# mmaker/c-lwe-snarks

Measured on AMD Instinct MI355X. Metric: snark_proofs_per_sec, higher is better.
Workload: dtype u32 limbs (704-bit integers mod 2^704) + AES-256 bytes; int8 digits on the matrix cores, int32 accumulation (exact)

## Files before the change

c-lwe-snarks_amd/__init__.py:

```python
from __future__ import annotations

import ctypes
import os
from dataclasses import dataclass

import numpy as np

_HERE = os.path.dirname(os.path.abspath(__file__))
LIB_PATH = os.environ.get("MFHIP_LIB") or os.path.join(_HERE, "libmfhip.so")
P = 0xFFFFFFFB


class MfhError(RuntimeError):
    pass


@dataclass(frozen=True)
class Params:

    n: int = 1470
    logq: int = 736
    d: int = 1 << 15
    m: int = 21845

    @property
    def L(self):
        return (self.logq + 63) // 64

    @property
    def K(self):
        return self.logq // 64

    @property
    def lanes(self):
        return (64 * self.K + 55) // 56

    @property
    def ctb(self):
        return self.logq // 8

    @property
    def ctr_ct(self):
        return self.ctb * self.n

    @property
    def ctr_s(self):
        return 0

    @property
    def ctr_as(self):
        return self.ctr_ct * self.d

    @property
    def ctr_bt(self):
        return 2 * self.ctr_ct * self.d

    @property
    def ctr_bv(self):
        return 2 * self.ctr_ct * self.d + self.ctr_ct

    @property
    def ct_limbs(self):
        return (self.n + 1) * self.L


DEBUG = Params(d=256, m=64)
DEFAULT = Params()


class _CParams(ctypes.Structure):
    _fields_ = [("n", ctypes.c_uint32), ("logq", ctypes.c_uint32), ("d", ctypes.c_uint32), ("m", ctypes.c_uint32)]


_lib = None

EXPORTS = [
    "mfh_ctx_create", "mfh_ctx_destroy", "mfh_set_stream", "mfh_sync", "mfh_scrub_staging", "mfh_last_error", "mfh_set_seed",
    "mfh_keystream", "mfh_sample_rows", "mfh_ct_add", "mfh_ct_mul_ui", "mfh_ct_addmul_ui", "mfh_eval_rows",
    "mfh_encrypt_rows", "mfh_decrypt", "mfh_ct_smudge", "mfh_ssp_upload", "mfh_witness_poly", "mfh_version",
    "mfh_workspace_bytes", "mfh_last_kernel_ms", "mfh_set_timing", "mfh_set_overlap", "mfh_eval_rows_multi", "mfh_prove_batch", "mfh_crs_mm_image_bytes", "mfh_crs_expand_mm", "mfh_crs_set_resident_mm", "mfh_witness_poly_multi", "mfh_witness_poly_mm", "mfh_poly_h_multi", "mfh_poly_mul", "mfh_poly_add", "mfh_poly_prepare_t",
    "mfh_ssp_prepare", "mfh_poly_h", "mfh_setup_messages", "mfh_setup", "mfh_setup_image", "mfh_crs_image_set_b", "mfh_prove",
    "mfh_prove_partial", "mfh_prove_finish", "mfh_ct_to_lanes", "mfh_ct_from_lanes", "mfh_lanes_per_value", "mfh_digest128", "mfh_timing_drain", "mfh_timing_busy_ms", "mfh_timing_work_rows", "mfh_set_batch_image", "mfh_set_batch_slabs", "mfh_set_expand_path", "mfh_set_encrypt_path", "mfh_set_batch_launch", "mfh_set_batch_bw", "mfh_set_mm_chunk_rows", "mfh_set_mm_pack", "mfh_set_poly_exact", "mfh_poly_exact_fallbacks", "mfh_set_mm_stream", "mfh_add_dotp", "mfh_set_encrypt_chunks", "mfh_set_witness_per", "mfh_set_eval_path", "mfh_set_decrypt_path", "mfh_decrypt_rows",
    "mfh_crs_mm_share_bytes", "mfh_crs_expand_mm_share", "mfh_crs_set_resident_mm_share", "mfh_batch_chain", "mfh_batch_witness_cols", "mfh_batch_chain_from_w", "mfh_witness_poly_mm_cols", "mfh_prove_batch_partial", "mfh_prove_batch_finish",
    "mfh_resident_row_bytes", "mfh_crs_expand", "mfh_eval_rows_resident", "mfh_crs_set_resident",
    "mfh_witness_lanes", "mfh_witness_from_lanes", "mfh_prove_partial_w", "mfh_verify",
    "mfh_ssp_set_prg", "mfh_ssp_prg_make_t", "mfh_ssp_prg_fill",
    "mfh_resident_share_rows", "mfh_crs_expand_share", "mfh_crs_set_resident_share", "mfh_crs_set_resident_prefix",
    "mfh_prove_batch_supergroup", "mfh_prove_batch_stream_wait", "mfh_set_mm_width",
    "mfh_setup_public", "mfh_prove_public", "mfh_prove_batch_public", "mfh_vk_derive", "mfh_verify_public",
    "mfh_ssp_from_rows", "mfh_ssp_set_rows", "mfh_ssp_rows_fill", "mfh_circuit_create", "mfh_circuit_destroy", "mfh_circuit_assign",
    "mfh_circuit_create_global",
]


def load_library():
    global _lib
    if _lib is not None:
        return _lib
    if not os.path.exists(LIB_PATH):
        raise MfhError(f"{LIB_PATH} is missing: run `python -c 'import __graft_entry__ as g; g.build()'` "
                       "(hipcc --offload-arch=gfx950).  There is no CPU fallback.")
    lib = ctypes.CDLL(LIB_PATH)
    vp, u64, sz, i32, u32 = ctypes.c_void_p, ctypes.c_uint64, ctypes.c_size_t, ctypes.c_int, ctypes.c_uint32
    sig = {
        "mfh_ctx_create": (i32, [ctypes.POINTER(vp), i32, ctypes.POINTER(_CParams)]),
        "mfh_ctx_destroy": (None, [vp]),
        "mfh_set_stream": (i32, [vp, vp]),
        "mfh_sync": (i32, [vp]),
        "mfh_scrub_staging": (i32, [vp]),
        "mfh_last_error": (ctypes.c_char_p, [vp]),
        "mfh_set_seed": (i32, [vp, ctypes.c_char_p]),
        "mfh_keystream": (i32, [vp, u64, vp, sz]),
        "mfh_sample_rows": (i32, [vp, u64, sz, vp]),
        "mfh_ct_add": (i32, [vp, vp, vp, vp, sz]),
        "mfh_ct_mul_ui": (i32, [vp, vp, vp, u32, sz]),
        "mfh_ct_addmul_ui": (i32, [vp, vp, vp, u32, sz]),
        "mfh_eval_rows": (i32, [vp, u64, sz, vp, vp, vp, vp, vp, i32]),
        "mfh_encrypt_rows": (i32, [vp, u64, sz, vp, vp, vp, vp]),
        "mfh_decrypt": (i32, [vp, vp, vp, sz, vp]),
        "mfh_ct_smudge": (i32, [vp, vp, sz, ctypes.c_char_p, sz, ctypes.c_char_p]),
        "mfh_ssp_upload": (i32, [vp, vp, vp, sz, sz]),
        "mfh_witness_poly": (i32, [vp, vp, ctypes.c_char_p, u32, vp]),
        "mfh_version": (ctypes.c_char_p, []),
        "mfh_workspace_bytes": (sz, [vp]),
        "mfh_last_kernel_ms": (ctypes.c_float, [vp, ctypes.c_char_p]),
        "mfh_set_timing": (i32, [vp, i32]),
        "mfh_set_overlap": (i32, [vp, i32]),
        "mfh_eval_rows_multi": (i32, [vp, u64, sz, vp, vp, u32, u32, vp, i32]),
        "mfh_poly_h_multi": (i32, [vp, vp, vp, u32]),
        "mfh_witness_poly_mm": (i32, [vp, vp, u32, ctypes.c_char_p, sz, vp, vp]),
        "mfh_witness_poly_multi": (i32, [vp, vp, u32, ctypes.c_char_p, sz, vp, vp]),
        "mfh_crs_mm_image_bytes": (sz, [vp]),
        "mfh_crs_expand_mm": (i32, [vp, vp, vp]),
        "mfh_crs_set_resident_mm": (i32, [vp, vp]),
        "mfh_prove_batch": (i32, [vp, vp, vp, u32, ctypes.c_char_p, sz, vp, ctypes.c_char_p, sz, ctypes.c_char_p, vp]),
        "mfh_prove_batch_supergroup": (u32, [vp]),
        "mfh_set_mm_width": (i32, [vp, u32, i32]),
        "mfh_prove_batch_stream_wait": (i32, [vp, u32, vp]),
        "mfh_poly_mul": (i32, [vp, vp, sz, vp, sz, vp]),
        "mfh_poly_add": (i32, [vp, vp, vp, sz, vp]),
        "mfh_poly_prepare_t": (i32, [vp, vp]),
        "mfh_ssp_prepare": (i32, [vp, vp]),
        "mfh_poly_h": (i32, [vp, vp, vp]),
        "mfh_setup_messages": (i32, [vp, vp, u32, u32, u32, vp]),
        "mfh_setup": (i32, [vp, vp, u32, u32, u32, vp, vp, vp]),
        "mfh_setup_image": (i32, [vp, vp, u32, u32, u32, vp, vp, vp, vp]),
        "mfh_prove": (i32, [vp, vp, vp, ctypes.c_char_p, u32, ctypes.c_char_p, sz, ctypes.c_char_p, vp]),
        "mfh_prove_partial": (i32, [vp, vp, vp, ctypes.c_char_p, u32, u32, u32, vp]),
        "mfh_prove_finish": (i32, [vp, vp, ctypes.c_char_p, sz, ctypes.c_char_p]),
        "mfh_lanes_per_value": (u32, [vp]),
        "mfh_digest128": (i32, [vp, vp, sz, vp]),
        "mfh_ct_to_lanes": (i32, [vp, vp, sz, vp]),
        "mfh_ct_from_lanes": (i32, [vp, vp, sz, vp]),
        "mfh_add_dotp": (i32, [vp, vp, vp, vp, sz]),
        "mfh_crs_set_resident_prefix": (i32, [vp, vp, sz]),
        "mfh_resident_share_rows": (sz, [vp, u32, u32]),
        "mfh_crs_expand_share": (i32, [vp, vp, u32, u32, vp]),
        "mfh_crs_set_resident_share": (i32, [vp, vp, u32, u32]),
        "mfh_ssp_set_prg": (i32, [vp, u64, vp]),
        "mfh_ssp_prg_make_t": (i32, [vp, u64, ctypes.c_char_p, vp]),
        "mfh_ssp_prg_fill": (i32, [vp, u64, sz, sz, vp]),
        "mfh_verify": (i32, [vp, vp, u32, u32, u32, vp, vp, sz, vp]),
        "mfh_witness_lanes": (i32, [vp, vp, ctypes.c_char_p, u32, u32, vp]),
        "mfh_witness_from_lanes": (i32, [vp, vp, vp, u32, vp]),
        "mfh_prove_partial_w": (i32, [vp, vp, vp, ctypes.c_char_p, u32, u32, u32, vp, vp]),
        "mfh_resident_row_bytes": (sz, [vp]),
        "mfh_crs_expand": (i32, [vp, u64, sz, vp, vp]),
        "mfh_crs_image_set_b": (i32, [vp, sz, sz, vp, vp]),
        "mfh_eval_rows_resident": (i32, [vp, vp, sz, sz, vp, vp, vp, vp, i32]),
        "mfh_crs_set_resident": (i32, [vp, vp]),
        "mfh_timing_drain": (i32, [vp, ctypes.c_char_p, ctypes.POINTER(u64), ctypes.POINTER(ctypes.c_double), ctypes.POINTER(u64),
                                   ctypes.POINTER(ctypes.c_float)]),
        "mfh_timing_busy_ms": (ctypes.c_double, [vp]),
        "mfh_timing_work_rows": (u64, [vp]),
        "mfh_set_batch_image": (i32, [vp, i32]),
        "mfh_set_mm_chunk_rows": (i32, [vp, u32]),
        "mfh_set_mm_pack": (i32, [vp, i32]),
        "mfh_set_poly_exact": (i32, [vp, i32]),
        "mfh_poly_exact_fallbacks": (ctypes.c_long, [vp]),
        "mfh_set_mm_stream": (i32, [vp, i32, i32, i32, u32]),
        "mfh_set_batch_launch": (i32, [vp, u32, i32]),
        "mfh_set_batch_bw": (i32, [vp, i32]),
        "mfh_set_encrypt_path": (i32, [vp, i32]),
        "mfh_set_expand_path": (i32, [vp, i32]),
        "mfh_set_batch_slabs": (i32, [vp, u32]),
        "mfh_set_encrypt_chunks": (i32, [vp, u32]),
        "mfh_set_eval_path": (i32, [vp, i32]),
        "mfh_set_decrypt_path": (i32, [vp, i32]),
        "mfh_decrypt_rows": (i32, [vp, u64, sz, vp, vp, vp]),
        "mfh_set_witness_per": (i32, [vp, u32]),
        "mfh_crs_mm_share_bytes": (sz, [vp, u32, u32]),
        "mfh_crs_expand_mm_share": (i32, [vp, vp, u32, u32, vp]),
        "mfh_crs_set_resident_mm_share": (i32, [vp, vp, u32, u32]),
        "mfh_batch_chain": (i32, [vp, vp, u32, ctypes.c_char_p, sz, vp, vp, vp, vp]),
        "mfh_batch_witness_cols": (i32, [vp, vp, u32, ctypes.c_char_p, sz, vp, u32, u32, vp, sz]),
        "mfh_batch_chain_from_w": (i32, [vp, vp, u32, vp, vp, vp]),
        "mfh_witness_poly_mm_cols": (i32, [vp, vp, u32, ctypes.c_char_p, sz, vp, u32, u32, vp, sz]),
        "mfh_prove_batch_partial": (i32, [vp, vp, u32, u32, u32, ctypes.c_char_p, sz, vp, vp, vp, sz, vp]),
        "mfh_prove_batch_finish": (i32, [vp, vp, u32, vp, ctypes.c_char_p, sz, ctypes.c_char_p, vp]),
        "mfh_setup_public": (i32, [vp, vp, u32, u32, u32, u32, vp, vp, vp, vp]),
        "mfh_prove_public": (i32, [vp, vp, vp, u32, ctypes.c_char_p, u32, ctypes.c_char_p, sz, ctypes.c_char_p, vp]),
        "mfh_prove_batch_public": (i32, [vp, vp, vp, u32, u32, ctypes.c_char_p, sz, vp, ctypes.c_char_p, sz, ctypes.c_char_p, vp]),
        "mfh_vk_derive": (i32, [vp, vp, u32, u32, vp]),
        "mfh_verify_public": (i32, [vp, vp, u32, u32, u32, vp, vp, ctypes.c_char_p, sz, sz, vp]),
        "mfh_ssp_from_rows": (i32, [vp, u32, vp, vp, vp, vp]),
        "mfh_ssp_set_rows": (i32, [vp, u32, vp, vp, vp, u32]),
        "mfh_ssp_rows_fill": (i32, [vp, sz, sz, vp]),
        "mfh_circuit_create": (i32, [vp, u32, u32, vp, u32, vp, ctypes.POINTER(vp)]),
        "mfh_circuit_create_global": (i32, [vp, u32, u32, vp, u32, vp, ctypes.POINTER(vp)]),
        "mfh_circuit_destroy": (None, [vp]),
        "mfh_circuit_assign": (i32, [vp, vp, u32, vp, sz, vp, sz, vp]),
    }
    for name, (res, args) in sig.items():
        fn = getattr(lib, name)
        fn.restype = res
        fn.argtypes = args
    _lib = lib
    return lib


def rows_to_csr(rows):
    if isinstance(rows, tuple) and len(rows) == 3 and all(isinstance(a, np.ndarray) for a in rows):
        row_ptr, wire, coef = rows
    else:
        lens = [len(r) for r in rows]
        row_ptr = np.zeros(len(lens) + 1, dtype=np.int64)
        np.cumsum(lens, out=row_ptr[1:])
        flat = [(int(w), int(a) % P) for r in rows for (w, a) in r]
        wire = np.array([w for w, _ in flat], dtype=np.int64)
        coef = np.array([a for _, a in flat], dtype=np.int64)
    if len(row_ptr) == 0 or min(np.min(row_ptr), np.min(wire, initial=0), np.min(coef, initial=0)) < 0:
        raise MfhError("rows: row_ptr needs nrows + 1 entries, and no entry may be negative")
    if max(np.max(row_ptr), np.max(wire, initial=0), np.max(coef, initial=0)) > 0xFFFFFFFF:
        raise MfhError("rows: entries must fit 32 bits")
    return tuple(np.ascontiguousarray(a, dtype=np.uint32) for a in (row_ptr, wire, coef))


def _ptr(t):
    return ctypes.c_void_p(t.data_ptr()) if t is not None else ctypes.c_void_p(0)


CIRCUIT_MAX_WIRES = 32767


class CircuitProgram:

    def __init__(self, ctx, nin, ngates, handle, state="lds"):
        self._ctx, self.nin, self.ngates, self._h, self.state = ctx, nin, ngates, handle, state

    def close(self):
        if self._h:
            self._ctx.lib.mfh_circuit_destroy(self._h)
            self._h = ctypes.c_void_p()

    def __del__(self):
        try:
            self.close()
        except Exception:
            pass


class Context:

    def __init__(self, params: Params = DEFAULT, device: int = 0):
        import torch

        if not torch.cuda.is_available():
            raise MfhError("no HIP device visible: the MI355X path has no CPU fallback")
        self.torch = torch
        self.lib = load_library()
        self.params = params
        self.device = torch.device("cuda", device)
        self._h = ctypes.c_void_p()
        cp = _CParams(params.n, params.logq, params.d, params.m)
        rc = self.lib.mfh_ctx_create(ctypes.byref(self._h), device, ctypes.byref(cp))
        if rc != 0:
            raise MfhError(f"mfh_ctx_create failed ({rc})")
        self._chk(self.lib.mfh_set_stream(self._h, ctypes.c_void_p(torch.cuda.current_stream(self.device).cuda_stream)))

    def close(self):
        if self._h:
            self.lib.mfh_ctx_destroy(self._h)
            self._h = ctypes.c_void_p()

    def __del__(self):
        try:
            self.close()
        except Exception:
            pass

    def _chk(self, rc):
        if rc != 0:
            raise MfhError(f"libmfhip error {rc}: {self.lib.mfh_last_error(self._h).decode()}")

    def empty(self, nbytes):
        return self.torch.empty(int(nbytes), dtype=self.torch.uint8, device=self.device)

    def zeros(self, nbytes):
        return self.torch.zeros(int(nbytes), dtype=self.torch.uint8, device=self.device)

    def to_device(self, arr):
        a = np.ascontiguousarray(arr)
        if not a.flags.writeable:
            import warnings

            with warnings.catch_warnings():
                warnings.simplefilter("ignore", UserWarning)
                return self.torch.from_numpy(a.view(np.uint8).reshape(-1)).to(self.device)
        return self.torch.from_numpy(a.view(np.uint8).reshape(-1)).to(self.device)

    def to_host(self, t, dtype=np.uint8):
        return t.cpu().numpy().view(dtype)

    def sync(self):
        self._chk(self.lib.mfh_sync(self._h))

    def set_timing(self, on=True):
        self._chk(self.lib.mfh_set_timing(self._h, 1 if on else 0))

    def set_overlap(self, mode=1):
        self._chk(self.lib.mfh_set_overlap(self._h, int(mode)))

    def set_batch_image(self, on=True):
        self._chk(self.lib.mfh_set_batch_image(self._h, 1 if on else 0))

    def set_batch_slabs(self, nslabs=0):
        self._chk(self.lib.mfh_set_batch_slabs(self._h, int(nslabs)))

    def set_expand_path(self, path=0):
        self._chk(self.lib.mfh_set_expand_path(self._h, int(path)))

    def set_encrypt_path(self, path=0):
        self._chk(self.lib.mfh_set_encrypt_path(self._h, int(path)))

    def set_eval_path(self, path=0):
        self._chk(self.lib.mfh_set_eval_path(self._h, int(path)))

    def set_encrypt_chunks(self, chunks=0):
        self._chk(self.lib.mfh_set_encrypt_chunks(self._h, int(chunks)))

    def set_witness_per(self, statements=0):
        self._chk(self.lib.mfh_set_witness_per(self._h, int(statements)))

    def set_batch_launch(self, groups_per_launch=4, merge_regions=True):
        self._chk(self.lib.mfh_set_batch_launch(self._h, int(groups_per_launch), 1 if merge_regions else 0))

    def set_batch_bw(self, merged=True):
        self._chk(self.lib.mfh_set_batch_bw(self._h, 1 if merged else 0))

    def set_mm_stream(self, map=0, persistent=False, sync_mode=0, spin_max=64):
        self._chk(self.lib.mfh_set_mm_stream(self._h, int(map), int(persistent), int(sync_mode), int(spin_max)))

    def set_mm_width(self, per_xcd=32, early_chain=False):
        self._chk(self.lib.mfh_set_mm_width(self._h, int(per_xcd), 1 if early_chain else 0))

    def set_mm_pack(self, on=True):
        self._chk(self.lib.mfh_set_mm_pack(self._h, 1 if on else 0))

    def set_poly_exact(self, mode=1):
        self._chk(self.lib.mfh_set_poly_exact(self._h, int(mode)))

    def poly_exact_fallbacks(self):
        return int(self.lib.mfh_poly_exact_fallbacks(self._h))

    def set_mm_chunk_rows(self, rows=0):
        self._chk(self.lib.mfh_set_mm_chunk_rows(self._h, int(rows)))

    def timing_drain(self, which):
        n, rows, ms, last = ctypes.c_uint64(), ctypes.c_uint64(), ctypes.c_double(), ctypes.c_float()
        self._chk(self.lib.mfh_timing_drain(self._h, which.encode(), ctypes.byref(n), ctypes.byref(ms), ctypes.byref(rows), ctypes.byref(last)))
        return n.value, ms.value, rows.value

    def timing_busy_ms(self):
        return float(self.lib.mfh_timing_busy_ms(self._h))

    def timing_work_rows(self):
        return int(self.lib.mfh_timing_work_rows(self._h))

    def last_kernel_ms(self, which):
        return float(self.lib.mfh_last_kernel_ms(self._h, which.encode()))

    def set_seed(self, seed: bytes):
        assert len(seed) == 40
        self._chk(self.lib.mfh_set_seed(self._h, bytes(seed)))

    def keystream(self, off, nbytes, out=None):
        out = self.empty(nbytes) if out is None else out
        self._chk(self.lib.mfh_keystream(self._h, off, _ptr(out), nbytes))
        return out

    def sample_rows(self, off, nrows):
        p = self.params
        out = self.empty(nrows * p.n * p.L * 8)
        self._chk(self.lib.mfh_sample_rows(self._h, off, nrows, _ptr(out)))
        return out

    def ct_add(self, a, b, count=1, out=None):
        out = self.empty(a.numel()) if out is None else out
        self._chk(self.lib.mfh_ct_add(self._h, _ptr(out), _ptr(a), _ptr(b), count))
        return out

    def ct_mul_ui(self, a, x, count=1, out=None):
        out = self.empty(a.numel()) if out is None else out
        self._chk(self.lib.mfh_ct_mul_ui(self._h, _ptr(out), _ptr(a), x, count))
        return out

    def ct_addmul_ui(self, rop, a, x, count=1):
        self._chk(self.lib.mfh_ct_addmul_ui(self._h, _ptr(rop), _ptr(a), x, count))
        return rop

    def eval_rows(self, off, nrows, c8, coeff0, coeff1=None, rop0=None, rop1=None, accumulate=False):
        p = self.params
        if rop0 is None:
            rop0 = self.empty(p.ct_limbs * 8)
        if coeff1 is not None and rop1 is None:
            rop1 = self.empty(p.ct_limbs * 8)
        self._chk(self.lib.mfh_eval_rows(self._h, off, nrows, _ptr(c8), _ptr(coeff0), _ptr(coeff1), _ptr(rop0), _ptr(rop1),
                                         1 if accumulate else 0))
        return rop0, rop1

    def eval_rows_multi(self, off, nrows, c8, coeffs, nvec, out=None, accumulate=False, coeff_bytes=4):
        out = self.empty(nvec * self.params.ct_limbs * 8) if out is None else out
        self._chk(self.lib.mfh_eval_rows_multi(self._h, off, nrows, _ptr(c8), _ptr(coeffs), nvec, coeff_bytes, _ptr(out), 1 if accumulate else 0))
        return out

    def encrypt_rows(self, off, nrows, sk, msg, err, out=None):
        p = self.params
        out = self.empty(nrows * p.ctb) if out is None else out
        self._chk(self.lib.mfh_encrypt_rows(self._h, off, nrows, _ptr(sk), _ptr(msg), _ptr(err), _ptr(out)))
        return out

    def decrypt(self, sk, cts, count, out=None):
        out = self.empty(4 * count) if out is None else out
        self._chk(self.lib.mfh_decrypt(self._h, _ptr(sk), _ptr(cts), count, _ptr(out)))
        return out

    def set_decrypt_path(self, path=0):
        self._chk(self.lib.mfh_set_decrypt_path(self._h, int(path)))

    def decrypt_rows(self, off, nrows, sk, c8, out=None):
        out = self.empty(4 * nrows) if out is None else out
        self._chk(self.lib.mfh_decrypt_rows(self._h, off, nrows, _ptr(sk), _ptr(c8), _ptr(out)))
        return out

    def ct_smudge(self, cts, count, mag: bytes, maglen, sign: bytes):
        self._chk(self.lib.mfh_ct_smudge(self._h, _ptr(cts), count, bytes(mag), maglen, bytes(sign)))
        return cts

    def ssp_upload(self, ssp_host_u64: np.ndarray, d_ssp=None, first_slot=0, nslots=None):
        p = self.params
        nslots = p.m + 3 if nslots is None else nslots
        if d_ssp is None:
            d_ssp = self.empty((p.m + 3) * p.d * 4)
        a = np.ascontiguousarray(ssp_host_u64)
        self._chk(self.lib.mfh_ssp_upload(self._h, ctypes.c_void_p(a.ctypes.data), _ptr(d_ssp), first_slot, nslots))
        return d_ssp

    def ssp_from_rows(self, rows, d_ssp=None):
        p = self.params
        row_ptr, wire, coef = rows_to_csr(rows)
        if d_ssp is None:
            d_ssp = self.empty((p.m + 3) * p.d * 4)
        self._chk(self.lib.mfh_ssp_from_rows(self._h, len(row_ptr) - 1, ctypes.c_void_p(row_ptr.ctypes.data), ctypes.c_void_p(wire.ctypes.data),
                                             ctypes.c_void_p(coef.ctypes.data), _ptr(d_ssp)))
        return d_ssp

    def ssp_set_rows(self, rows, lu_max=0):
        if rows is None:
            self._chk(self.lib.mfh_ssp_set_rows(self._h, 0, None, None, None, 0))
            return
        row_ptr, wire, coef = rows_to_csr(rows)
        self._chk(self.lib.mfh_ssp_set_rows(self._h, len(row_ptr) - 1, ctypes.c_void_p(row_ptr.ctypes.data), ctypes.c_void_p(wire.ctypes.data),
                                            ctypes.c_void_p(coef.ctypes.data), int(lu_max)))

    def ssp_rows_fill(self, first_slot, nslots):
        out = self.empty(max(nslots, 1) * self.params.d * 4)
        self._chk(self.lib.mfh_ssp_rows_fill(self._h, first_slot, nslots, _ptr(out)))
        return out

    def circuit_load(self, compiled, state="lds"):
        if state not in ("lds", "global", "auto"):
            raise MfhError(f"circuit_load: state must be 'lds', 'global' or 'auto', got {state!r}")
        gates = np.ascontiguousarray(compiled.gates, dtype=np.uint32).reshape(-1, 3)
        asserts = np.ascontiguousarray(compiled.asserts, dtype=np.uint32).reshape(-1, 2)
        nin = compiled.nwires - len(gates)
        if state == "auto":
            state = "lds" if compiled.nwires <= CIRCUIT_MAX_WIRES else "global"
        create = self.lib.mfh_circuit_create if state == "lds" else self.lib.mfh_circuit_create_global
        h = ctypes.c_void_p()
        self._chk(create(self._h, nin, len(gates), ctypes.c_void_p(gates.ctypes.data), len(asserts), ctypes.c_void_p(asserts.ctypes.data), ctypes.byref(h)))
        return CircuitProgram(self, nin, len(gates), h, state)

    def circuit_assign(self, prog, bits):
        bits = np.asarray(bits, dtype=np.uint8)
        if bits.ndim != 2 or bits.shape[1] != prog.nin:
            raise MfhError(f"circuit_assign: bits must be [nb, {prog.nin}] (public then private bits), got {bits.shape}")
        nb = bits.shape[0]
        packed = np.ascontiguousarray(np.packbits(bits & 1, axis=1, bitorder="little"))
        stride = (self.params.m + 7) // 8
        witness = np.zeros((nb, stride), dtype=np.uint8)
        holds = np.zeros(nb, dtype=np.uint8)
        self._chk(self.lib.mfh_circuit_assign(self._h, prog._h, nb, ctypes.c_void_p(packed.ctypes.data), packed.shape[1], ctypes.c_void_p(witness.ctypes.data),
# ... 313 lines not shown
```

c-lwe-snarks_amd/csrc/ctx.hpp:

```cpp
#pragma once
#include <hip/hip_runtime.h>

#include <stdint.h>
#include <string.h>

#include <string>
#include <vector>

#include "aes_dev.hpp"
#include "mfhip.h"
#include "ssp_prg.hpp"

#define HIP_TRY(ctx, expr)                                                        \
  do {                                                                            \
    hipError_t e_ = (expr);                                                       \
    if (e_ != hipSuccess) {                                                       \
      (ctx)->err = std::string(#expr) + ": " + hipGetErrorString(e_);             \
      return MFH_EDEVICE;                                                         \
    }                                                                             \
  } while (0)

struct PolyState;
struct SspInterp;
struct SspRows;
struct RowsTree;

struct PinBuf {
  void *p = nullptr;
  size_t cap = 0;
  hipEvent_t ev = nullptr;
  bool pending = false;
  size_t used = 0;
};

struct mfh_ctx {
  mfh_params P{};
  int device = 0;
  hipStream_t own_stream = nullptr;
  hipStream_t stream = nullptr;
  mf::AesKey key{};
  bool have_seed = false;
  uint32_t *d_t0 = nullptr;
  void *ws = nullptr;
  size_t ws_bytes = 0;
  void *ws2 = nullptr;
  size_t ws2_bytes = 0;
  int mm_ws_sel = 0;
  void *ws3 = nullptr;
  size_t ws3_bytes = 0;
  std::vector<hipEvent_t> ev_cdone, ev_rdone, ev_wdone;
  std::vector<hipEvent_t> ev_round;
  std::vector<hipEvent_t> ev_sgdone;
  uint32_t last_batch_sg = 0, last_batch_n = 0;
  void *wws = nullptr;
  size_t wws_bytes = 0;
  uint64_t *lazy = nullptr;
  uint32_t *lazy_cnt = nullptr;
  size_t lazy_bytes = 0;
  bool eval_dense = false;
  bool overlap = true;
  int overlap_mode = 1;
  hipStream_t side = nullptr, side2 = nullptr;
  hipEvent_t ev_fork = nullptr, ev_join = nullptr;
  hipEvent_t ev_chain = nullptr, ev_chain_done = nullptr;
  std::string err;
  bool timing = false;
  struct Timed {
    hipEvent_t e0, e1;
    int kind;
    uint64_t rows;
    uint64_t work;
    int sub;
  };
  std::vector<Timed> timed;
  double last_busy_ms = 0;
  uint64_t last_work_rows = 0;
  std::vector<hipEvent_t> ev_pool;
  PolyState *poly = nullptr;
  void *aux = nullptr;
  size_t aux_bytes = 0;
  uint32_t *d_msg = nullptr;
  size_t msg_rows = 0;
  uint32_t *d_prover = nullptr;
  size_t prover_words = 0;
  std::vector<uint32_t> h_cw;
  const uint8_t *mm_image = nullptr;
  uint32_t mm_rank = 0, mm_world = 1;
  uint64_t mm_off[3] = {0, 0, 0}, mm_rows[3] = {0, 0, 0};
  size_t mm_base[3] = {0, 0, 0};
  void *ssp_frag = nullptr;
  size_t ssp_frag_bytes = 0;
  const uint32_t *ssp_frag_src = nullptr;
  SspInterp *interp = nullptr;
  void *circ_io = nullptr;
  size_t circ_io_bytes = 0;
  void *circ_state = nullptr;
  size_t circ_state_bytes = 0;
  void *d_batch = nullptr;
  size_t batch_bytes = 0;
  void *batch_img = nullptr;
  size_t batch_img_bytes = 0;
  int batch_image = 1;
  int mm_map = 1;
  bool mm_persist = true;
  bool mm_wave1 = false;
  uint32_t mm_sync_mode = 0, mm_spin = 64;
  uint32_t mm_width = 32;
  size_t early_ws_half = 0;
  bool batch_early_chain = false;
  uint32_t *mm_sync = nullptr;
  int poly_exact = 1;
  bool mm_pack = true;
  uint32_t mm_chunk_rows = 131071;
  int expand_path = 0;
  int enc_path = 0;
  uint32_t ncu = 256;
  int dec_path = 0;
  int eval_path = 0;
  uint32_t enc_chunks = 0;
  uint32_t witness_per = 0;
  uint32_t batch_slabs = 0;
  int batch_bw_merged = 1;
  int batch_merge = 1;
  uint32_t batch_ngl = 8;
  PinBuf pin_rows, pin_cw, pin_smudge;
  PinBuf pin_pub;
  uint8_t *d_pub = nullptr;
  size_t pub_bytes = 0;
  PinBuf pin_wring[8];
  uint32_t pin_wnext = 0;
  hipEvent_t ev_sample = nullptr;
  void *sample_tmp = nullptr;
  size_t sample_bytes = 0;
  void *uploader = nullptr;
  bool prg_on = false;
  uint64_t prg_seed = 0;
  const uint32_t *prg_t = nullptr;
  SspRows *rows = nullptr;
  RowsTree *rows_tree = nullptr;
  const uint32_t *rows_prefix = nullptr;
  uint32_t rows_lu_max = 0;
  const uint8_t *resident_rows = nullptr;
  uint64_t resident_nrows = ~0ull;
  bool resident_sharded = false;
  uint32_t res_rank = 0, res_world = 1;
};

struct Timer {
  mfh_ctx *c;
  mfh_ctx::Timed t{};
  bool on;
  Timer(mfh_ctx *c_, int kind, uint64_t rows, uint64_t work = 0, int sub = 0) : c(c_), on(c_->timing) {
    if (!on) return;
    auto get = [&]() {
      hipEvent_t e;
      if (!c->ev_pool.empty()) { e = c->ev_pool.back(); c->ev_pool.pop_back(); }
      else hipEventCreate(&e);
      return e;
    };
    t.e0 = get(); t.e1 = get(); t.kind = kind; t.rows = rows; t.work = work ? work : rows; t.sub = sub;
    hipEventRecord(t.e0, c->stream);
  }
  ~Timer() {
    if (!on) return;
    hipEventRecord(t.e1, c->stream);
    c->timed.push_back(t);
  }
};

inline void *pin_acquire(mfh_ctx *c, PinBuf &b, size_t bytes) {
  if (b.pending) { hipEventSynchronize(b.ev); b.pending = false; }
  if (bytes > b.cap) {
    if (b.p) hipHostFree(b.p);
    b.cap = (bytes + 4095) & ~(size_t)4095;
    if (hipHostMalloc(&b.p, b.cap, hipHostMallocDefault) != hipSuccess) { b.p = nullptr; b.cap = 0; c->err = "hipHostMalloc failed"; return nullptr; }
  }
  if (!b.ev) hipEventCreateWithFlags(&b.ev, hipEventDisableTiming);
  b.used = bytes;
  return b.p;
}
inline void pin_release(mfh_ctx *c, PinBuf &b) {
  hipEventRecord(b.ev, c->stream);
  b.pending = true;
}
inline void pin_scrub(PinBuf &b) {
  if (b.pending) { hipEventSynchronize(b.ev); b.pending = false; }
  if (b.p && b.used) {
    volatile unsigned char *q = (volatile unsigned char *)b.p;
    memset((void *)q, 0, b.used);
    __asm__ __volatile__("" : : "r"(b.p) : "memory");
  }
  b.used = 0;
}
inline void pin_free(PinBuf &b) {
  if (b.pending) hipEventSynchronize(b.ev);
  if (b.p) hipHostFree(b.p);
  if (b.ev) hipEventDestroy(b.ev);
  b = PinBuf();
}

inline int ssp_src(mfh_ctx *c, const uint32_t *d_ssp, mf::SspSrc &src, bool rows_ok = false) {
  if (d_ssp) { src = mf::SspSrc{d_ssp, d_ssp, 0}; return MFH_OK; }
  if (c->rows_prefix) {
    if (!rows_ok) { c->err = "this entry point does not take the row SSP (mfh_ssp_set_rows): pass a dense d_ssp"; return MFH_EUNSUPPORTED; }
    src = mf::SspSrc{c->rows_prefix, c->rows_prefix, 0, c->rows_lu_max + 2};
    return MFH_OK;
  }
  if (!c->prg_on || !c->prg_t) { c->err = "d_ssp is NULL and no generator-defined SSP is registered (mfh_ssp_set_prg)"; return MFH_EINVAL; }
  src = mf::SspSrc{nullptr, c->prg_t, c->prg_seed};
  return MFH_OK;
}

void mfh_poly_destroy(mfh_ctx *c);
void ssp_interp_free(mfh_ctx *c);
void ssp_rows_free(mfh_ctx *c, bool tree);
int ssp_rows_check(mfh_ctx *c, const char *who, uint32_t nrows, const uint32_t *h_row_ptr, const uint32_t *h_wire, const uint32_t *h_coef);
int ssp_rows_tree(mfh_ctx *c, const char *who, const uint32_t *&d_t, const uint32_t *&h_w);
int ssp_rows_witness(mfh_ctx *c, uint32_t nstmt, const uint8_t *h_bits, size_t bits_stride, const uint32_t *h_delta, uint32_t *d_w, size_t w_stride);
int ssp_rows_msg_evals(mfh_ctx *c, uint32_t s, uint32_t beta, uint32_t *d_msg_evals);
inline bool ssp_is_rows(const mfh_ctx *c, const uint32_t *d_ssp) { return !d_ssp && c->rows_prefix; }
inline int ssp_rows_lu_check(mfh_ctx *c, const uint32_t *d_ssp, uint32_t lu) {
  if (ssp_is_rows(c, d_ssp) && lu > c->rows_lu_max) { c->err = "lu exceeds the lu_max the row SSP was registered with (mfh_ssp_set_rows)"; return MFH_EINVAL; }
  return MFH_OK;
}
extern "C" int mfh_witness_poly_mm(mfh_ctx *c, const uint32_t *d_ssp, uint32_t nstmt, const uint8_t *h_bits, size_t bits_stride, const uint32_t *h_delta,
                                   uint32_t *d_w);
extern "C" int mfh_witness_poly_mm_cols(mfh_ctx *c, const uint32_t *d_ssp, uint32_t nstmt, const uint8_t *h_bits, size_t bits_stride, const uint32_t *h_delta,
                                        uint32_t col0, uint32_t ncols, uint32_t *d_w, size_t w_stride);
extern "C" int mfh_poly_h_multi(mfh_ctx *c, const uint32_t *d_v, uint32_t *d_h, uint32_t nb);
int aux_reserve(mfh_ctx *c, size_t bytes);
int expand_mm_region(mfh_ctx *c, uint64_t off, uint32_t nrows, const uint8_t *c8, uint8_t *image);
int encrypt_rows_mm(mfh_ctx *c, uint64_t off, size_t nrows, const uint64_t *sk, const uint32_t *msg, const uint64_t *err, uint8_t *c8);
int decrypt_mm(mfh_ctx *c, const uint64_t *sk, const uint64_t *cts, size_t count, uint32_t *out);
int decrypt_rows_mm(mfh_ctx *c, uint64_t off, size_t nrows, const uint64_t *sk, const uint8_t *c8, uint32_t *out);

struct MmIo {
  const uint32_t *coef[2];
  uint32_t csplit;
  uint64_t *out[2];
  uint32_t osplit;
  uint64_t ostride;
  const uint8_t *bits;
  uint32_t bits_stride;
  int64_t *sc_zeroed;
  uint64_t cstride;
  uint32_t bits_row0;
  const uint64_t *add_ct;
  const uint32_t *add_scale;
  uint32_t sa_from1;
};
int eval_rows_multi_io(mfh_ctx *c, uint64_t off, size_t nrows, const uint8_t *d_c8, const MmIo &io, uint32_t nvec, uint32_t coeff_bytes, int accumulate);
int eval_rows_multi_io_set(mfh_ctx *c, uint64_t off, size_t nrows, const uint8_t *d_c8, const MmIo *ios, const uint32_t *nvecs, uint32_t ng,
                           uint32_t coeff_bytes);
struct MmRegion { uint64_t off; const uint8_t *c8; };
int eval_rows_multi_io_regions(mfh_ctx *c, const MmRegion *regs, uint32_t nreg, size_t nrows, const MmIo *ios, const uint32_t *nvecs, uint32_t ng,
                               uint32_t coeff_bytes, int accumulate);
bool mm_image_covers(const mfh_ctx *c, uint64_t off, size_t nrows);
struct MmsPlan {
  uint32_t ng, ngt, ND, nrows, nchunks, rpc, rpad, ntiles, mtiles;
  size_t cd_bytes, part_bytes;
  const uint8_t *img[2];
  int8_t *cd;
  int *part;
};
bool mms_plan(mfh_ctx *c, const MmRegion *regs, uint32_t nreg, size_t nrows, const MmIo *ios, const uint32_t *nvecs, uint32_t ng, uint32_t coeff_bytes,
              MmsPlan &P);
size_t mms_ws_bytes(const MmsPlan &P);
void mms_bind(MmsPlan &P, void *ws);
int mms_digits(mfh_ctx *c, const MmsPlan &P, const MmIo *ios, const uint32_t *nvecs);
int mms_stream(mfh_ctx *c, const MmsPlan &P);
int mms_finish(mfh_ctx *c, const MmsPlan &P, const MmIo *ios, const uint32_t *nvecs, int accumulate);

inline int buf_reserve(mfh_ctx *c, void *&buf, size_t &have, size_t bytes) {
  if (bytes <= have) return MFH_OK;
  if (buf) {
    hipStreamSynchronize(c->stream);
    hipFree(buf);
    buf = nullptr;
    have = 0;
  }
  bytes = (bytes + (1u << 20) - 1) & ~(size_t)((1u << 20) - 1);
  if (hipMalloc(&buf, bytes) != hipSuccess) {
    c->err = "hipMalloc(workspace) failed";
    return MFH_ENOMEM;
  }
  have = bytes;
  return MFH_OK;
}
inline int lazy_reserve(mfh_ctx *c, size_t bytes) {
  if (bytes <= c->lazy_bytes) return MFH_OK;
  if (c->lazy) {
    hipStreamSynchronize(c->stream);
    hipFree(c->lazy);
    c->lazy = nullptr;
    c->lazy_bytes = 0;
  }
  bytes = (bytes + 255) & ~(size_t)255;
  if (hipMalloc((void **)&c->lazy, bytes + 256) != hipSuccess) {
    c->err = "hipMalloc(lazy image) failed";
    return MFH_ENOMEM;
  }
  if (hipMemsetAsync(c->lazy, 0, bytes + 256, c->stream) != hipSuccess) return MFH_EDEVICE;
  c->lazy_cnt = reinterpret_cast<uint32_t *>(reinterpret_cast<uint8_t *>(c->lazy) + bytes);
  c->lazy_bytes = bytes;
  return MFH_OK;
}
inline int ws_reserve(mfh_ctx *c, size_t bytes) { return buf_reserve(c, c->ws, c->ws_bytes, bytes); }
inline int wws_reserve(mfh_ctx *c, size_t bytes) { return buf_reserve(c, c->wws, c->wws_bytes, bytes); }
inline int ws2_reserve(mfh_ctx *c, size_t bytes) { return buf_reserve(c, c->ws2, c->ws2_bytes, bytes); }
```

c-lwe-snarks_amd/csrc/evalmm.hip:

```cpp
#include <algorithm>
#include <cstring>

#include "ctx.hpp"

namespace {

using mf::AesKey;

constexpr int CT = 4;
constexpr int SB = 88;
constexpr int VB = 92;
constexpr int MB = CT * SB;
constexpr int MT = MB / 32;
constexpr int RT = 128;
constexpr int TSTRIDE = 384;
constexpr int BLK_PER_ROW = 24;
static_assert(MB % 32 == 0 && CT * VB + 15 <= TSTRIDE, "tile geometry");

typedef int v4i __attribute__((ext_vector_type(4)));
typedef int v16i __attribute__((ext_vector_type(16)));

__device__ __forceinline__ uint32_t coef_at(const MmIo &io, uint32_t v, uint32_t nrows, uint32_t i) {
  if (io.bits) {
    const uint32_t a = io.bits_row0 + i;
// ... 1029 lines not shown
      y ^= y >> 16;
      y *= 0x7FEB352Du;
      y ^= y >> 15;
      y *= 0x846CA68Bu;
      y ^= y >> 16;
      x[e] = y;
    }
    v4i bq[4];
#pragma unroll
    for (int w = 0; w < 4; w++)
#pragma unroll
      for (int j = 0; j < 4; j++) {
        const uint32_t lo = __builtin_amdgcn_perm(x[4 * j + 1], x[4 * j], 0x0c0c0400u + 0x00000101u * w);
        const uint32_t hi = __builtin_amdgcn_perm(x[4 * j + 3], x[4 * j + 2], 0x04000c0cu + 0x01010000u * w);
        bq[w][j] = (int)((lo | hi) ^ 0x80808080u);
      }
#pragma unroll
    for (int t = 0; t < MT; t++)
#pragma unroll
      for (int w = 0; w < 4; w++) acc[t][w] = __builtin_amdgcn_mfma_i32_32x32x32_i8(aq[t], bq[w], acc[t][w], 0, 0, 0);
  };
  uint32_t K = K0;
  for (; K + 2 <= K1; K += 2) {
    step(K, 0);
    step(K + 1, 1);
  }
  if (K < K1) step(K, 0);
#pragma unroll
  for (int t = 0; t < MT; t++)
#pragma unroll
    for (int w = 0; w < 4; w++)
#pragma unroll
      for (int e = 0; e < 16; e++) {
        const uint32_t stmt = 32 * t + (e & 3) + 8 * (e >> 2) + 4 * h;
        part[(((uint64_t)blockIdx.y * 4 + w) * (32 * MT) + stmt) * d + k] = acc[t][w][e];
      }
}
__global__ __launch_bounds__(512) void k_witness_mm8q_prg(const uint32_t *__restrict__ rowkeys, const v4i *__restrict__ bitfrag, uint32_t nrowsel ,
                                                          uint32_t ksteps_per_chunk, uint32_t d, int *__restrict__ part, WCols wc) {
  constexpr int MT = 8, RING = 4;
  __shared__ v4i bits[RING][MT][64];
  __shared__ uint32_t xch[3][2][4][64][4];
  const uint32_t tid = threadIdx.x, lane = tid & 63, wave = tid >> 6;
  const uint32_t r32 = lane & 31, h = lane >> 5;
  const uint32_t tile = wave >> 2, pl = wave & 3;
  const uint32_t sh = pl >> 1, pp = pl & 1;
  const uint32_t pos = (pl + (lane >> 4)) & 3;
  const uint32_t ktl = blockIdx.x * 2 + tile, kt = wc.kt0 + ktl;
  const uint32_t kc = kt * 32 + r32 + 0x632BE5ABu;
  const uint32_t K0 = blockIdx.y * ksteps_per_chunk, K1 = min((nrowsel + 31) / 32, K0 + ksteps_per_chunk);
  v16i acc[4][2];
#pragma unroll
  for (int t = 0; t < 4; t++)
#pragma unroll
    for (int q = 0; q < 2; q++)
#pragma unroll
      for (int e = 0; e < 16; e++) acc[t][q][e] = 0;
  if (K0 >= K1) return;
  auto bits_load = [&](uint32_t K) -> v4i { return bitfrag[(uint64_t)min(K, K1 - 1) * MT * 64 + tid]; };
  auto bits_store = [&](uint32_t K, v4i st) { (&bits[K % RING][0][0])[tid] = st; };
  auto rk_load = [&](uint32_t K) -> uint4 { return *reinterpret_cast<const uint4 *>(rowkeys + 32 * (uint64_t)min(K, K1 - 1) + 16 * h + 4 * pos); };
  auto hash1 = [&](uint32_t rowkey) -> uint32_t {
#ifdef WPRG_NOHASH
    return kc ^ rowkey;
#endif
    uint32_t y = kc * rowkey;
    y ^= y >> 16;
    y *= 0x7FEB352Du;
    y ^= y >> 15;
    y *= 0x846CA68Bu;
    y ^= y >> 16;
    return y;
  };
  auto publish = [&](uint32_t K, const uint32_t (&x)[4]) {
#pragma unroll
    for (int w = 0; w < 4; w++) {
      const uint32_t lo = __builtin_amdgcn_perm(x[1], x[0], 0x0c0c0400u + 0x00000101u * w);
      const uint32_t hi = __builtin_amdgcn_perm(x[3], x[2], 0x04000c0cu + 0x01010000u * w);
      xch[K % 3][tile][w][lane][pos] = (lo | hi) ^ 0x80808080u;
    }
  };
  auto fragment = [&](uint32_t K, uint32_t q) -> v4i { return *reinterpret_cast<const v4i *>(&xch[K % 3][tile][2 * pp + q][lane][0]); };
  uint4 rkr[4];
  v4i sta, stb;
  sta = bits_load(K0);
  bits_store(K0, sta);
  sta = bits_load(K0 + 1);
  stb = bits_load(K0 + 2);
  {
    const uint4 r0 = rk_load(K0), r1 = rk_load(K0 + 1);
    const uint32_t x0[4] = {hash1(r0.x), hash1(r0.y), hash1(r0.z), hash1(r0.w)};
    const uint32_t x1[4] = {hash1(r1.x), hash1(r1.y), hash1(r1.z), hash1(r1.w)};
    publish(K0, x0);
    publish(K0 + 1, x1);
  }
#pragma unroll
  for (int i = 2; i <= 5; i++) rkr[i & 3] = rk_load(K0 + i);
  __syncthreads();
  v4i bq0 = fragment(K0, 0), bq1 = fragment(K0, 1);
  uint32_t K = K0;
  auto step = [&](int slot, v4i &st) {
    const v4i bn0 = fragment(K + 1, 0), bn1 = fragment(K + 1, 1);
    const uint4 rk = rkr[(slot + 2) & 3];
    const uint32_t hr[4] = {rk.x, rk.y, rk.z, rk.w};
    uint32_t hx[4];
    bits_store(K + 1, st);
    const v4i *aq = &bits[K % RING][4 * sh][lane];
#pragma unroll
    for (int t = 0; t < 4; t++) {
      const v4i a = aq[t * 64];
#ifdef WPRG_NOMFMA
      acc[t][0][0] += a[0] ^ bq0[t];
      acc[t][1][0] += a[1] ^ bq1[t];
#else
      acc[t][0] = __builtin_amdgcn_mfma_i32_32x32x32_i8(a, bq0, acc[t][0], 0, 0, 0);
      acc[t][1] = __builtin_amdgcn_mfma_i32_32x32x32_i8(a, bq1, acc[t][1], 0, 0, 0);
#endif
      hx[t] = hash1(hr[t]);
    }
    publish(K + 2, hx);
    rkr[(slot + 2) & 3] = rk_load(K + 6);
    bq0 = bn0;
    bq1 = bn1;
    st = bits_load(K + 3);
#ifndef WPRG_NOSYNC
    __syncthreads();
#endif
    K++;
  };
  while (K + 4 <= K1) {
    step(0, sta);
    step(1, stb);
    step(2, sta);
    step(3, stb);
  }
  if (K < K1) step(0, sta);
  if (K < K1) step(1, stb);
  if (K < K1) step(2, sta);
  uint32_t dd = d;
  asm volatile("" : "+s"(dd));
#pragma unroll
  for (int q = 0; q < 2; q++) {
    int *dst = part + (((uint64_t)blockIdx.y * 4 + 2 * pp + q) * (32 * MT) + 128 * sh) * dd + ktl * 32 + r32 + (uint64_t)(4 * h) * dd;
#pragma unroll
    for (int t = 0; t < 4; t++) {
#pragma unroll
      for (int e = 0; e < 16; e++) dst[(uint64_t)((e & 3) + 8 * (e >> 2)) * dd] = acc[t][q][e];
      dst += (uint64_t)32 * dd;
    }
  }
}
__global__ __launch_bounds__(512) void k_witness_mm8q(const v4i *__restrict__ sspfrag, const v4i *__restrict__ bitfrag, uint32_t nrowsel ,
                                                      uint32_t ksteps_per_chunk, uint32_t d, int *__restrict__ part, const uint32_t *__restrict__ tpoly ,
                                                      const uint32_t *__restrict__ cnt_delta, uint32_t nstmt, uint32_t *__restrict__ w_out, WCols wc) {
  constexpr int MT = 8, RING = 4, PF = 4;
  __shared__ v4i bits[RING][MT][64];
  __shared__ uint32_t xch[2][3][16][64];
  const uint32_t tid = threadIdx.x, lane = tid & 63, wave = tid >> 6;
  const uint32_t r32 = lane & 31, h = lane >> 5;
  const uint32_t tile = wave >> 2, pl = wave & 3;
  const uint32_t ktl = blockIdx.x * 2 + tile, kt = wc.kt0 + ktl;
  const uint32_t K0 = blockIdx.y * ksteps_per_chunk, K1 = min((nrowsel + 31) / 32, K0 + ksteps_per_chunk);
  v16i acc[MT];
#pragma unroll
  for (int t = 0; t < MT; t++)
#pragma unroll
    for (int e = 0; e < 16; e++) acc[t][e] = 0;
  if (K0 >= K1) return;
  auto bits_load = [&](uint32_t K) -> v4i { return bitfrag[(uint64_t)min(K, K1 - 1) * MT * 64 + tid]; };
  auto bits_store = [&](uint32_t K, v4i st) { (&bits[K % RING][0][0])[tid] = st; };
  auto ssp_load = [&](uint32_t K) -> v4i { return sspfrag[(((uint64_t)kt * wc.KS + min(K, K1 - 1)) * 4 + pl) * 64 + lane]; };
  v4i stg[PF], bq[PF];
  {
    const v4i s0 = bits_load(K0), s1 = bits_load(K0 + 1);
    __builtin_amdgcn_sched_barrier(0);
#pragma unroll
    for (int i = 0; i < PF; i++) {
      bq[i] = ssp_load(K0 + i);
      stg[i] = bits_load(K0 + 2 + i);
      __builtin_amdgcn_sched_barrier(0);
    }
    bits_store(K0, s0);
    bits_store(K0 + 1, s1);
  }
  __syncthreads();
  v4i acur[MT];
#pragma unroll
  for (int t = 0; t < MT; t++) acur[t] = bits[K0 % RING][t][lane];
  uint32_t K = K0;
  auto step = [&](int slot) {
    bits_store(K + 2, stg[slot]);
    v4i anext[MT];
    const v4i *aq = &bits[(K + 1) % RING][0][lane];
#pragma unroll
    for (int t = 0; t < MT; t++) anext[t] = aq[t * 64];
    __builtin_amdgcn_sched_barrier(0);
#pragma unroll
    for (int t = 0; t < MT; t++) acc[t] = __builtin_amdgcn_mfma_i32_32x32x32_i8(acur[t], bq[slot], acc[t], 0, 0, 0);
    __builtin_amdgcn_sched_barrier(0);
    bq[slot] = ssp_load(K + PF);
    stg[slot] = bits_load(K + 2 + PF);
#pragma unroll
    for (int t = 0; t < MT; t++) acur[t] = anext[t];
    __syncthreads();
    K++;
  };
  while (K + PF <= K1) {
#pragma unroll
    for (int i = 0; i < PF; i++) step(i);
  }
#pragma unroll
  for (int i = 0; i + 1 < PF; i++)
    if (K < K1) step(i);
  uint32_t dd = d;
  asm volatile("" : "+s"(dd));
  if (part) {
    int *dst = part + ((uint64_t)blockIdx.y * 4 + pl) * (32 * MT) * dd + ktl * 32 + r32 + (uint64_t)(4 * h) * dd;
#pragma unroll
    for (int t = 0; t < MT; t++) {
#pragma unroll
      for (int e = 0; e < 16; e++) dst[(uint64_t)((e & 3) + 8 * (e >> 2)) * dd] = acc[t][e];
      dst += (uint64_t)32 * dd;
    }
    return;
  }
  asm volatile("" : "+s"(cnt_delta), "+s"(tpoly));
  const uint32_t k = ktl * 32 + r32;
  const uint64_t tk = tpoly[k], ws = wc.wstride, P = MFH_P;
#pragma unroll
  for (int t = 0; t < MT; t++) {
    const uint32_t owner = t >> 1;
    uint32_t mine[16];
#pragma unroll
    for (int e = 0; e < 16; e++) {
      const uint32_t b = 32 * t + (e & 3) + 8 * (e >> 2) + 4 * h;
      mine[e] = (uint32_t)acc[t][e] + (b < nstmt ? 128u * cnt_delta[2 * b] : 0u);
    }
    if (pl != owner) {
      const uint32_t sidx = pl - (pl > owner);
#pragma unroll
      for (int e = 0; e < 16; e++) xch[tile][sidx][e][lane] = mine[e];
    }
    __syncthreads();
    if (pl == owner) {
#pragma unroll
      for (int e = 0; e < 16; e++) {
        const uint32_t b = 32 * t + (e & 3) + 8 * (e >> 2) + 4 * h;
        if (b < nstmt) {
          uint64_t val = (uint64_t)mine[e] << (8 * owner);
#pragma unroll
          for (int o = 0; o < 4; o++)
            if (o != (int)owner) val += (uint64_t)xch[tile][o - (o > (int)owner)][e][lane] << (8 * o);
          w_out[(uint64_t)b * ws + k] = (uint32_t)((val % P + tk * cnt_delta[2 * b + 1] % P) % P);
        }
      }
    }
    __syncthreads();
  }
}
__global__ void k_witness_bits(const uint8_t *__restrict__ bits, size_t bits_stride, uint32_t nstmt, uint32_t nrowsel, uint32_t ksteps, uint32_t MT,
                               int8_t *__restrict__ bitfrag) {
  const uint32_t i = blockIdx.x * blockDim.x + threadIdx.x;
  if (i >= ksteps * MT * 64) return;
  const uint32_t lane = i & 63, t = (i >> 6) % MT, K = (i >> 6) / MT, stmt = 32 * t + (lane & 31), h = lane >> 5;
  const uint32_t r0 = K * 32 + 16 * h;
  uint32_t w = 0;
  if (stmt < nstmt && r0 < nrowsel) {
    const uint8_t *b = bits + (size_t)stmt * bits_stride + (r0 >> 3);
    w = b[0];
    if (r0 + 8 < nrowsel) w |= (uint32_t)b[1] << 8;
    if (nrowsel - r0 < 16) w &= (1u << (nrowsel - r0)) - 1;
  }
  uint32_t o[4];
#pragma unroll
  for (int q = 0; q < 4; q++) {
    const uint32_t n4 = (w >> (4 * q)) & 15;
    o[q] = (n4 & 1) | ((n4 & 2) << 7) | ((n4 & 4) << 14) | ((n4 & 8) << 21);
  }
  reinterpret_cast<uint4 *>(bitfrag)[i] = uint4{o[0], o[1], o[2], o[3]};
}
__global__ void k_witness_mm_finish(const int *__restrict__ part, uint32_t nchunks, const uint32_t *__restrict__ t, const uint32_t *__restrict__ cnt_delta,
                                    uint32_t nstmt, uint32_t mrows , uint32_t d, uint32_t *__restrict__ w_out, uint64_t wstride) {
  const uint32_t k = blockIdx.x * blockDim.x + threadIdx.x, b = blockIdx.y;
  if (k >= d || b >= nstmt) return;
  const uint64_t corr = 128ull * cnt_delta[2 * b];
  const uint32_t delta = cnt_delta[2 * b + 1];
  uint64_t val = 0;
#pragma unroll
  for (int w = 0; w < 4; w++) {
    int64_t g = 0;
    for (uint32_t ch = 0; ch < nchunks; ch++) g += part[(((uint64_t)ch * 4 + w) * mrows + b) * d + k];
    val += (uint64_t)(g + (int64_t)corr) << (8 * w);
  }
  const uint64_t P = MFH_P;
  w_out[(uint64_t)b * wstride + k] = (uint32_t)((val % P + (uint64_t)t[k] * delta % P) % P);
}

}

extern "C" {

struct WideGeom { uint32_t ct, sby, vby, mt, mbp, LL; };
static WideGeom wide_geom(const mfh_ctx *c) {
  if (c->P.logq == 736) return {W16<736>::CT, W16<736>::SBY, W16<736>::VBY, W16<736>::MT, W16<736>::MBP, W16<736>::LL};
  return {W16<1472>::CT, W16<1472>::SBY, W16<1472>::VBY, W16<1472>::MT, W16<1472>::MBP, W16<1472>::LL};
}

#define FINISH_LAUNCH(kern, ND_, PK_, grid, ...)                                                                         \
  do {                                                                                                                   \
    if ((PK_) && wg.sby / 4 <= 22) hipLaunchKernelGGL((kern<ND_, 22, true>), grid, dim3(256), 0, c->stream, __VA_ARGS__);  \
    else if (PK_) hipLaunchKernelGGL((kern<ND_, 46, true>), grid, dim3(256), 0, c->stream, __VA_ARGS__);                 \
    else if (wg.sby / 4 <= 22) hipLaunchKernelGGL((kern<ND_, 22, false>), grid, dim3(256), 0, c->stream, __VA_ARGS__);   \
    else hipLaunchKernelGGL((kern<ND_, 46, false>), grid, dim3(256), 0, c->stream, __VA_ARGS__);                         \
  } while (0)
// ... 209 lines not shown
  if (mms_group_args(P, ios, nvecs, A)) {
    uint32_t nvmax = 0;
    for (uint32_t g = 0; g < P.ngt; g++) nvmax = std::max(nvmax, nvecs[g]);
    FINISH_LAUNCH(k_evalmm_finish_groups, 4, pk, dim3(n + 1, (nvmax + 63) / 64, P.ngt), P.part, (uint64_t)(P.part_bytes / 4), P.nchunks, P.ntiles, (uint32_t)N2, n, P.nrows,
                  wg.ct, wg.mbp, wg.sby, wg.LL, A, accumulate);
    HIP_TRY(c, hipGetLastError());
    return MFH_OK;
  }
  for (uint32_t g = 0; g < P.ngt; g++) {
    const dim3 fgrid(n + 1, (nvecs[g] + 63) / 64);
    int *pg = P.part + g * (P.part_bytes / 4);
    if (P.ND == 4)
      FINISH_LAUNCH(k_evalmm_finish, 4, pk, fgrid, pg, ios[g].sc_zeroed, P.nchunks, P.ntiles, (uint32_t)N2, nvecs[g], n, P.nrows, wg.ct, wg.mbp, wg.sby, wg.LL, ios[g],
                    accumulate);
    else
      FINISH_LAUNCH(k_evalmm_finish, 1, pk, fgrid, pg, ios[g].sc_zeroed, P.nchunks, P.ntiles, (uint32_t)N2, nvecs[g], n, P.nrows, wg.ct, wg.mbp, wg.sby, wg.LL, ios[g],
                    accumulate);
  }
  HIP_TRY(c, hipGetLastError());
  return MFH_OK;
}
int eval_rows_multi_io_regions(mfh_ctx *c, const MmRegion *regs, uint32_t nreg, size_t nrows, const MmIo *ios, const uint32_t *nvecs, uint32_t ng,
                               uint32_t coeff_bytes, int accumulate) {
  if (!c || !regs || !ios || !nvecs || !ng || !nreg || nreg * ng > 16) return MFH_EINVAL;
  MmsPlan P;
  if (!mms_plan(c, regs, nreg, nrows, ios, nvecs, ng, coeff_bytes, P)) {
    for (uint32_t g = 0; g < nreg * ng; g++) {
      int rc = eval_rows_multi_io(c, regs[g / ng].off, nrows, regs[g / ng].c8, ios[g], nvecs[g], coeff_bytes, accumulate);
      if (rc) return rc;
    }
    return MFH_OK;
  }
  HIP_TRY(c, hipSetDevice(c->device));
  int rc = c->mm_ws_sel ? ws2_reserve(c, mms_ws_bytes(P)) : ws_reserve(c, mms_ws_bytes(P));
  if (rc) return rc;
  mms_bind(P, c->mm_ws_sel ? c->ws2 : c->ws);
  rc = mms_digits(c, P, ios, nvecs);
  if (!rc) rc = mms_stream(c, P);
  if (!rc) rc = mms_finish(c, P, ios, nvecs, accumulate);
  return rc;
}
int eval_rows_multi_io_set(mfh_ctx *c, uint64_t off, size_t nrows, const uint8_t *d_c8, const MmIo *ios, const uint32_t *nvecs, uint32_t ng,
                           uint32_t coeff_bytes) {
  const MmRegion reg = {off, d_c8};
  return eval_rows_multi_io_regions(c, &reg, 1, nrows, ios, nvecs, ng, coeff_bytes, 0);
}
bool mm_image_covers(const mfh_ctx *c, uint64_t off, size_t nrows) {
  for (int r = 0; r < 3 && c->mm_image; r++)
    if (c->mm_off[r] == off && c->mm_rows[r] == nrows && nrows) return true;
  return false;
}

extern "C" {

static size_t mm_region_bytes(const mfh_ctx *c, uint64_t rows) {
  const WideGeom wg = wide_geom(c);
  const uint64_t mtiles = (uint64_t)((c->P.n + 1 + wg.ct - 1) / wg.ct) * wg.mt, ksteps = (rows + RT2 - 1) / RT2 * (RT2 / 64);
  return (size_t)(mtiles * ksteps * 1024);
}
struct MmShare { uint64_t row0[3], rows[3]; };
static MmShare mm_share(const mfh_ctx *c, uint32_t rank, uint32_t world) {
  const uint64_t d = c->P.d, m = c->P.m;
  const uint64_t loS = d * rank / world, cS = d * (rank + 1) / world - loS, lo = m * rank / world, cnt = m * (rank + 1) / world - lo;
  return MmShare{{loS, d + loS, 2 * d + lo}, {cS, cS, cnt}};
}
size_t mfh_crs_mm_share_bytes(const mfh_ctx *c, uint32_t rank, uint32_t world) {
  if (!c || !world || rank >= world) return 0;
  const MmShare sh = mm_share(c, rank, world);
  return mm_region_bytes(c, sh.rows[0]) + mm_region_bytes(c, sh.rows[1]) + mm_region_bytes(c, sh.rows[2]);
}
size_t mfh_crs_mm_image_bytes(const mfh_ctx *c) { return mfh_crs_mm_share_bytes(c, 0, 1); }
int mfh_crs_expand_mm_share(mfh_ctx *c, const uint8_t *d_crs_c8, uint32_t rank, uint32_t world, uint8_t *d_image) {
  if (!c || !d_crs_c8 || !d_image || !world || rank >= world) return MFH_EINVAL;
  if (!c->have_seed) { c->err = "mfh_set_seed has not been called"; return MFH_EINVAL; }
  const WideGeom wg = wide_geom(c);
  const uint32_t n = c->P.n;
  if (((uint64_t)n * wg.vby) & 7) { c->err = "mfh_crs_expand_mm: the row length must be a multiple of 8"; return MFH_EUNSUPPORTED; }
  HIP_TRY(c, hipSetDevice(c->device));
  const uint64_t ctr_ct = (uint64_t)wg.vby * n;
  const MmShare sh = mm_share(c, rank, world);
  AesKey keyx = c->key;
  for (int i = 56; i < 60; i++) keyx.rk[i] ^= 0x80808080u;
  const uint32_t ntiles = (n + 1 + wg.ct - 1) / wg.ct;
  size_t base = 0;
  for (int r = 0; r < 3; r++) {
    if (!sh.rows[r]) continue;
    const uint32_t units = (uint32_t)((sh.rows[r] + RT2 - 1) / RT2);
    const uint32_t nchunks = std::max(1u, std::min(units, 4u));
    const uint32_t rpc = (units + nchunks - 1) / nchunks * RT2;
    Timer t(c, 9, sh.rows[r]);
    const dim3 grid(ntiles, (uint32_t)((sh.rows[r] + rpc - 1) / rpc));
    const uint8_t *c8 = d_crs_c8 + (size_t)sh.row0[r] * wg.vby;
    if (c->expand_path == 0 && ((ctr_ct * sh.row0[r]) & 7) == 0) {
      int rc = expand_mm_region(c, ctr_ct * sh.row0[r], (uint32_t)sh.rows[r], c8, d_image + base);
      if (rc) return rc;
      base += mm_region_bytes(c, sh.rows[r]);
      continue;
    }
    if (c->P.logq == 736)
      hipLaunchKernelGGL((k_evalmm16<1, 736>), grid, dim3(1024), 0, c->stream, keyx, c->d_t0, ctr_ct * sh.row0[r], n, (uint32_t)sh.rows[r], rpc, c8,
                         (const int8_t *)nullptr, (int *)nullptr, d_image + base);
    else
      hipLaunchKernelGGL((k_evalmm16<1, 1472>), grid, dim3(1024), 0, c->stream, keyx, c->d_t0, ctr_ct * sh.row0[r], n, (uint32_t)sh.rows[r], rpc, c8,
                         (const int8_t *)nullptr, (int *)nullptr, d_image + base);
    base += mm_region_bytes(c, sh.rows[r]);
  }
  HIP_TRY(c, hipGetLastError());
  return MFH_OK;
}
int mfh_crs_expand_mm(mfh_ctx *c, const uint8_t *d_crs_c8, uint8_t *d_image) { return mfh_crs_expand_mm_share(c, d_crs_c8, 0, 1, d_image); }
int mfh_set_mm_stream(mfh_ctx *c, int map, int persistent, int sync_mode, uint32_t spin_max) {
  if (!c || map < 0 || map > 1 || sync_mode < 0 || sync_mode > 2 || persistent < 0 || persistent > 2) return MFH_EINVAL;
  c->mm_map = map;
  c->mm_persist = persistent != 0;
  c->mm_wave1 = persistent == 2;
  c->mm_sync_mode = (uint32_t)sync_mode;
  c->mm_spin = spin_max;
  return MFH_OK;
}
int mfh_set_mm_width(mfh_ctx *c, uint32_t per_xcd, int early_chain) {
  if (!c || per_xcd < 1 || per_xcd > 32) return MFH_EINVAL;
  c->mm_width = per_xcd;
  c->batch_early_chain = early_chain != 0;
  return MFH_OK;
}
int mfh_set_mm_pack(mfh_ctx *c, int on) {
  if (!c) return MFH_EINVAL;
  c->mm_pack = on != 0;
  return MFH_OK;
}
int mfh_set_mm_chunk_rows(mfh_ctx *c, uint32_t rows) {
  if (!c || rows > 131071) return MFH_EINVAL;
  c->mm_chunk_rows = rows ? rows : 131071;
  return MFH_OK;
}
int mfh_crs_set_resident_mm_share(mfh_ctx *c, const uint8_t *d_image, uint32_t rank, uint32_t world) {
  if (!c || !world || rank >= world) return MFH_EINVAL;
  c->mm_image = d_image;
  c->mm_rank = rank;
  c->mm_world = world;
  const uint64_t ctr_ct = (uint64_t)wide_geom(c).vby * c->P.n;
  const MmShare sh = mm_share(c, rank, world);
  size_t base = 0;
  for (int r = 0; r < 3; r++) {
    c->mm_off[r] = ctr_ct * sh.row0[r];
    c->mm_rows[r] = sh.rows[r];
    c->mm_base[r] = base;
    base += mm_region_bytes(c, sh.rows[r]);
  }
  return MFH_OK;
}
int mfh_crs_set_resident_mm(mfh_ctx *c, const uint8_t *d_image) { return mfh_crs_set_resident_mm_share(c, d_image, 0, 1); }

int mfh_witness_poly_mm_cols(mfh_ctx *c, const uint32_t *d_ssp, uint32_t nstmt, const uint8_t *h_bits, size_t bits_stride, const uint32_t *h_delta,
                             uint32_t col0, uint32_t ncols, uint32_t *d_w, size_t w_stride) {
  if (!c || !h_bits || !h_delta || !d_w || nstmt == 0 || nstmt > 256) return MFH_EINVAL;
  mf::SspSrc src;
  {
    int rc0 = ssp_src(c, d_ssp, src);
    if (rc0) return rc0;
  }
  const uint32_t MT = nstmt > 128 ? 8 : nstmt > 64 ? 4 : nstmt > 32 ? 2 : 1;
  const uint32_t d = c->P.d, m = c->P.m;
  if (d % 128 || m < 2) { c->err = "mfh_witness_poly_mm: d must be a multiple of 128"; return MFH_EUNSUPPORTED; }
  if ((uint64_t)col0 + ncols > d || w_stride < ncols) return MFH_EINVAL;
  if (ncols == 0) return MFH_OK;
  if (col0 % 128 || ncols % 128) { c->err = "mfh_witness_poly_mm_cols: the coefficient range must start and end at multiples of 128"; return MFH_EUNSUPPORTED; }
  const uint32_t nc = ncols;
  const WCols wc = {col0 / 32, (m - 1 + 31) / 32, (uint64_t)w_stride};
  const uint32_t *tpoly = src.t + col0;
  for (uint32_t b = 0; b < nstmt; b++)
    if (h_delta[b] >= MFH_P) { c->err = "delta must be < p"; return MFH_EINVAL; }
  HIP_TRY(c, hipSetDevice(c->device));
  const uint32_t nrowsel = m - 1, ksteps = (nrowsel + 31) / 32;
  const bool fused = MT == 8 && src.dense && m < 65536 && (nc >= 16384 || ksteps <= 64);
  const uint32_t nchunks = fused ? 1u : std::min(ksteps, 4u), kpc = (ksteps + nchunks - 1) / nchunks;
  const size_t sfrag_b = (size_t)ksteps * 32 * d * 4;
  if (src.dense && (c->ssp_frag_src != d_ssp || c->ssp_frag_bytes < sfrag_b)) {
    if (c->ssp_frag_bytes < sfrag_b) {
      if (c->ssp_frag) { hipStreamSynchronize(c->stream); hipFree(c->ssp_frag); c->ssp_frag = nullptr; c->ssp_frag_bytes = 0; }
      HIP_TRY(c, hipMalloc(&c->ssp_frag, sfrag_b));
      c->ssp_frag_bytes = sfrag_b;
    }
    const uint64_t nthreads = (uint64_t)ksteps * (d / 32) * 256;
    hipLaunchKernelGGL(k_ssp_frag, dim3((uint32_t)((nthreads + 255) / 256)), dim3(256), 0, c->stream, d_ssp, nrowsel, d, (uint32_t *)c->ssp_frag);
    HIP_TRY(c, hipGetLastError());
    c->ssp_frag_src = d_ssp;
  }
  const size_t packed = (size_t)nstmt * bits_stride, head_b = ((packed + 8 + 256 * 8 + 255) & ~(size_t)255);
  const size_t frag_b = (size_t)ksteps * MT * 1024, part_b = (size_t)nchunks * 4 * 32 * MT * nc * 4;
  const size_t rk_b = src.dense ? 0 : (((size_t)ksteps * 32 * 4 + 255) & ~(size_t)255);
  int rc = wws_reserve(c, head_b + frag_b + part_b + rk_b);
  if (rc) return rc;
  PinBuf &wpin = c->pin_wring[c->pin_wnext++ % 8];
  uint8_t *stage = (uint8_t *)pin_acquire(c, wpin, head_b);
  if (!stage) return MFH_ENOMEM;
  memcpy(stage, h_bits, packed);
  uint32_t *cd = (uint32_t *)(stage + packed + ((8 - packed % 8) % 8));
  for (uint32_t b = 0; b < nstmt; b++) {
    uint32_t cnt = 0;
    const uint8_t *hb = h_bits + (size_t)b * bits_stride;
    for (uint32_t r = 0; r + 8 <= nrowsel; r += 8) cnt += (uint32_t)__builtin_popcount(hb[r >> 3]);
    for (uint32_t r = nrowsel & ~7u; r < nrowsel; r++) cnt += (hb[r >> 3] >> (r & 7)) & 1;
    cd[2 * b] = cnt;
    cd[2 * b + 1] = h_delta[b];
  }
  uint8_t *dev = (uint8_t *)c->wws;
  HIP_TRY(c, hipMemcpyAsync(dev, stage, head_b, hipMemcpyHostToDevice, c->stream));
  pin_release(c, wpin);
  const uint32_t *d_cd = (const uint32_t *)(dev + packed + ((8 - packed % 8) % 8));
  int8_t *d_frag = (int8_t *)(dev + head_b);
  int *d_part = (int *)(dev + head_b + frag_b);
  hipLaunchKernelGGL(k_witness_bits, dim3((uint32_t)((frag_b / 16 + 255) / 256)), dim3(256), 0, c->stream, dev, bits_stride, nstmt, nrowsel, ksteps, MT, d_frag);
  if (!src.dense) {
    uint32_t *d_rk = (uint32_t *)(dev + head_b + frag_b + part_b);
    const dim3 grid(nc / 128, (ksteps + kpc - 1) / kpc);
    hipLaunchKernelGGL(k_prg_rowkeys, dim3((ksteps * 32 + 255) / 256), dim3(256), 0, c->stream, src.seed, ksteps * 32, d_rk);
    if (MT == 8)
      hipLaunchKernelGGL(k_witness_mm8q_prg, dim3(nc / 64, (ksteps + kpc - 1) / kpc), dim3(512), 0, c->stream, d_rk, (const v4i *)d_frag, nrowsel, kpc, nc, d_part, wc);
    else if (MT == 1) hipLaunchKernelGGL(k_witness_mm_prg<1>, grid, dim3(256), 0, c->stream, d_rk, (const v4i *)d_frag, nrowsel, kpc, nc, d_part, wc);
    else if (MT == 2) hipLaunchKernelGGL(k_witness_mm_prg<2>, grid, dim3(256), 0, c->stream, d_rk, (const v4i *)d_frag, nrowsel, kpc, nc, d_part, wc);
    else hipLaunchKernelGGL(k_witness_mm_prg<4>, grid, dim3(256), 0, c->stream, d_rk, (const v4i *)d_frag, nrowsel, kpc, nc, d_part, wc);
  } else if (MT == 8) {
    hipLaunchKernelGGL(k_witness_mm8q, dim3(nc / 64, (ksteps + kpc - 1) / kpc), dim3(512), 0, c->stream, (const v4i *)c->ssp_frag, (const v4i *)d_frag, nrowsel, kpc, nc,
                       fused ? (int *)nullptr : d_part, tpoly, d_cd, nstmt, d_w, wc);
    if (fused) {
      HIP_TRY(c, hipGetLastError());
      return MFH_OK;
    }
  } else if (MT == 1)
    hipLaunchKernelGGL(k_witness_mm<1>, dim3(nc / 128, (ksteps + kpc - 1) / kpc), dim3(256), 0, c->stream, (const v4i *)c->ssp_frag, (const v4i *)d_frag,
                       nrowsel, kpc, nc, d_part, wc);
  else if (MT == 2)
    hipLaunchKernelGGL(k_witness_mm<2>, dim3(nc / 128, (ksteps + kpc - 1) / kpc), dim3(256), 0, c->stream, (const v4i *)c->ssp_frag, (const v4i *)d_frag,
                       nrowsel, kpc, nc, d_part, wc);
  else
    hipLaunchKernelGGL(k_witness_mm<4>, dim3(nc / 128, (ksteps + kpc - 1) / kpc), dim3(256), 0, c->stream, (const v4i *)c->ssp_frag, (const v4i *)d_frag,
                       nrowsel, kpc, nc, d_part, wc);
  hipLaunchKernelGGL(k_witness_mm_finish, dim3((nc + 255) / 256, nstmt), dim3(256), 0, c->stream, d_part, (ksteps + kpc - 1) / kpc, tpoly, d_cd, nstmt, 32 * MT,
                     nc, d_w, (uint64_t)w_stride);
  HIP_TRY(c, hipGetLastError());
  return MFH_OK;
}

int mfh_witness_poly_mm(mfh_ctx *c, const uint32_t *d_ssp, uint32_t nstmt, const uint8_t *h_bits, size_t bits_stride, const uint32_t *h_delta,
                        uint32_t *d_w) {
  if (!c) return MFH_EINVAL;
  if (ssp_is_rows(c, d_ssp)) {
    if (!h_bits || !h_delta || !d_w || nstmt == 0 || nstmt > 256) return MFH_EINVAL;
    return ssp_rows_witness(c, nstmt, h_bits, bits_stride, h_delta, d_w, c->P.d);
  }
  return mfh_witness_poly_mm_cols(c, d_ssp, nstmt, h_bits, bits_stride, h_delta, 0, c->P.d, d_w, c->P.d);
}

}
```

c-lwe-snarks_amd/csrc/mfhip.hip:

```cpp
#include <hip/hip_runtime.h>

#include <stdint.h>
#include <stdio.h>
#include <string.h>

#include <algorithm>
#include <string>
#include <thread>
#include <vector>

#include "aes_dev.hpp"
#include "mfhip.h"

using mf::AesKey;

template <int LOGQ>
struct PS {
  static constexpr int CTB = LOGQ / 8;
  static constexpr int EW = CTB / 4;
  static constexpr int L = (LOGQ + 63) / 64;
  static constexpr int K = LOGQ / 64;
  static constexpr int KW = 2 * K;
  static constexpr int TILE = LOGQ == 736 ? 512 : 256;
  static constexpr int ROWS = 2;
// ... 936 lines not shown
  if (P->logq != 736 && P->logq != 1472) return MFH_EUNSUPPORTED;
  if (P->n == 0 || P->n > (1u << 20)) return MFH_EINVAL;
  int ndev = 0;
  if (hipGetDeviceCount(&ndev) != hipSuccess || ndev <= 0 || device < 0 || device >= ndev) return MFH_EDEVICE;
  if (hipSetDevice(device) != hipSuccess) return MFH_EDEVICE;
  mfh_ctx *c = new mfh_ctx();
  c->P = *P;
  c->device = device;
  {
    int ncu = 0;
    if (hipDeviceGetAttribute(&ncu, hipDeviceAttributeMultiprocessorCount, device) == hipSuccess && ncu > 0) c->ncu = (uint32_t)ncu;
  }
  if (hipStreamCreateWithFlags(&c->own_stream, hipStreamNonBlocking) != hipSuccess) {
    delete c;
    return MFH_EDEVICE;
  }
  c->stream = c->own_stream;
  uint32_t t0[512];
  mf::make_t0_le(t0);
  for (int a = 0; a < 256; a++) t0[256 + a] = (t0[a] << 24) | (t0[a] >> 8);
  if (hipMalloc(&c->d_t0, sizeof t0) != hipSuccess || hipMemcpy(c->d_t0, t0, sizeof t0, hipMemcpyHostToDevice) != hipSuccess) {
    mfh_ctx_destroy(c);
    return MFH_EDEVICE;
  }
  *out = c;
  return MFH_OK;
}

void mfh_ctx_destroy(mfh_ctx *c) {
  if (!c) return;
  hipSetDevice(c->device);
  if (c->stream) hipStreamSynchronize(c->stream);
  mfh_poly_destroy(c);
  ssp_interp_free(c);
  ssp_rows_free(c, true);
  upload_free(c);
  if (c->sample_tmp) hipFree(c->sample_tmp);
  if (c->ev_sample) hipEventDestroy(c->ev_sample);
  pin_free(c->pin_rows);
  for (auto &b : c->pin_wring) pin_free(b);
  pin_free(c->pin_cw);
  pin_free(c->pin_smudge);
  pin_free(c->pin_pub);
  if (c->side) hipStreamSynchronize(c->side);
  if (c->ws) hipFree(c->ws);
  if (c->wws) hipFree(c->wws);
  if (c->ws2) hipFree(c->ws2);
  if (c->ws3) hipFree(c->ws3);
  if (c->mm_sync) hipFree(c->mm_sync);
  for (hipEvent_t e : c->ev_round) hipEventDestroy(e);
  for (hipEvent_t e : c->ev_sgdone) hipEventDestroy(e);
  for (hipEvent_t e : c->ev_cdone) hipEventDestroy(e);
  for (hipEvent_t e : c->ev_rdone) hipEventDestroy(e);
  for (hipEvent_t e : c->ev_wdone) hipEventDestroy(e);
  if (c->lazy) hipFree(c->lazy);
  if (c->aux) hipFree(c->aux);
  if (c->ev_fork) hipEventDestroy(c->ev_fork);
  if (c->ev_join) hipEventDestroy(c->ev_join);
  if (c->ev_chain) hipEventDestroy(c->ev_chain);
  if (c->ev_chain_done) hipEventDestroy(c->ev_chain_done);
  if (c->side) hipStreamDestroy(c->side);
  if (c->side2) hipStreamDestroy(c->side2);
  if (c->d_msg) hipFree(c->d_msg);
  if (c->d_prover) hipFree(c->d_prover);
  if (c->d_pub) hipFree(c->d_pub);
  if (c->d_batch) hipFree(c->d_batch);
  if (c->batch_img) hipFree(c->batch_img);
  if (c->circ_io) hipFree(c->circ_io);
  if (c->circ_state) hipFree(c->circ_state);
  if (c->ssp_frag) hipFree(c->ssp_frag);
  if (c->d_t0) hipFree(c->d_t0);
  for (auto &t : c->timed) { hipEventDestroy(t.e0); hipEventDestroy(t.e1); }
  for (auto e : c->ev_pool) hipEventDestroy(e);
  if (c->own_stream) hipStreamDestroy(c->own_stream);
  delete c;
}

int mfh_set_stream(mfh_ctx *c, void *s) {
  if (!c) return MFH_EINVAL;
  c->stream = (hipStream_t)s;
  return MFH_OK;
}

int mfh_sync(mfh_ctx *c) {
  if (!c) return MFH_EINVAL;
  HIP_TRY(c, hipStreamSynchronize(c->stream));
  return MFH_OK;
}

int mfh_scrub_staging(mfh_ctx *c) {
  if (!c) return MFH_EINVAL;
  pin_scrub(c->pin_rows);
  pin_scrub(c->pin_cw);
  pin_scrub(c->pin_smudge);
  for (auto &b : c->pin_wring) pin_scrub(b);
  return MFH_OK;
}

const char *mfh_last_error(const mfh_ctx *c) { return c ? c->err.c_str() : "null context"; }
size_t mfh_workspace_bytes(const mfh_ctx *c) { return c ? c->ws_bytes : 0; }
int mfh_set_overlap(mfh_ctx *c, int en) {
  if (!c) return MFH_EINVAL;
  c->overlap = en != 0;
  c->overlap_mode = en > 1 ? en : 1;
  return MFH_OK;
}

int mfh_set_expand_path(mfh_ctx *c, int path) {
  if (!c || path < 0 || path > 1) return MFH_EINVAL;
  c->expand_path = path;
  return MFH_OK;
}

int mfh_set_encrypt_path(mfh_ctx *c, int path) {
  if (!c || path < 0 || path > 2) return MFH_EINVAL;
  c->enc_path = path;
  return MFH_OK;
}

int mfh_set_eval_path(mfh_ctx *c, int path) {
  if (!c || path < 0 || path > 1) return MFH_EINVAL;
  c->eval_path = path;
  return MFH_OK;
}
int mfh_set_encrypt_chunks(mfh_ctx *c, uint32_t chunks) {
  if (!c || chunks > 64) return MFH_EINVAL;
  c->enc_chunks = chunks;
  return MFH_OK;
}
int mfh_set_witness_per(mfh_ctx *c, uint32_t statements) {
  if (!c || (statements && (statements < 32 || statements > 256))) return MFH_EINVAL;
  c->witness_per = statements;
  return MFH_OK;
}
int mfh_set_batch_slabs(mfh_ctx *c, uint32_t nslabs) {
  if (!c || nslabs > 256) return MFH_EINVAL;
  c->batch_slabs = nslabs;
  return MFH_OK;
}

int mfh_set_batch_launch(mfh_ctx *c, uint32_t groups_per_launch, int merge_regions) {
  if (!c || groups_per_launch < 1 || groups_per_launch > 8) return MFH_EINVAL;
  c->batch_ngl = groups_per_launch;
  c->batch_merge = merge_regions != 0;
  return MFH_OK;
}

int mfh_set_batch_bw(mfh_ctx *c, int merged) {
  if (!c) return MFH_EINVAL;
  c->batch_bw_merged = merged != 0;
  return MFH_OK;
}

int mfh_set_batch_image(mfh_ctx *c, int en) {
  if (!c) return MFH_EINVAL;
  c->batch_image = en != 0;
  if (!en && c->batch_img) {
    HIP_TRY(c, hipDeviceSynchronize());
    hipFree(c->batch_img);
    c->batch_img = nullptr;
    c->batch_img_bytes = 0;
  }
  return MFH_OK;
}

int mfh_set_timing(mfh_ctx *c, int en) {
  if (!c) return MFH_EINVAL;
  c->timing = en != 0;
  return MFH_OK;
}
static int timing_kind(const char *which) {
  if (!strcmp(which, "keystream")) return 0;
  if (!strcmp(which, "eval1")) return 1;
  if (!strcmp(which, "eval2")) return 2;
  if (!strcmp(which, "encrypt")) return 3;
  if (!strcmp(which, "eval")) return 12;
  if (!strcmp(which, "expand")) return 4;
  if (!strcmp(which, "mac1")) return 5;
  if (!strcmp(which, "mac2")) return 6;
  if (!strcmp(which, "evalmm")) return 7;
  if (!strcmp(which, "evalmm_resident")) return 8;
  if (!strcmp(which, "expandmm")) return 9;
  if (!strcmp(which, "decrypt")) return 11;
  if (!strcmp(which, "decrypt_rows")) return 13;
  if (!strcmp(which, "mmstream_bw")) return 14;
  if (!strcmp(which, "mmstream_rounds")) return 10;
  if (!strcmp(which, "mmstream_rounds_persistent")) return 110;
  if (!strcmp(which, "mmstream_bw_persistent")) return 114;
  if (!strcmp(which, "ssp_interp")) return 15;
  if (!strcmp(which, "circuit_assign")) return 16;
  if (!strcmp(which, "circuit_assign_global")) return 17;
  return -1;
}

int mfh_timing_drain(mfh_ctx *c, const char *which, uint64_t *count, double *total_ms, uint64_t *total_rows, float *last_ms) {
  if (!c || !which) return MFH_EINVAL;
  const int kind = timing_kind(which);
  if (kind < 0) return MFH_EINVAL;
  HIP_TRY(c, hipStreamSynchronize(c->stream));
  if (c->side) HIP_TRY(c, hipStreamSynchronize(c->side));
  uint64_t n = 0, rows = 0, work = 0;
  double tot = 0;
  float last = -1.f;
  std::vector<mfh_ctx::Timed> keep;
  std::vector<std::pair<float, float>> spans;
  hipEvent_t base = nullptr;
  for (auto &t : c->timed) {
    const bool match = t.kind == kind || (kind == 12 && (t.kind == 1 || t.kind == 2)) || (kind == 8 && (t.kind == 10 || t.kind == 14)) || (kind >= 100 && t.kind == kind - 100 && t.sub == 1);
    if (!match) { keep.push_back(t); continue; }
    float ms = 0;
    if (hipEventElapsedTime(&ms, t.e0, t.e1) == hipSuccess) {
      n++; tot += ms; rows += t.rows; work += t.work; last = ms;
      if (!base) base = t.e0;
      float s0 = 0;
      if (hipEventElapsedTime(&s0, base, t.e0) == hipSuccess) spans.emplace_back(s0, s0 + ms);
    }
  }
  std::sort(spans.begin(), spans.end());
  double busy = 0;
  float hi = -1e30f;
  for (auto &sp : spans) {
    if (sp.second <= hi) continue;
    busy += sp.second - std::max(sp.first, hi);
    hi = sp.second;
  }
  c->last_busy_ms = busy;
  c->last_work_rows = work;
  for (auto &t : c->timed) {
    const bool match = t.kind == kind || (kind == 12 && (t.kind == 1 || t.kind == 2)) || (kind == 8 && (t.kind == 10 || t.kind == 14)) || (kind >= 100 && t.kind == kind - 100 && t.sub == 1);
    if (!match) continue;
    c->ev_pool.push_back(t.e0);
    c->ev_pool.push_back(t.e1);
  }
  c->timed.swap(keep);
  if (count) *count = n;
  if (total_ms) *total_ms = tot;
  if (total_rows) *total_rows = rows;
  if (last_ms) *last_ms = last;
  return MFH_OK;
}

double mfh_timing_busy_ms(const mfh_ctx *c) { return c ? c->last_busy_ms : -1.0; }
uint64_t mfh_timing_work_rows(const mfh_ctx *c) { return c ? c->last_work_rows : 0; }

float mfh_last_kernel_ms(mfh_ctx *c, const char *which) {
  float last = -1.f;
  if (mfh_timing_drain(c, which, nullptr, nullptr, nullptr, &last) != MFH_OK) return -1.f;
  return last;
}

int mfh_set_seed(mfh_ctx *c, const uint8_t seed[40]) {
  if (!c || !seed) return MFH_EINVAL;
  mf::expand_key(c->key, seed);
  c->have_seed = true;
  return MFH_OK;
}

#define NEED_SEED(c)                                  \
  do {                                                \
    if (!(c)->have_seed) {                            \
      (c)->err = "mfh_set_seed has not been called";  \
      return MFH_EINVAL;                              \
    }                                                 \
  } while (0)

#define DISPATCH_LOGQ(c, CALL736, CALL1472) \
  do {                                      \
    if ((c)->P.logq == 736) {               \
      CALL736;                              \
    } else {                                \
      CALL1472;                             \
    }                                       \
  } while (0)

int mfh_digest128(mfh_ctx *c, const void *d_buf, size_t nbytes, uint64_t h_digest[2]) {
  if (!c || (!d_buf && nbytes) || !h_digest || (reinterpret_cast<uintptr_t>(d_buf) & 3)) return MFH_EINVAL;
  HIP_TRY(c, hipSetDevice(c->device));
  int rc = aux_reserve(c, 16);
  if (rc) return rc;
  HIP_TRY(c, hipMemsetAsync(c->aux, 0, 16, c->stream));
  const uint64_t nwords = (nbytes + 3) / 4;
  const uint32_t grid = (uint32_t)std::min<uint64_t>(2048, (nwords + 255) / 256);
  if (grid) hipLaunchKernelGGL(k_digest128, dim3(grid), dim3(256), 0, c->stream, (const uint8_t *)d_buf, (uint64_t)nbytes, (unsigned long long *)c->aux);
  HIP_TRY(c, hipGetLastError());
  HIP_TRY(c, hipMemcpyAsync(h_digest, c->aux, 16, hipMemcpyDeviceToHost, c->stream));
  HIP_TRY(c, hipStreamSynchronize(c->stream));
  return MFH_OK;
}

int mfh_keystream(mfh_ctx *c, uint64_t off, void *d_out, size_t nbytes) {
  if (!c || (!d_out && nbytes)) return MFH_EINVAL;
  NEED_SEED(c);
  if (!nbytes) return MFH_OK;
  HIP_TRY(c, hipSetDevice(c->device));
  uint64_t nblk = ((off & 15) + nbytes + 15) >> 4;
  uint32_t grid = (uint32_t)std::min<uint64_t>((nblk + 1023) / 1024, 256 * 2);
  {
    Timer t(c, 0, nblk);
    hipLaunchKernelGGL(k_keystream, dim3(grid), dim3(1024), 0, c->stream, c->key, c->d_t0, off, (uint8_t *)d_out, (uint64_t)nbytes);
  }
  HIP_TRY(c, hipGetLastError());
  return MFH_OK;
}

int mfh_sample_rows(mfh_ctx *c, uint64_t off, size_t nrows, uint64_t *d_out) {
  if (!c || (!d_out && nrows)) return MFH_EINVAL;
// ... 669 lines not shown
```

c-lwe-snarks_amd/csrc/poly.hip:

```cpp
#include <algorithm>

#include "ctx.hpp"
#include "ntt.hpp"

namespace {

#define MF_NEEDED(need, vs) do { if ((need) && (vs) >= *(need)) return; } while (0)

using namespace mf_ntt;

__device__ __forceinline__ uint32_t lz_mont(uint32_t a, uint32_t b, uint32_t p, uint32_t ninv) {
  uint64_t t = (uint64_t)a * b;
  uint32_t m = (uint32_t)t * ninv;
  return (uint32_t)((t + (uint64_t)m * p) >> 32);
}
__device__ __forceinline__ uint32_t lz_add(uint32_t a, uint32_t b, uint32_t p2) {
  uint32_t s = a + b;
  return min(s, s - p2);
}
__device__ __forceinline__ uint32_t lz_canon(uint32_t a, uint32_t p) { return min(a, a - p); }
__device__ __forceinline__ void lz_dif(uint32_t &x, uint32_t &y, uint32_t w, uint32_t p, uint32_t ninv) {
  const uint32_t u = x, z = y;
  x = lz_add(u, z, 2 * p);
  y = lz_mont(u - z + 2 * p, w, p, ninv);
// ... 761 lines not shown
  std::vector<uint32_t> one(Nc);
  HIP_TRY(c, hipMemcpyAsync(one.data(), sp, (size_t)Nc * 4, hipMemcpyDeviceToHost, c->stream));
  HIP_TRY(c, hipStreamSynchronize(c->stream));
  if (one[0] != 1 || std::any_of(one.begin() + 1, one.end(), [](uint32_t x) { return x != 0; })) return MFH_OK;
  HIP_TRY(c, hipMalloc(&S->d_That, (size_t)3 * Nc * 4));
  hipLaunchKernelGGL(k_ntt_load, dim3((Nc + 255) / 256, 3), dim3(256), 0, c->stream, inv[cur], Nc, Nc, S->P, S->d_That, (size_t)0, (const uint32_t *)nullptr,
                     (const uint32_t *)nullptr);
  forward(c, S->d_That, logNc);
  std::vector<uint32_t> pw((size_t)4 * Nc);
  for (int j = 0; j < 4; j++) {
    uint64_t z = 0x9e3779b97f4a7c15ull * (uint64_t)(j + 1);
    z = (z ^ (z >> 30)) * 0xbf58476d1ce4e5b9ull;
    z = (z ^ (z >> 27)) * 0x94d049bb133111ebull;
    const uint64_t r = 2 + (z ^ (z >> 31)) % (P32 - 2);
    uint64_t x = 1, tv = 0;
    for (uint32_t i = 0; i < Nc; i++) {
      pw[(size_t)j * Nc + i] = (uint32_t)x;
      if (i < d) tv = (tv + x * t[i]) % P32;
      x = x * r % P32;
    }
    S->chk_t[j] = (uint32_t)tv;
  }
  HIP_TRY(c, hipMalloc(&S->d_chk, pw.size() * 4));
  HIP_TRY(c, hipMemcpyAsync(S->d_chk, pw.data(), pw.size() * 4, hipMemcpyHostToDevice, c->stream));
  HIP_TRY(c, hipGetLastError());
  HIP_TRY(c, hipStreamSynchronize(c->stream));
  S->logNc = logNc;
  S->cyc = true;
  return MFH_OK;
}

}

int ntt_reserve(mfh_ctx *c, uint32_t logmax) { return poly_init(c, std::max(logmax, 1u)); }
const Primes3 &ntt_primes(const mfh_ctx *c) { return c->poly->P; }
Crt ntt_crt_make(const mfh_ctx *c, uint32_t logB) { return make_crt(c->poly, logB); }
void ntt_blocks_forward(mfh_ctx *c, uint32_t *buf, uint32_t N, uint32_t logB, uint32_t nb) {
  PolyState *S = c->poly;
  const uint32_t half_max = 1u << (S->logmax - 1), B = std::min(logB, 11u);
  const uint32_t *nil = nullptr;
  uint32_t top = logB - B, len = 1u << logB;
  while (top) {
    const uint32_t k = top > 5 ? std::min(top - 3, 5u) : top;
    dim3 g(((N >> k) + 255) / 256, 3 * nb);
    switch (k) {
      case 5: hipLaunchKernelGGL(k_ntt_dif_multi<5>, g, dim3(256), 0, c->stream, buf, N, len, S->d_tw, half_max, S->P, nil, 0u, (size_t)0, nil, nil); break;
      case 4: hipLaunchKernelGGL(k_ntt_dif_multi<4>, g, dim3(256), 0, c->stream, buf, N, len, S->d_tw, half_max, S->P, nil, 0u, (size_t)0, nil, nil); break;
      case 3: hipLaunchKernelGGL(k_ntt_dif_multi<3>, g, dim3(256), 0, c->stream, buf, N, len, S->d_tw, half_max, S->P, nil, 0u, (size_t)0, nil, nil); break;
      case 2: hipLaunchKernelGGL(k_ntt_dif_multi<2>, g, dim3(256), 0, c->stream, buf, N, len, S->d_tw, half_max, S->P, nil, 0u, (size_t)0, nil, nil); break;
      default: hipLaunchKernelGGL(k_ntt_dif_multi<1>, g, dim3(256), 0, c->stream, buf, N, len, S->d_tw, half_max, S->P, nil, 0u, (size_t)0, nil, nil); break;
    }
    len >>= k;
    top -= k;
  }
  hipLaunchKernelGGL(k_ntt_lds<false>, dim3(N >> B, 3 * nb), dim3(256), 0, c->stream, buf, N, B, S->d_tw, half_max, S->P);
}
void ntt_blocks_inverse(mfh_ctx *c, uint32_t *buf, uint32_t N, uint32_t logB, uint32_t nb) {
  PolyState *S = c->poly;
  const uint32_t half_max = 1u << (S->logmax - 1), B = std::min(logB, 11u);
  hipLaunchKernelGGL(k_ntt_lds<true>, dim3(N >> B, 3 * nb), dim3(256), 0, c->stream, buf, N, B, S->d_twi, half_max, S->P);
  uint32_t top = logB - B, len = 2u << B;
  while (top) {
    const uint32_t k = top > 5 ? std::min(top - 3, 5u) : top;
    dim3 g(((N >> k) + 255) / 256, 3 * nb);
    const uint32_t *nil = nullptr;
    switch (k) {
      case 5: hipLaunchKernelGGL(k_ntt_dit_multi<5>, g, dim3(256), 0, c->stream, buf, N, len, S->d_twi, half_max, S->P, nil); break;
      case 4: hipLaunchKernelGGL(k_ntt_dit_multi<4>, g, dim3(256), 0, c->stream, buf, N, len, S->d_twi, half_max, S->P, nil); break;
      case 3: hipLaunchKernelGGL(k_ntt_dit_multi<3>, g, dim3(256), 0, c->stream, buf, N, len, S->d_twi, half_max, S->P, nil); break;
      case 2: hipLaunchKernelGGL(k_ntt_dit_multi<2>, g, dim3(256), 0, c->stream, buf, N, len, S->d_twi, half_max, S->P, nil); break;
      default: hipLaunchKernelGGL(k_ntt_dit_multi<1>, g, dim3(256), 0, c->stream, buf, N, len, S->d_twi, half_max, S->P, nil); break;
    }
    len <<= k;
    top -= k;
  }
}

void mfh_poly_destroy(mfh_ctx *c) {
  delete c->poly;
  c->poly = nullptr;
}

extern "C" {

int mfh_poly_mul(mfh_ctx *c, const uint32_t *d_a, size_t la, const uint32_t *d_b, size_t lb, uint32_t *d_c) {
  if (!c || !d_a || !d_b || !d_c || !la || !lb) return MFH_EINVAL;
  HIP_TRY(c, hipSetDevice(c->device));
  int rc = poly_init(c, std::max(ceil_log2(la + lb - 1), 1u));
  if (rc) return rc;
  return poly_mul(c, d_a, (uint32_t)la, d_b, (uint32_t)lb, nullptr, 0, d_c, (uint32_t)(la + lb - 1));
}

int mfh_poly_prepare_t(mfh_ctx *c, const uint32_t *d_t) {
  if (!c) return MFH_EINVAL;
  c->ssp_frag_src = nullptr;
  if (c->poly) {
    c->poly->have_t = false;
    c->poly->cyc = false;
  }
  if (!d_t) return MFH_EINVAL;
  HIP_TRY(c, hipSetDevice(c->device));
  const uint32_t d = c->P.d;
  std::vector<uint32_t> t(d);
  HIP_TRY(c, hipMemcpyAsync(t.data(), d_t, (size_t)d * 4, hipMemcpyDeviceToHost, c->stream));
  HIP_TRY(c, hipStreamSynchronize(c->stream));
  int64_t dt = -1;
  for (int64_t i = (int64_t)d - 1; i >= 0; i--)
    if (t[i]) { dt = i; break; }
  if (dt < 0) {
    c->err = "t(x) is the zero polynomial: (v^2-1)/t is undefined (nmod_poly_div would raise)";
    return MFH_EINVAL;
  }
  const uint32_t n = 2 * d - 1 - (uint32_t)dt;
  uint32_t logmax = std::max(ceil_log2((size_t)2 * d), ceil_log2((size_t)2 * n + dt + 2));
  int rc = poly_init(c, logmax);
  if (rc) return rc;
  PolyState *S = c->poly;
  for (uint32_t **p : {&S->d_G, &S->d_Ghat, &S->d_f})
    if (*p) { hipFree(*p); *p = nullptr; }
  S->have_t = false;
  S->d = d; S->dt = (uint32_t)dt; S->n = n;
  S->logN2 = std::max(ceil_log2((size_t)2 * n - 1), 1u);
  const uint32_t N2 = 1u << S->logN2;
  HIP_TRY(c, hipMalloc(&S->d_G, (size_t)std::max(n, 2u) * 4 * 2));
  HIP_TRY(c, hipMalloc(&S->d_Ghat, (size_t)3 * N2 * 4));
  HIP_TRY(c, hipMalloc(&S->d_f, (size_t)(dt + 1) * 4));
  hipLaunchKernelGGL(k_reverse, g1((uint32_t)dt + 1), dim3(256), 0, c->stream, d_t, dt, (uint32_t)dt + 1, S->d_f);
  uint32_t g0 = invp(t[dt]);
  HIP_TRY(c, hipMemsetAsync(S->d_G, 0, (size_t)std::max(n, 2u) * 4 * 2, c->stream));
  HIP_TRY(c, hipMemcpyAsync(S->d_G, &g0, 4, hipMemcpyHostToDevice, c->stream));
  HIP_TRY(c, hipStreamSynchronize(c->stream));
  for (uint32_t k = 1; k < n;) {
    const uint32_t k2 = std::min(2 * k, n);
    const uint32_t lf = std::min(k2, (uint32_t)dt + 1);
    rc = poly_mul(c, S->d_f, lf, S->d_G, k, nullptr, 0, S->d_tmp, std::min(k2, lf + k - 1));
    if (rc) return rc;
    if (lf + k - 1 < k2) HIP_TRY(c, hipMemsetAsync(S->d_tmp + (lf + k - 1), 0, (size_t)(k2 - (lf + k - 1)) * 4, c->stream));
    hipLaunchKernelGGL(k_two_minus, g1(k2), dim3(256), 0, c->stream, S->d_tmp, k2);
    rc = poly_mul(c, S->d_G, k, S->d_tmp, k2, nullptr, 0, S->d_tmp2, k2);
    if (rc) return rc;
    HIP_TRY(c, hipMemcpyAsync(S->d_G, S->d_tmp2, (size_t)k2 * 4, hipMemcpyDeviceToDevice, c->stream));
    k = k2;
  }
  hipLaunchKernelGGL(k_ntt_load, dim3((N2 + 255) / 256, 3), dim3(256), 0, c->stream, S->d_G, n, N2, S->P, S->d_Ghat, (size_t)0, (const uint32_t *)nullptr,
                     (const uint32_t *)nullptr);
  forward(c, S->d_Ghat, S->logN2);
  HIP_TRY(c, hipGetLastError());
  HIP_TRY(c, hipStreamSynchronize(c->stream));
  if ((rc = prepare_exact(c, d_t, t))) return rc;
  S->have_t = true;
  return MFH_OK;
}

int mfh_poly_h_multi(mfh_ctx *c, const uint32_t *d_v, uint32_t *d_h, uint32_t nb) {
  if (!c || !d_v || !d_h || !nb || nb > kMaxBatch) return MFH_EINVAL;
  PolyState *S = c->poly;
  if (!S || !S->have_t) {
    c->err = "mfh_poly_prepare_t has not been called for this SSP";
    return MFH_EINVAL;
  }
  HIP_TRY(c, hipSetDevice(c->device));
  int rc = poly_batch_reserve(c, nb);
  if (rc) return rc;
  const uint32_t d = S->d, n = S->n;
  const size_t Nmax = (size_t)1 << S->logmax;
  const uint32_t *need = nullptr;
  bool exact = S->cyc && c->poly_exact && nb >= 4;
  if (exact && c->poly_exact == 1) {
    if (*(volatile uint32_t *)S->h_seen) {
      *(volatile uint32_t *)S->h_seen = 0;
      S->rest = 64;
    }
    if (S->rest) {
      S->rest--;
      exact = false;
    }
  }
  if (exact) {
    const uint32_t Nc = 1u << S->logNc;
    HIP_TRY(c, hipMemsetAsync(S->d_need, 0, 4, c->stream));
    if (S->logNc >= 12 && S->logNc <= 16) {
      const uint32_t half_max = 1u << (S->logmax - 1), K = S->logNc - 11;
      const Crt C = make_crt(S, S->logNc);
      const dim3 gs(((Nc >> K) + 255) / 256, nb), gl(Nc >> 11, 3 * nb);
      forward_top(c, S->d_bufA, S->logNc, nb, d_v, d, d);
      hipLaunchKernelGGL(k_ntt_lds_mul8, gl, dim3(256), 0, c->stream, S->d_bufA, (const uint32_t *)nullptr, Nc, S->d_tw, S->d_twi, half_max, S->P, (const uint32_t *)nullptr);
#define MF_SEAM(K_, LAST_, out_, keep_, stride_) \
  hipLaunchKernelGGL((k_exact_seam<K_, LAST_>), gs, dim3(256), 0, c->stream, S->d_bufA, Nc, S->d_tw, S->d_twi, half_max, S->P, C, out_, keep_, stride_)
#define MF_SEAM_K(LAST_, out_, keep_, stride_)                  \
  switch (K) {                                                  \
    case 1: MF_SEAM(1, LAST_, out_, keep_, stride_); break;     \
    case 2: MF_SEAM(2, LAST_, out_, keep_, stride_); break;     \
    case 3: MF_SEAM(3, LAST_, out_, keep_, stride_); break;     \
    case 4: MF_SEAM(4, LAST_, out_, keep_, stride_); break;     \
    default: MF_SEAM(5, LAST_, out_, keep_, stride_); break;    \
  }
      MF_SEAM_K(false, (uint32_t *)nullptr, 0u, (size_t)0)
      hipLaunchKernelGGL(k_ntt_lds_mul8, gl, dim3(256), 0, c->stream, S->d_bufA, (const uint32_t *)S->d_That, Nc, S->d_tw, S->d_twi, half_max, S->P, (const uint32_t *)nullptr);
      MF_SEAM_K(true, d_h, d, (size_t)d)
#undef MF_SEAM_K
#undef MF_SEAM
    } else {
      rc = poly_mul(c, d_v, d, d_v, d, nullptr, 0, S->d_tmp, Nc, nb, d, Nmax, nullptr, S->logNc);
      if (rc) return rc;
      hipLaunchKernelGGL(k_sub_const0, dim3(nb), dim3(64), 0, c->stream, S->d_tmp, 1u, Nmax, (const uint32_t *)nullptr);
      rc = poly_mul(c, S->d_tmp, Nc, nullptr, Nc, S->d_That, S->logNc, d_h, d, nb, Nmax, d, nullptr, S->logNc);
      if (rc) return rc;
    }
    hipLaunchKernelGGL(k_exact_check, dim3(nb), dim3(1024), 0, c->stream, d_v, d_h, d, S->d_chk, Nc, uint4{S->chk_t[0], S->chk_t[1], S->chk_t[2], S->chk_t[3]},
                       S->d_need, S->h_seen);
    need = S->d_need;
  }
  const uint32_t *map = need ? need + 2 : nullptr;
  if (S->dt >= 1) {
    rc = poly_mul(c, d_v, d, d_v, d, nullptr, 0, S->d_tmp2, n, nb, d, Nmax, need, 0, map, (int64_t)(2 * d - 2), 2 * d - 1);
    if (rc) return rc;
    rc = poly_mul(c, S->d_tmp2, n, nullptr, n, S->d_Ghat, S->logN2, d_h, d, nb, Nmax, d, need, 0, nullptr, (int64_t)n - 1, n, map);
    if (rc) return rc;
    HIP_TRY(c, hipGetLastError());
    return MFH_OK;
  }
  rc = poly_mul(c, d_v, d, d_v, d, nullptr, 0, S->d_tmp, 2 * d - 1, nb, d, Nmax, need, 0, map);
  if (rc) return rc;
  hipLaunchKernelGGL(k_sub_const0, dim3(nb), dim3(64), 0, c->stream, S->d_tmp, 1u, Nmax, need);
  hipLaunchKernelGGL(k_reverse, dim3((n + 255) / 256, nb), dim3(256), 0, c->stream, S->d_tmp, (int64_t)(2 * d - 2), n, S->d_tmp2, Nmax, Nmax, need);
  rc = poly_mul(c, S->d_tmp2, n, nullptr, n, S->d_Ghat, S->logN2, S->d_tmp, n, nb, Nmax, Nmax, need);
  if (rc) return rc;
  hipLaunchKernelGGL(k_unreverse_pad, dim3((d + 255) / 256, nb), dim3(256), 0, c->stream, S->d_tmp, n, d, d_h, Nmax, (size_t)d, need, map);
  HIP_TRY(c, hipGetLastError());
  return MFH_OK;
}
int mfh_set_poly_exact(mfh_ctx *c, int mode) {
  if (!c || mode < 0 || mode > 2) return MFH_EINVAL;
  c->poly_exact = mode;
  if (c->poly && c->poly->h_seen) {
    *c->poly->h_seen = 0;
    c->poly->rest = 0;
  }
  return MFH_OK;
}
long mfh_poly_exact_fallbacks(mfh_ctx *c) {
  if (!c || !c->poly || !c->poly->cyc) return -1;
  HIP_TRY(c, hipSetDevice(c->device));
  uint32_t w[2] = {0, 0};
  if (hipMemcpyAsync(w, c->poly->d_need, 8, hipMemcpyDeviceToHost, c->stream) != hipSuccess || hipStreamSynchronize(c->stream) != hipSuccess ||
      hipMemsetAsync(c->poly->d_need + 1, 0, 4, c->stream) != hipSuccess)
    return -1;
  return (long)w[1];
}
int mfh_poly_h(mfh_ctx *c, const uint32_t *d_v, uint32_t *d_h) { return mfh_poly_h_multi(c, d_v, d_h, 1); }

int mfh_poly_add(mfh_ctx *c, const uint32_t *d_a, const uint32_t *d_b, size_t count, uint32_t *d_out) {
  if (!c || !d_a || !d_b || !d_out) return MFH_EINVAL;
  HIP_TRY(c, hipSetDevice(c->device));
  hipLaunchKernelGGL(k_add_vec, g1((uint32_t)count), dim3(256), 0, c->stream, d_a, d_b, (uint32_t)count, d_out);
  HIP_TRY(c, hipGetLastError());
  return MFH_OK;
}

}
```

c-lwe-snarks_amd/csrc/snark.hip:

```cpp
#include <algorithm>
#include <cstdlib>
#include <cstring>
#include <vector>

#include "ctx.hpp"
#include "p32.hpp"

namespace {

__device__ __forceinline__ uint32_t ssp_coef(const mf::SspSrc &src, uint32_t slot, uint32_t rowkey, uint32_t d, uint32_t k) {
  if (src.dense) return src.dense[(uint64_t)slot * d + k];
  return slot == 0 ? src.t[k] : mf::ssp_prg_coeff(rowkey, k);
}

__global__ void k_powers(uint32_t s, uint32_t d, uint32_t *__restrict__ pw) {
  uint32_t k = blockIdx.x * blockDim.x + threadIdx.x;
  if (k >= d) return;
  uint32_t r = 1, b = s, e = k;
  while (e) {
    if (e & 1) r = mulp(r, b);
    b = mulp(b, b);
    e >>= 1;
  }
  pw[k] = r;
// ... 516 lines not shown
constexpr uint32_t BSG_REGEN = 248;

struct OnStream {
  mfh_ctx *c;
  hipStream_t keep;
  OnStream(mfh_ctx *c_, hipStream_t s) : c(c_), keep(c_->stream) { c->stream = s; }
  ~OnStream() { c->stream = keep; }
};
struct OnSide {
  mfh_ctx *c;
  hipStream_t keep;
  OnSide(mfh_ctx *c_, hipStream_t s) : c(c_), keep(c_->stream) { c->stream = s; c->mm_ws_sel = 1; }
  ~OnSide() { c->stream = keep; c->mm_ws_sel = 0; }
};

struct BatchScratch {
  uint32_t *WHV;
  uint8_t *CW;
  size_t cw_stride, cw_delta_off;
  uint32_t *SMU;
  uint8_t *SMS;
  uint32_t *ONE;
  uint64_t *CT_T;
  int64_t *SCZ;
  size_t nslots;
};
int batch_scratch(mfh_ctx *c, uint32_t nproofs, uint32_t whv , BatchScratch &B, uint32_t ncw = 1,
                  uint32_t nsmudge = 0 ) {
  const uint32_t d = c->P.d, m = c->P.m, n = c->P.n;
  const size_t ctl = (size_t)(n + 1) * ((c->P.logq + 63) / 64);
  const size_t nsg = ((size_t)nproofs + BSG_REGEN - 1) / BSG_REGEN;
  B.nslots = nsg * (2 + 2 * ((BSG + BG - 1) / BG));
  const size_t whv_b = (size_t)whv * 3 * BSG * d * 4;
  const size_t packed = ((size_t)BSG * ((m + 6) / 8) + 3) & ~(size_t)3;
  const size_t cw_b = packed + (size_t)BSG * 4;
  const size_t cw_pad = (cw_b + 255) & ~(size_t)255;
  const size_t KW = 2 * (c->P.logq / 64);
  const size_t sm_b = ((size_t)nsmudge * 5 * (KW * 4 + 1) + 255) & ~(size_t)255;
  const size_t need = whv_b + cw_pad * ncw + sm_b + 256 + ctl * 8 + B.nslots * 2048;
  if (c->batch_bytes < need) {
    if (c->d_batch) { hipDeviceSynchronize(); hipFree(c->d_batch); c->d_batch = nullptr; c->batch_bytes = 0; }
    HIP_TRY(c, hipMalloc(&c->d_batch, need));
    c->batch_bytes = need;
  }
  uint8_t *base = (uint8_t *)c->d_batch;
  B.WHV = (uint32_t *)base;
  B.CW = base + whv_b;
  B.cw_stride = cw_pad;
  B.cw_delta_off = packed;
  B.SMU = (uint32_t *)(base + whv_b + cw_pad * ncw);
  B.SMS = (uint8_t *)B.SMU + (size_t)nsmudge * 5 * KW * 4;
  B.ONE = (uint32_t *)(base + whv_b + cw_pad * ncw + sm_b);
  B.CT_T = (uint64_t *)(base + whv_b + cw_pad * ncw + sm_b + 256);
  B.SCZ = (int64_t *)(base + whv_b + cw_pad * ncw + sm_b + 256 + ctl * 8);
  return MFH_OK;
}
int batch_stage_host(mfh_ctx *c, const BatchScratch &B, uint32_t nproofs, const uint8_t *h_bits, size_t bits_stride, const uint32_t *h_delta,
                     const uint8_t *h_mag, size_t maglen, const uint8_t *h_sign, uint32_t SG) {
  const uint32_t m = c->P.m, nsg = (nproofs + SG - 1) / SG;
  const uint32_t bstride = (m + 6) / 8, KW = 2 * (c->P.logq / 64);
  if (maglen + 4 > (size_t)KW * 4) { c->err = "smudge magnitude too wide"; return MFH_EINVAL; }
  const size_t total = (size_t)((uint8_t *)B.SMS - B.CW) + (size_t)nproofs * 5;
  uint8_t *st = (uint8_t *)pin_acquire(c, c->pin_cw, total);
  if (!st) return MFH_ENOMEM;
  for (uint32_t g = 0; g < nsg; g++) {
    const uint32_t s0 = g * SG, sg = std::min(SG, nproofs - s0);
    uint8_t *a = st + (size_t)g * B.cw_stride;
    for (uint32_t b = 0; b < sg; b++) memcpy(a + (size_t)b * bstride, h_bits + (size_t)(s0 + b) * bits_stride, bstride);
    memcpy(a + B.cw_delta_off, h_delta + s0, (size_t)sg * 4);
  }
  uint32_t *up = (uint32_t *)(st + ((uint8_t *)B.SMU - B.CW));
  for (size_t i = 0; i < (size_t)nproofs * 5; i++) {
    uint64_t carry = 0;
    for (uint32_t l = 0; l < KW; l++) {
      uint32_t w = 0;
      const size_t o = (size_t)l * 4;
      if (o < maglen) memcpy(&w, h_mag + i * maglen + o, std::min<size_t>(4, maglen - o));
      const uint64_t t = (uint64_t)w * P32 + carry;
      up[i * KW + l] = (uint32_t)t;
      carry = t >> 32;
    }
  }
  memcpy(st + ((uint8_t *)B.SMS - B.CW), h_sign, (size_t)nproofs * 5);
  HIP_TRY(c, hipMemcpyAsync(B.CW, st, total, hipMemcpyHostToDevice, c->stream));
  pin_release(c, c->pin_cw);
  return MFH_OK;
}
__global__ void k_smudge_batch(uint64_t *cts, uint32_t n, uint32_t L, uint32_t KW, const uint32_t *__restrict__ up, const uint8_t *__restrict__ sign,
                               uint32_t count, uint32_t per, uint32_t slot0, uint32_t uslot0) {
  const uint32_t i = blockIdx.x * blockDim.x + threadIdx.x;
  if (i >= count) return;
  const uint32_t pb = i / per, j = i % per;
  uint32_t *b = reinterpret_cast<uint32_t *>(cts + ((uint64_t)(pb * 5 + slot0 + j) * (n + 1) + n) * L);
  const uint32_t *u = up + (uint64_t)(pb * 5 + uslot0 + j) * KW;
  if (sign[pb * 5 + uslot0 + j] & 1) {
    uint32_t borrow = 0;
    for (uint32_t l = 0; l < KW; l++) {
      const uint64_t t = (uint64_t)b[l] - u[l] - borrow;
      b[l] = (uint32_t)t;
      borrow = (uint32_t)(t >> 63);
    }
  } else {
    uint32_t carry = 0;
    for (uint32_t l = 0; l < KW; l++) {
      const uint64_t t = (uint64_t)b[l] + u[l] + carry;
      b[l] = (uint32_t)t;
      carry = (uint32_t)(t >> 32);
    }
  }
  for (uint32_t l = KW; l < 2 * L; l++) b[l] = 0;
}
int batch_smudge_staged(mfh_ctx *c, const BatchScratch &B, uint64_t *sproofs, uint32_t s0, uint32_t sg) {
  const uint32_t L = (c->P.logq + 63) / 64, KW = 2 * (c->P.logq / 64);
  const uint32_t *up = B.SMU + (size_t)s0 * 5 * KW;
  const uint8_t *sn = B.SMS + (size_t)s0 * 5;
  hipLaunchKernelGGL(k_smudge_batch, dim3((sg * 4 + 63) / 64), dim3(64), 0, c->stream, sproofs, c->P.n, L, KW, up, sn, sg * 4, 4u, 0u, 0u);
  hipLaunchKernelGGL(k_smudge_batch, dim3((sg + 63) / 64), dim3(64), 0, c->stream, sproofs, c->P.n, L, KW, up, sn, sg, 1u, 3u, 4u);
  HIP_TRY(c, hipGetLastError());
  return MFH_OK;
}
int batch_streams(mfh_ctx *c) {
  if (!c->side) {
    HIP_TRY(c, hipStreamCreateWithFlags(&c->side, hipStreamNonBlocking));
    HIP_TRY(c, hipEventCreateWithFlags(&c->ev_fork, hipEventDisableTiming));
    HIP_TRY(c, hipEventCreateWithFlags(&c->ev_join, hipEventDisableTiming));
  }
  if (!c->ev_chain) {
    HIP_TRY(c, hipStreamCreateWithFlags(&c->side2, hipStreamNonBlocking));
    HIP_TRY(c, hipEventCreateWithFlags(&c->ev_chain, hipEventDisableTiming));
    HIP_TRY(c, hipEventCreateWithFlags(&c->ev_chain_done, hipEventDisableTiming));
  }
  return MFH_OK;
}

constexpr uint32_t kPubDirect = 64;
constexpr int kPubNB = 16;
struct PubBatch {
  uint32_t lu;
  const uint8_t *d_ubits;
  uint32_t ub;
  const uint8_t *h_pub;
  size_t pub_stride;
  const uint32_t *h_zero;
  PubBatch at(uint32_t s0) const {
    PubBatch p = *this;
    p.d_ubits += (size_t)s0 * ub;
    if (h_pub) p.h_pub += (size_t)s0 * pub_stride;
    if (h_zero) p.h_zero += s0;
    return p;
  }
};

int batch_chain_launch(mfh_ctx *c, const mf::SspSrc &src, const uint32_t *d_ssp, uint32_t sg, const uint8_t *h_bits, size_t bits_stride,
                       const uint32_t *h_delta, uint32_t *W, uint32_t *H, uint32_t *V, hipEvent_t ev_witness = nullptr, const PubBatch *pub = nullptr) {
  const uint32_t d = c->P.d;
  int rc = MFH_OK;
  auto witness_pass = [&](const uint8_t *bits, size_t stride, const uint32_t *delta, uint32_t *out) -> int {
    if (d % 128 == 0) {
      const uint32_t per = c->witness_per ? c->witness_per : 256u;
      for (uint32_t b0 = 0; b0 < sg; b0 += per) {
        int r = mfh_witness_poly_mm(c, d_ssp, std::min(per, sg - b0), bits + (size_t)b0 * stride, stride, delta + b0, out + (size_t)b0 * d);
        if (r) return r;
      }
    } else {
      for (uint32_t b0 = 0; b0 < sg; b0 += 12) {
        int r = mfh_witness_poly_multi(c, d_ssp, std::min(12u, sg - b0), bits + (size_t)b0 * stride, stride, delta + b0, out + (size_t)b0 * d);
        if (r) return r;
      }
    }
    return MFH_OK;
  };
  rc = witness_pass(h_bits, bits_stride, h_delta, W);
  if (rc) return rc;
  const bool pub_pass = pub && pub->lu > kPubDirect;
  if (pub_pass) {
    rc = witness_pass(pub->h_pub, pub->pub_stride, pub->h_zero, H);
    if (rc) return rc;
  }
  if (ev_witness) HIP_TRY(c, hipEventRecord(ev_witness, c->stream));
  if (pub)
    hipLaunchKernelGGL(k_add_public<kPubNB>, dim3((d + 255) / 256, (sg + kPubNB - 1) / kPubNB), dim3(256), 0, c->stream, W, src, d, pub_pass ? 0u : pub->lu,
                       pub->d_ubits, pub->ub, sg, pub_pass ? H : nullptr, V);
  else
    hipLaunchKernelGGL(k_add_slot_multi, dim3((d + 255) / 256, sg), dim3(256), 0, c->stream, W, src, 1u, d, V);
  HIP_TRY(c, hipGetLastError());
  return mfh_poly_h_multi(c, V, H, sg);
}

struct BatchCoef {
  const uint32_t *w, *h, *v;
  uint64_t stride;
};

int batch_bw(mfh_ctx *c, const uint8_t *d_crs_c8, uint32_t rank, uint32_t world, uint32_t sg, const uint8_t *d_cw, bool has_delta, uint64_t *sproofs,
             const BatchScratch &B, size_t &slot, int accumulate) {
  const uint32_t d = c->P.d, m = c->P.m, n = c->P.n;
  const uint32_t ctb = c->P.logq / 8;
  const size_t ctl = (size_t)(n + 1) * ((c->P.logq + 63) / 64);
  const uint64_t ctr_ct = (uint64_t)ctb * n;
  const uint64_t pstride = 5 * ctl;
  const uint32_t lo = (uint32_t)((uint64_t)m * rank / world), cnt = (uint32_t)((uint64_t)m * (rank + 1) / world) - lo;
  const uint32_t bstride = (m + 6) / 8;
  MmIo io_bw = {{nullptr, nullptr}, sg, {sproofs + 4 * ctl, nullptr}, sg, pstride, d_cw, bstride, B.SCZ + 256 * slot++};
  io_bw.bits_row0 = lo;
  if (has_delta) {
    io_bw.add_ct = B.CT_T;
    io_bw.add_scale = (const uint32_t *)(d_cw + B.cw_delta_off);
  }
  return eval_rows_multi_io(c, ctr_ct * ((uint64_t)2 * d + lo), cnt, d_crs_c8 + ((size_t)2 * d + lo) * ctb, io_bw, sg, 1, accumulate);
}
int batch_rows_supergroup(mfh_ctx *c, const uint8_t *d_crs_c8, uint32_t rank, uint32_t world, uint32_t sg, const uint8_t *h_bits,
                          size_t bits_stride, const BatchCoef &co, uint64_t *sproofs, const BatchScratch &B, size_t &slot,
                          const uint32_t *h_delta, hipEvent_t wait_ev, int accumulate = 0, const uint8_t *d_cw = nullptr, bool bw_done = false,
                          uint32_t ws_slot = 0 , bool *tail_on_side = nullptr ) {
  const uint32_t d = c->P.d, m = c->P.m, n = c->P.n;
  const uint32_t ctb = c->P.logq / 8;
  const size_t ctl = (size_t)(n + 1) * ((c->P.logq + 63) / 64);
  const uint64_t ctr_ct = (uint64_t)ctb * n;
  const uint64_t pstride = 5 * ctl;
  hipStream_t const main_stream = c->stream, side_stream = c->side;
  const uint32_t loS = (uint32_t)((uint64_t)d * rank / world), cS = (uint32_t)((uint64_t)d * (rank + 1) / world) - loS;
  int rc = MFH_OK;
  if (!bw_done) {
    if (!d_cw) {
      const uint32_t bstride = (m + 6) / 8;
      const size_t staged = B.cw_delta_off + (h_delta ? (size_t)sg * 4 : 0);
      uint8_t *h_cw = (uint8_t *)pin_acquire(c, c->pin_cw, staged);
      if (!h_cw) return MFH_ENOMEM;
      for (uint32_t b = 0; b < sg; b++) memcpy(h_cw + (size_t)b * bstride, h_bits + (size_t)b * bits_stride, bstride);
      if (h_delta) memcpy(h_cw + B.cw_delta_off, h_delta, (size_t)sg * 4);
      HIP_TRY(c, hipMemcpyAsync(B.CW, h_cw, staged, hipMemcpyHostToDevice, c->stream));
      pin_release(c, c->pin_cw);
      d_cw = B.CW;
    }
    rc = batch_bw(c, d_crs_c8, rank, world, sg, d_cw, h_delta != nullptr, sproofs, B, slot, accumulate);
    if (rc) return rc;
  }
  if (wait_ev) HIP_TRY(c, hipStreamWaitEvent(main_stream, wait_ev, 0));
  HIP_TRY(c, hipEventRecord(c->ev_fork, main_stream));
  HIP_TRY(c, hipStreamWaitEvent(side_stream, c->ev_fork, 0));
  constexpr uint32_t NGLMAX = 8;
  const uint32_t NGL = c->mm_image ? c->batch_ngl : 1u;
  const MmRegion regs[2] = {{ctr_ct * loS, d_crs_c8 + (size_t)loS * ctb}, {ctr_ct * ((uint64_t)d + loS), d_crs_c8 + ((size_t)d + loS) * ctb}};
  const bool merged = mm_image_covers(c, regs[0].off, cS) && mm_image_covers(c, regs[1].off, cS) && c->batch_merge;
  if (merged) {
    constexpr uint32_t RMAX = (2 * BSG + 62) / 63;
    MmIo io[RMAX][2 * NGLMAX];
    uint32_t nv[RMAX][2 * NGLMAX];
    MmsPlan plan[RMAX];
    uint32_t R = 0;
    size_t ws_need = 0;
    const uint32_t nvtot = 2 * sg;
    auto run_io = [&](int region, uint32_t p, uint32_t cnt, uint32_t lender1) -> MmIo {
      const uint32_t x0 = std::min(p, sg), x1 = std::min(p + cnt, sg), y0 = std::max(p, sg) - sg;
      const uint32_t *X = region == 0 ? co.w : co.h, *Y = region == 0 ? co.h : co.v;
      uint64_t *OX = sproofs + (region == 0 ? 3 : 1) * ctl, *OY = sproofs + (region == 0 ? 0 : 2) * ctl;
      MmIo m = MmIo{{X + (uint64_t)x0 * co.stride, Y + (uint64_t)y0 * co.stride}, x1 - x0, {OX + (uint64_t)x0 * pstride, OY + (uint64_t)y0 * pstride}, x1 - x0, pstride,
                    nullptr, 0, B.SCZ + 256 * slot++, co.stride, 0};
      m.sa_from1 = lender1;
      return m;
    };
    for (uint32_t p0 = 0; p0 < nvtot; R++) {
      uint32_t cnt[NGLMAX], pos[NGLMAX], ng = 0, p = p0;
      for (; ng < NGL && p < nvtot; ng++) {
        pos[ng] = p;
        cnt[ng] = std::min(ng == 0 ? 63u : 64u, nvtot - p);
        p += cnt[ng];
      }
      for (uint32_t k = 0; k < ng; k++) {
        io[R][k] = run_io(0, pos[k], cnt[k], k ? 1 : 0);
        io[R][ng + k] = run_io(1, pos[k], cnt[k], k ? ng + 1 : 0);
        nv[R][k] = nv[R][ng + k] = cnt[k];
      }
      p0 = p;
      if (!mms_plan(c, regs, 2, cS, io[R], nv[R], ng, 4, plan[R])) { c->err = "mfh_prove_batch: the registered image does not serve the S / AS regions"; return MFH_EINVAL; }
      ws_need += (mms_ws_bytes(plan[R]) + 255) & ~(size_t)255;
    }
    const bool early = c->batch_early_chain && tail_on_side;
    if (early && (ws_slot == 0 || c->early_ws_half < ws_need)) {
      if (ws_slot != 0) { c->err = "early chain: a later super-group needs more scratch than the call's first"; return MFH_EINVAL; }
      c->early_ws_half = ws_need;
    }
    rc = buf_reserve(c, c->ws3, c->ws3_bytes, early ? 2 * c->early_ws_half : ws_need);
    if (rc) return rc;
    size_t wo = early ? (size_t)(ws_slot & 1) * c->early_ws_half : 0;
    for (uint32_t r = 0; r < R; r++) {
      mms_bind(plan[r], (uint8_t *)c->ws3 + wo);
      wo += (mms_ws_bytes(plan[r]) + 255) & ~(size_t)255;
      rc = mms_digits(c, plan[r], io[r], nv[r]);
      if (rc) return rc;
    }
    for (uint32_t r = 0; r < R; r++) {
      rc = mms_stream(c, plan[r]);
      if (rc) return rc;
      if (early) {
        while (c->ev_round.size() <= r) {
          hipEvent_t e;
          HIP_TRY(c, hipEventCreateWithFlags(&e, hipEventDisableTiming));
          c->ev_round.push_back(e);
        }
        HIP_TRY(c, hipEventRecord(c->ev_round[r], main_stream));
        HIP_TRY(c, hipStreamWaitEvent(side_stream, c->ev_round[r], 0));
        OnStream side(c, side_stream);
        rc = mms_finish(c, plan[r], io[r], nv[r], accumulate);
        if (rc) return rc;
        continue;
      }
      rc = mms_finish(c, plan[r], io[r], nv[r], accumulate);
      if (rc) return rc;
    }
    if (early) {
      *tail_on_side = true;
      return MFH_OK;
    }
  } else {
    for (uint32_t g0 = 0; g0 < sg; g0 += NGL * BG) {
      MmIo io[2 * NGLMAX];
      uint32_t nv[2 * NGLMAX], ng = 0;
      for (uint32_t k = 0; k < NGL && g0 + k * BG < sg; k++) ng++;
      for (uint32_t k = 0; k < ng; k++) {
        const uint32_t gg = g0 + k * BG, g = std::min(BG, sg - gg);
        uint64_t *proofs = sproofs + (size_t)gg * 5 * ctl;
        const uint64_t o = (uint64_t)gg * co.stride;
        io[k] = MmIo{{co.w + o, co.h + o}, g, {proofs + 3 * ctl, proofs}, g, pstride, nullptr, 0, B.SCZ + 256 * slot++, co.stride, 0};
        io[ng + k] = MmIo{{co.h + o, co.v + o}, g, {proofs + ctl, proofs + 2 * ctl}, g, pstride, nullptr, 0, B.SCZ + 256 * slot++, co.stride, 0};
        nv[k] = nv[ng + k] = 2 * g;
      }
      rc = eval_rows_multi_io_regions(c, regs, 1, cS, io, nv, ng, 4, accumulate);
      if (rc) return rc;
      {
        OnSide side(c, side_stream);
        rc = eval_rows_multi_io_regions(c, regs + 1, 1, cS, io + ng, nv + ng, ng, 4, accumulate);
        if (rc) return rc;
      }
    }
  }
  HIP_TRY(c, hipEventRecord(c->ev_join, side_stream));
  HIP_TRY(c, hipStreamWaitEvent(main_stream, c->ev_join, 0));
  return MFH_OK;
}

int batch_smudge(mfh_ctx *c, uint64_t *sproofs, uint32_t sg, const uint8_t *h_smudge_mag, size_t maglen, const uint8_t *h_smudge_sign) {
  std::vector<uint8_t> mags((size_t)sg * 5 * maglen), signs((size_t)sg * 5);
  for (int pass = 0; pass < 2; pass++) {
    std::fill(mags.begin(), mags.end(), 0);
    std::fill(signs.begin(), signs.end(), 0);
    for (uint32_t b = 0; b < sg; b++) {
      const uint8_t *pm = h_smudge_mag + (size_t)b * 5 * maglen, *ps = h_smudge_sign + (size_t)b * 5;
      if (pass == 0) {
        memcpy(&mags[(size_t)b * 5 * maglen], pm, 4 * maglen);
        memcpy(&signs[(size_t)b * 5], ps, 4);
      } else {
        memcpy(&mags[((size_t)b * 5 + 3) * maglen], pm + 4 * maglen, maglen);
        signs[(size_t)b * 5 + 3] = ps[4];
      }
    }
    int rc = mfh_ct_smudge(c, sproofs, (size_t)sg * 5, mags.data(), maglen, signs.data());
    if (rc) return rc;
  }
  return MFH_OK;
}

int batch_ct_t(mfh_ctx *c, const uint8_t *d_crs_c8, const BatchScratch &B) {
  const uint32_t d = c->P.d, ctb = c->P.logq / 8;
  HIP_TRY(c, hipMemsetD32Async((hipDeviceptr_t)B.ONE, 1, 1, c->stream));
  return mfh_eval_rows(c, (uint64_t)ctb * c->P.n * 2 * d, 1, d_crs_c8 + (size_t)2 * d * ctb, B.ONE, nullptr, B.CT_T, nullptr, 0);
}

struct ImageGuard {
  mfh_ctx *c;
  bool on;
  ~ImageGuard() { if (on) mfh_crs_set_resident_mm(c, nullptr); }
};
int batch_transient_image(mfh_ctx *c, const uint8_t *d_crs_c8, uint32_t nproofs, uint32_t rank, uint32_t world, ImageGuard &guard) {
  const uint32_t ctb = c->P.logq / 8;
  if (c->mm_image || !c->batch_image || nproofs <= BG || (((uint64_t)c->P.n * ctb) & 7)) return MFH_OK;
  const size_t ib = mfh_crs_mm_share_bytes(c, rank, world);
  if (c->batch_img_bytes < ib) {
    if (c->batch_img) { hipDeviceSynchronize(); hipFree(c->batch_img); c->batch_img = nullptr; c->batch_img_bytes = 0; }
    size_t mem_free = 0, mem_total = 0;
    if (hipMemGetInfo(&mem_free, &mem_total) != hipSuccess) mem_free = 0;
    if (ib <= mem_free / 4 * 3 && hipMalloc(&c->batch_img, ib) == hipSuccess) c->batch_img_bytes = ib;
    else { c->batch_img = nullptr; (void)hipGetLastError(); }
  }
  if (!c->batch_img) return MFH_OK;
  int rc = mfh_crs_expand_mm_share(c, d_crs_c8, rank, world, (uint8_t *)c->batch_img);
  if (rc) return rc;
  mfh_crs_set_resident_mm_share(c, (const uint8_t *)c->batch_img, rank, world);
  guard.on = true;
  return MFH_OK;
}

int prove_batch_impl(mfh_ctx *c, const uint8_t *d_crs_c8, const uint32_t *d_ssp, uint32_t nproofs, const uint8_t *h_witness_bits,
                     size_t bits_stride, const uint32_t *h_delta, const uint8_t *h_smudge_mag, size_t maglen, const uint8_t *h_smudge_sign,
                     uint64_t *d_proofs, const PubBatch *pub) {
  if (!c) return MFH_EINVAL;
  if (!nproofs) return MFH_OK;
  if (!d_crs_c8 || !h_witness_bits || !h_delta || !h_smudge_mag || !h_smudge_sign || !d_proofs) return MFH_EINVAL;
  if (c->resident_rows) { c->err = "mfh_prove_batch regenerates the keystream: clear the resident CRS image first"; return MFH_EUNSUPPORTED; }
  if (c->mm_image && c->mm_world != 1) { c->err = "mfh_prove_batch: the registered matrix-core image holds one rank's row shares (use mfh_prove_batch_partial)"; return MFH_EINVAL; }
  mf::SspSrc src;
  {
    int rc0 = ssp_src(c, d_ssp, src, true);
    if (rc0) return rc0;
    if (pub && (rc0 = ssp_rows_lu_check(c, d_ssp, pub->lu))) return rc0;
  }
  const uint32_t d = c->P.d, m = c->P.m, n = c->P.n;
  if (bits_stride < (m + 6) / 8) { c->err = "bits_stride shorter than the m - 1 witness bits"; return MFH_EINVAL; }
  for (uint32_t b = 0; b < nproofs; b++)
    if (h_delta[b] >= P32) { c->err = "delta must be < p"; return MFH_EINVAL; }
  if (maglen + 4 > (size_t)(c->P.logq / 64) * 8) { c->err = "smudge magnitude too wide"; return MFH_EINVAL; }
  const size_t ctl = (size_t)(n + 1) * ((c->P.logq + 63) / 64);
  HIP_TRY(c, hipSetDevice(c->device));
  const bool will_stream = c->mm_image || (c->batch_image && nproofs > BG && (((uint64_t)n * (c->P.logq / 8)) & 7) == 0);
  const uint32_t SG = will_stream ? BSG : BSG_REGEN;
  const uint32_t nsg = (nproofs + SG - 1) / SG;
  uint32_t nsl = 1;
  const uint32_t ctb0 = c->P.logq / 8;
  const bool slabs_ok = !c->mm_image && c->batch_image && nproofs > BG && (((uint64_t)n * ctb0) & 7) == 0;
  if (slabs_ok && c->batch_slabs) nsl = std::min(c->batch_slabs, std::max(1u, std::min(d, m)));
  else if (slabs_ok) {
    size_t mem_free = 0, mem_total = 0;
    if (hipMemGetInfo(&mem_free, &mem_total) == hipSuccess) {
      const size_t ib = mfh_crs_mm_image_bytes(c), avail = mem_free + c->batch_img_bytes + c->batch_bytes;
      if (ib > avail / 4 * 3) {
        const size_t budget = std::max<size_t>(avail / 3, (size_t)1 << 30);
        nsl = (uint32_t)std::min<size_t>(256, (ib + budget - 1) / budget);
        const size_t area = (size_t)3 * BSG * d * 4, maxsg = std::max<size_t>(1, avail / 4 / area);
        if (nsg > maxsg) {
          const size_t ctl0 = (size_t)(n + 1) * ((c->P.logq + 63) / 64);
          for (uint32_t s0 = 0; s0 < nproofs; s0 += (uint32_t)maxsg * SG) {
            const uint32_t cnt = std::min<uint32_t>((uint32_t)maxsg * SG, nproofs - s0);
            const PubBatch sub = pub ? pub->at(s0) : PubBatch{};
            int r = prove_batch_impl(c, d_crs_c8, d_ssp, cnt, h_witness_bits + (size_t)s0 * bits_stride, bits_stride, h_delta + s0,
                                     h_smudge_mag + (size_t)s0 * 5 * maglen, maglen, h_smudge_sign + (size_t)s0 * 5, d_proofs + (size_t)s0 * 5 * ctl0,
                                     pub ? &sub : nullptr);
            if (r) return r;
          }
          c->last_batch_sg = 0;
          return MFH_OK;
        }
      }
    }
  }
  const uint32_t nbuf = nsl > 1 ? nsg : 2;
  while (c->ev_sgdone.size() < nsg) {
    hipEvent_t e;
    HIP_TRY(c, hipEventCreateWithFlags(&e, hipEventDisableTiming));
    c->ev_sgdone.push_back(e);
  }
  c->last_batch_sg = 0;
  BatchScratch B;
  int rc = batch_scratch(c, nproofs, nbuf, B, nsl > 1 ? 1 : nsg, nsl > 1 ? 0 : nproofs);
  if (rc) return rc;
  size_t slot = 0;
  HIP_TRY(c, hipMemsetAsync(B.SCZ, 0, B.nslots * 2048, c->stream));
  rc = batch_streams(c);
  if (rc) return rc;
  while (c->ev_cdone.size() < nbuf) {
    hipEvent_t e0, e1, e2;
    HIP_TRY(c, hipEventCreateWithFlags(&e0, hipEventDisableTiming));
    HIP_TRY(c, hipEventCreateWithFlags(&e1, hipEventDisableTiming));
    HIP_TRY(c, hipEventCreateWithFlags(&e2, hipEventDisableTiming));
    c->ev_cdone.push_back(e0);
    c->ev_rdone.push_back(e1);
    c->ev_wdone.push_back(e2);
  }
  hipStream_t const main_stream = c->stream, chain_stream = c->side2;
  auto whv_of = [&](uint32_t sgi, uint32_t *&W, uint32_t *&H, uint32_t *&V) {
    W = B.WHV + (size_t)(sgi % nbuf) * 3 * BSG * d;
    H = W + (size_t)BSG * d;
    V = H + (size_t)BSG * d;
  };
  auto launch_chain = [&](uint32_t sgi) -> int {
    const uint32_t s0 = sgi * SG, sg = std::min(SG, nproofs - s0);
    uint32_t *WALL, *HALL, *VALL;
    whv_of(sgi, WALL, HALL, VALL);
    OnStream chain(c, chain_stream);
    const PubBatch psg = pub ? pub->at(s0) : PubBatch{};
    int r = batch_chain_launch(c, src, d_ssp, sg, h_witness_bits + (size_t)s0 * bits_stride, bits_stride, h_delta + s0, WALL, HALL, VALL, c->ev_wdone[sgi % nbuf],
                               pub ? &psg : nullptr);
    if (r) return r;
    HIP_TRY(c, hipEventRecord(c->ev_cdone[sgi % nbuf], chain_stream));
    return MFH_OK;
  };
  HIP_TRY(c, hipEventRecord(c->ev_chain, main_stream));
  HIP_TRY(c, hipStreamWaitEvent(chain_stream, c->ev_chain, 0));
  rc = launch_chain(0);
  if (rc) return rc;
  if (nsl > 1) {
    for (uint32_t k = 1; k < nsg; k++) {
      rc = launch_chain(k);
      if (rc) return rc;
    }
    for (;;) {
      size_t ib = 0;
      for (uint32_t r = 0; r < nsl; r++) ib = std::max(ib, mfh_crs_mm_share_bytes(c, r, nsl));
      if (c->batch_img_bytes >= ib) break;
      if (c->batch_img) { hipDeviceSynchronize(); hipFree(c->batch_img); c->batch_img = nullptr; c->batch_img_bytes = 0; }
      size_t mem_free = 0, mem_total = 0;
      const bool fits = hipMemGetInfo(&mem_free, &mem_total) != hipSuccess || ib + ((size_t)8 << 30) <= mem_free;
      if (fits && hipMalloc(&c->batch_img, ib) == hipSuccess) { c->batch_img_bytes = ib; break; }
      c->batch_img = nullptr;
      (void)hipGetLastError();
      const uint32_t cap = std::min<uint32_t>(256u, std::max(1u, std::min(d, m)));
      if (nsl >= cap || c->batch_slabs) { c->err = "mfh_prove_batch: no room for a row slab of the CRS image"; return MFH_ENOMEM; }
      nsl = std::min(cap, nsl * 2);
    }
    rc = batch_ct_t(c, d_crs_c8, B);
    if (rc) return rc;
    ImageGuard slab{c, true};
    for (uint32_t r = 0; r < nsl; r++) {
      rc = mfh_crs_expand_mm_share(c, d_crs_c8, r, nsl, (uint8_t *)c->batch_img);
      if (rc) return rc;
      mfh_crs_set_resident_mm_share(c, (const uint8_t *)c->batch_img, r, nsl);
      HIP_TRY(c, hipMemsetAsync(B.SCZ, 0, B.nslots * 2048, c->stream));
      slot = 0;
      const uint32_t loS = (uint32_t)((uint64_t)d * r / nsl);
      for (uint32_t s0 = 0, sgi = 0; s0 < nproofs; s0 += SG, sgi++) {
        const uint32_t sg = std::min(SG, nproofs - s0);
        uint32_t *WALL, *HALL, *VALL;
        whv_of(sgi, WALL, HALL, VALL);
        const BatchCoef co = {WALL + loS, HALL + loS, VALL + loS, d};
        rc = batch_rows_supergroup(c, d_crs_c8, r, nsl, sg, h_witness_bits + (size_t)s0 * bits_stride, bits_stride, co, d_proofs + (size_t)s0 * 5 * ctl, B, slot,
                                   r == 0 ? h_delta + s0 : nullptr, r == 0 ? c->ev_cdone[sgi % nbuf] : nullptr, r > 0);
        if (rc) return rc;
      }
    }
    for (uint32_t s0 = 0; s0 < nproofs; s0 += SG) {
      rc = batch_smudge(c, d_proofs + (size_t)s0 * 5 * ctl, std::min(SG, nproofs - s0), h_smudge_mag + (size_t)s0 * 5 * maglen, maglen, h_smudge_sign + (size_t)s0 * 5);
      if (rc) return rc;
      HIP_TRY(c, hipEventRecord(c->ev_sgdone[s0 / SG], c->stream));
    }
    c->last_batch_sg = SG;
    c->last_batch_n = nproofs;
    return MFH_OK;
  }
  ImageGuard transient{c, false};
  rc = batch_transient_image(c, d_crs_c8, nproofs, 0, 1, transient);
  if (rc) return rc;
  rc = batch_stage_host(c, B, nproofs, h_witness_bits, bits_stride, h_delta, h_smudge_mag, maglen, h_smudge_sign, SG);
  if (rc) return rc;
  rc = batch_ct_t(c, d_crs_c8, B);
  if (rc) return rc;
  bool bw_done = false;
  if (c->batch_bw_merged && nsg > 1 && mm_image_covers(c, (uint64_t)ctb0 * n * 2 * d, m)) {
    const uint64_t ctr_ct = (uint64_t)ctb0 * n, pstride = 5 * ctl;
    const uint32_t bstride = (m + 6) / 8;
    const MmRegion reg = {ctr_ct * 2 * d, d_crs_c8 + (size_t)2 * d * ctb0};
    for (uint32_t g0 = 0; g0 < nsg; g0 += 8) {
      MmIo ios[8];
      uint32_t nvs[8];
      const uint32_t ng = std::min(8u, nsg - g0);
      for (uint32_t k = 0; k < ng; k++) {
        const uint32_t sgi = g0 + k, s0 = sgi * SG, sg = std::min(SG, nproofs - s0);
        const uint8_t *d_cw = B.CW + (size_t)sgi * B.cw_stride;
        ios[k] = MmIo{{nullptr, nullptr}, sg, {d_proofs + (size_t)s0 * 5 * ctl + 4 * ctl, nullptr}, sg, pstride, d_cw, bstride, B.SCZ + 256 * slot++};
        ios[k].add_ct = B.CT_T;
        ios[k].add_scale = (const uint32_t *)(d_cw + B.cw_delta_off);
        nvs[k] = sg;
      }
      rc = ng > 1 ? eval_rows_multi_io_regions(c, &reg, 1, m, ios, nvs, ng, 1, 0) : eval_rows_multi_io(c, reg.off, m, reg.c8, ios[0], nvs[0], 1, 0);
      if (rc) return rc;
    }
    bw_done = true;
  }
  const bool early = c->batch_early_chain && bw_done;
  bool any_on_side = false;
  for (uint32_t s0 = 0, sgi = 0; s0 < nproofs; s0 += SG, sgi++) {
    const uint32_t sg = std::min(SG, nproofs - s0);
    uint64_t *sproofs = d_proofs + (size_t)s0 * 5 * ctl;
    uint32_t *WALL, *HALL, *VALL;
    whv_of(sgi, WALL, HALL, VALL);
    const BatchCoef co = {WALL, HALL, VALL, d};
    if (early && sgi + 1 < nsg) {
      if (sgi >= 1) HIP_TRY(c, hipStreamWaitEvent(chain_stream, c->ev_rdone[(sgi - 1) % nbuf], 0));
      rc = launch_chain(sgi + 1);
      if (rc) return rc;
    }
    if (early && sgi >= 2) HIP_TRY(c, hipStreamWaitEvent(main_stream, c->ev_sgdone[sgi - 2], 0));
    HIP_TRY(c, hipStreamWaitEvent(main_stream, c->ev_wdone[sgi % nbuf], 0));
    bool on_side = false;
    rc = batch_rows_supergroup(c, d_crs_c8, 0, 1, sg, h_witness_bits + (size_t)s0 * bits_stride, bits_stride, co, sproofs, B, slot, h_delta + s0,
                               c->ev_cdone[sgi % nbuf], 0, B.CW + (size_t)sgi * B.cw_stride, bw_done, sgi, early ? &on_side : nullptr);
    if (rc) return rc;
    if (early) HIP_TRY(c, hipEventRecord(c->ev_rdone[sgi % nbuf], main_stream));
    else if (sgi + 1 < nsg) {
      HIP_TRY(c, hipEventRecord(c->ev_rdone[sgi % nbuf], main_stream));
      HIP_TRY(c, hipStreamWaitEvent(chain_stream, c->ev_rdone[sgi % nbuf], 0));
      rc = launch_chain(sgi + 1);
      if (rc) return rc;
    }
    {
      OnStream tail(c, on_side ? c->side : main_stream);
      rc = batch_smudge_staged(c, B, sproofs, s0, sg);
      if (rc) return rc;
      HIP_TRY(c, hipEventRecord(c->ev_sgdone[sgi], c->stream));
    }
    any_on_side = any_on_side || on_side;
  }
  if (any_on_side) {
    HIP_TRY(c, hipEventRecord(c->ev_join, c->side));
    HIP_TRY(c, hipStreamWaitEvent(main_stream, c->ev_join, 0));
  }
  c->last_batch_sg = SG;
  c->last_batch_n = nproofs;
  return MFH_OK;
}

}

extern "C" {

int mfh_prove_batch(mfh_ctx *c, const uint8_t *d_crs_c8, const uint32_t *d_ssp, uint32_t nproofs, const uint8_t *h_witness_bits,
                    size_t bits_stride, const uint32_t *h_delta, const uint8_t *h_smudge_mag, size_t maglen, const uint8_t *h_smudge_sign,
                    uint64_t *d_proofs) {
  return prove_batch_impl(c, d_crs_c8, d_ssp, nproofs, h_witness_bits, bits_stride, h_delta, h_smudge_mag, maglen, h_smudge_sign, d_proofs, nullptr);
}

int mfh_prove_batch_public(mfh_ctx *c, const uint8_t *d_crs_c8, const uint32_t *d_ssp, uint32_t lu, uint32_t nproofs, const uint8_t *h_bits,
                           size_t bits_stride, const uint32_t *h_delta, const uint8_t *h_smudge_mag, size_t maglen, const uint8_t *h_smudge_sign,
                           uint64_t *d_proofs) {
  if (!c) return MFH_EINVAL;
  if (lu >= c->P.m) { c->err = "lu must be < m (the m - 1 wires of the SSP)"; return MFH_EINVAL; }
  if (!lu) return mfh_prove_batch(c, d_crs_c8, d_ssp, nproofs, h_bits, bits_stride, h_delta, h_smudge_mag, maglen, h_smudge_sign, d_proofs);
  if (!nproofs) return MFH_OK;
  if (!h_bits) return MFH_EINVAL;
  const uint32_t m = c->P.m, bstride = (m + 6) / 8, ub = (lu + 7) / 8;
  if (bits_stride < bstride) { c->err = "bits_stride shorter than the m - 1 witness bits"; return MFH_EINVAL; }
  std::vector<uint8_t> priv((size_t)nproofs * bstride), pubb;
  std::vector<uint32_t> zero;
  for (uint32_t b = 0; b < nproofs; b++) {
    uint8_t *x = priv.data() + (size_t)b * bstride;
    memcpy(x, h_bits + (size_t)b * bits_stride, bstride);
    memset(x, 0, lu >> 3);
    if (lu & 7) x[lu >> 3] &= (uint8_t)(0xffu << (lu & 7));
  }
  if (lu > kPubDirect) {
    pubb.assign((size_t)nproofs * bstride, 0);
    zero.assign(nproofs, 0);
    for (uint32_t b = 0; b < nproofs; b++) {
      uint8_t *x = pubb.data() + (size_t)b * bstride;
      memcpy(x, h_bits + (size_t)b * bits_stride, ub);
      if (lu & 7) x[ub - 1] &= (uint8_t)((1u << (lu & 7)) - 1);
    }
  }
  HIP_TRY(c, hipSetDevice(c->device));
  const size_t need = (size_t)nproofs * ub;
  if (c->pub_bytes < need) {
    if (c->d_pub) { hipDeviceSynchronize(); hipFree(c->d_pub); c->d_pub = nullptr; c->pub_bytes = 0; }
    HIP_TRY(c, hipMalloc(&c->d_pub, need));
    c->pub_bytes = need;
  }
  uint8_t *st = (uint8_t *)pin_acquire(c, c->pin_pub, need);
  if (!st) return MFH_ENOMEM;
  for (uint32_t b = 0; b < nproofs; b++) memcpy(st + (size_t)b * ub, h_bits + (size_t)b * bits_stride, ub);
  HIP_TRY(c, hipMemcpyAsync(c->d_pub, st, need, hipMemcpyHostToDevice, c->stream));
  pin_release(c, c->pin_pub);
  const PubBatch pb{lu, c->d_pub, ub, lu > kPubDirect ? pubb.data() : nullptr, bstride, lu > kPubDirect ? zero.data() : nullptr};
  return prove_batch_impl(c, d_crs_c8, d_ssp, nproofs, priv.data(), bstride, h_delta, h_smudge_mag, maglen, h_smudge_sign, d_proofs, &pb);
}

uint32_t mfh_prove_batch_supergroup(const mfh_ctx *c) { return c ? c->last_batch_sg : 0; }

int mfh_prove_batch_stream_wait(mfh_ctx *c, uint32_t upto, void *hip_stream) {
  if (!c) return MFH_EINVAL;
  if (!c->last_batch_sg || !upto || upto > c->last_batch_n) { c->err = "mfh_prove_batch_stream_wait: no such statements in the last mfh_prove_batch call"; return MFH_EINVAL; }
  HIP_TRY(c, hipStreamWaitEvent((hipStream_t)hip_stream, c->ev_sgdone[(upto - 1) / c->last_batch_sg], 0));
  return MFH_OK;
}

int mfh_batch_chain(mfh_ctx *c, const uint32_t *d_ssp, uint32_t nstmt, const uint8_t *h_witness_bits, size_t bits_stride, const uint32_t *h_delta,
                    uint32_t *d_w, uint32_t *d_h, uint32_t *d_v) {
  if (!c) return MFH_EINVAL;
  if (!nstmt) return MFH_OK;
  if (!h_witness_bits || !h_delta || !d_w || !d_h || !d_v) return MFH_EINVAL;
  mf::SspSrc src;
  int rc = ssp_src(c, d_ssp, src, true);
  if (rc) return rc;
  const uint32_t d = c->P.d, m = c->P.m;
  if (bits_stride < (m + 6) / 8) { c->err = "bits_stride shorter than the m - 1 witness bits"; return MFH_EINVAL; }
  for (uint32_t b = 0; b < nstmt; b++)
    if (h_delta[b] >= P32) { c->err = "delta must be < p"; return MFH_EINVAL; }
  HIP_TRY(c, hipSetDevice(c->device));
  for (uint32_t s0 = 0; s0 < nstmt; s0 += BSG) {
    const size_t o = (size_t)s0 * d;
    rc = batch_chain_launch(c, src, d_ssp, std::min(BSG, nstmt - s0), h_witness_bits + (size_t)s0 * bits_stride, bits_stride, h_delta + s0, d_w + o, d_h + o,
                            d_v + o);
    if (rc) return rc;
  }
  return MFH_OK;
}

int mfh_batch_witness_cols(mfh_ctx *c, const uint32_t *d_ssp, uint32_t nstmt, const uint8_t *h_witness_bits, size_t bits_stride, const uint32_t *h_delta,
                           uint32_t col0, uint32_t ncols, uint32_t *d_w, size_t w_stride) {
  if (!c) return MFH_EINVAL;
  if (!nstmt || !ncols) return MFH_OK;
  if (!h_witness_bits || !h_delta || !d_w) return MFH_EINVAL;
  if (bits_stride < (c->P.m + 6) / 8) { c->err = "bits_stride shorter than the m - 1 witness bits"; return MFH_EINVAL; }
  for (uint32_t s0 = 0; s0 < nstmt; s0 += BSG) {
    int rc = mfh_witness_poly_mm_cols(c, d_ssp, std::min(BSG, nstmt - s0), h_witness_bits + (size_t)s0 * bits_stride, bits_stride, h_delta + s0, col0, ncols,
                                      d_w + (size_t)s0 * w_stride, w_stride);
    if (rc) return rc;
  }
  return MFH_OK;
}
int mfh_batch_chain_from_w(mfh_ctx *c, const uint32_t *d_ssp, uint32_t nstmt, const uint32_t *d_w, uint32_t *d_h, uint32_t *d_v) {
  if (!c) return MFH_EINVAL;
  if (!nstmt) return MFH_OK;
  if (!d_w || !d_h || !d_v) return MFH_EINVAL;
  mf::SspSrc src;
  int rc = ssp_src(c, d_ssp, src, true);
  if (rc) return rc;
  const uint32_t d = c->P.d;
  HIP_TRY(c, hipSetDevice(c->device));
  for (uint32_t s0 = 0; s0 < nstmt; s0 += BSG) {
    const uint32_t sg = std::min(BSG, nstmt - s0);
    const size_t o = (size_t)s0 * d;
    hipLaunchKernelGGL(k_add_slot_multi, dim3((d + 255) / 256, sg), dim3(256), 0, c->stream, d_w + o, src, 1u, d, d_v + o);
    HIP_TRY(c, hipGetLastError());
    rc = mfh_poly_h_multi(c, d_v + o, d_h + o, sg);
    if (rc) return rc;
  }
  return MFH_OK;
}

int mfh_prove_batch_partial(mfh_ctx *c, const uint8_t *d_crs_c8, uint32_t rank, uint32_t world, uint32_t nstmt, const uint8_t *h_witness_bits,
                            size_t bits_stride, const uint32_t *d_w, const uint32_t *d_h, const uint32_t *d_v, size_t coef_stride, uint64_t *d_partial) {
  if (!c || !world || rank >= world) return MFH_EINVAL;
  if (!nstmt) return MFH_OK;
  if (!d_crs_c8 || !h_witness_bits || !d_w || !d_h || !d_v || !d_partial) return MFH_EINVAL;
  if (c->resident_rows) { c->err = "mfh_prove_batch_partial: clear the single-proof resident CRS image first"; return MFH_EUNSUPPORTED; }
  if (c->mm_image && (c->mm_rank != rank || c->mm_world != world)) {
    c->err = "the registered matrix-core image holds the row shares of a different (rank, world)";
    return MFH_EINVAL;
  }
  const uint32_t d = c->P.d, m = c->P.m, n = c->P.n;
  const uint32_t cS = (uint32_t)((uint64_t)d * (rank + 1) / world) - (uint32_t)((uint64_t)d * rank / world);
  if (bits_stride < (m + 6) / 8) { c->err = "bits_stride shorter than the m - 1 witness bits"; return MFH_EINVAL; }
  if (coef_stride < cS) { c->err = "coef_stride shorter than the rank's share of the S / AS rows"; return MFH_EINVAL; }
// ... 79 lines not shown
```

include/mfhip.h:

```cpp
#pragma once
#include <stddef.h>
#include <stdint.h>

#ifdef __cplusplus
extern "C" {
#endif

#define MFH_P 0xfffffffbu

enum {
  MFH_OK = 0,
  MFH_EINVAL = -1,
  MFH_EDEVICE = -2,
  MFH_ENOMEM = -3,
  MFH_EUNSUPPORTED = -4
};

typedef struct {
  uint32_t n;
  uint32_t logq;
  uint32_t d;
  uint32_t m;
} mfh_params;

typedef struct mfh_ctx mfh_ctx;

int mfh_ctx_create(mfh_ctx **out, int device, const mfh_params *P);
void mfh_ctx_destroy(mfh_ctx *ctx);
int mfh_set_stream(mfh_ctx *ctx, void *hip_stream);
int mfh_sync(mfh_ctx *ctx);
int mfh_scrub_staging(mfh_ctx *ctx);
const char *mfh_last_error(const mfh_ctx *ctx);
int mfh_set_seed(mfh_ctx *ctx, const uint8_t h_seed[40]);

int mfh_keystream(mfh_ctx *ctx, uint64_t off, void *d_out, size_t nbytes);
int mfh_sample_rows(mfh_ctx *ctx, uint64_t off, size_t nrows, uint64_t *d_out);

int mfh_ct_add(mfh_ctx *ctx, uint64_t *d_rop, const uint64_t *d_a, const uint64_t *d_b, size_t count);
int mfh_ct_mul_ui(mfh_ctx *ctx, uint64_t *d_rop, const uint64_t *d_a, uint32_t b, size_t count);
int mfh_ct_addmul_ui(mfh_ctx *ctx, uint64_t *d_rop, const uint64_t *d_a, uint32_t b, size_t count);

int mfh_eval_rows(mfh_ctx *ctx, uint64_t off, size_t nrows, const uint8_t *d_c8, const uint32_t *d_coeff0,
                  const uint32_t *d_coeff1, uint64_t *d_rop0, uint64_t *d_rop1, int accumulate);

size_t mfh_resident_row_bytes(const mfh_ctx *ctx);
int mfh_crs_expand(mfh_ctx *ctx, uint64_t off, size_t nrows, const uint8_t *d_c8, void *d_rows_out);
int mfh_crs_image_set_b(mfh_ctx *ctx, size_t first_row, size_t nrows, const uint8_t *d_c8, void *d_rows);
int mfh_eval_rows_resident(mfh_ctx *ctx, const void *d_rows, size_t first_row, size_t nrows, const uint32_t *d_coeff0,
                           const uint32_t *d_coeff1, uint64_t *d_rop0, uint64_t *d_rop1, int accumulate);
int mfh_crs_set_resident(mfh_ctx *ctx, const void *d_rows);
int mfh_crs_set_resident_prefix(mfh_ctx *ctx, const void *d_rows, size_t nrows_resident);
size_t mfh_resident_share_rows(const mfh_ctx *ctx, uint32_t rank, uint32_t world);
int mfh_crs_expand_share(mfh_ctx *ctx, const uint8_t *d_crs_c8, uint32_t rank, uint32_t world, void *d_image);
int mfh_crs_set_resident_share(mfh_ctx *ctx, const void *d_image, uint32_t rank, uint32_t world);

int mfh_encrypt_rows(mfh_ctx *ctx, uint64_t off, size_t nrows, const uint64_t *d_sk, const uint32_t *d_msg,
                     const uint64_t *d_err, uint8_t *d_c8_out);
int mfh_set_encrypt_path(mfh_ctx *ctx, int path);

int mfh_decrypt(mfh_ctx *ctx, const uint64_t *d_sk, const uint64_t *d_cts, size_t count, uint32_t *d_out);
int mfh_set_decrypt_path(mfh_ctx *ctx, int path);
int mfh_decrypt_rows(mfh_ctx *ctx, uint64_t off, size_t nrows, const uint64_t *d_sk, const uint8_t *d_c8, uint32_t *d_out);

int mfh_add_dotp(mfh_ctx *ctx, uint64_t *d_rop, const uint64_t *d_a, const uint64_t *d_b, size_t len);

int mfh_ct_smudge(mfh_ctx *ctx, uint64_t *d_cts, size_t count, const uint8_t *h_mag, size_t maglen, const uint8_t *h_sign);

int mfh_ssp_upload(mfh_ctx *ctx, const void *h_ssp_u64, uint32_t *d_ssp, size_t first_slot, size_t nslots);
int mfh_witness_poly(mfh_ctx *ctx, const uint32_t *d_ssp, const uint8_t *h_witness_bits, uint32_t delta, uint32_t *d_w);

int mfh_ssp_set_prg(mfh_ctx *ctx, uint64_t seed, const uint32_t *d_t);
int mfh_ssp_prg_make_t(mfh_ctx *ctx, uint64_t seed, const uint8_t *h_witness_bits, uint32_t *d_t);
int mfh_ssp_prg_fill(mfh_ctx *ctx, uint64_t seed, size_t first_slot, size_t nslots, uint32_t *d_out);

int mfh_ssp_from_rows(mfh_ctx *ctx, uint32_t nrows, const uint32_t *h_row_ptr, const uint32_t *h_wire, const uint32_t *h_coef, uint32_t *d_ssp);

int mfh_ssp_set_rows(mfh_ctx *ctx, uint32_t nrows, const uint32_t *h_row_ptr, const uint32_t *h_wire, const uint32_t *h_coef, uint32_t lu_max);
int mfh_ssp_rows_fill(mfh_ctx *ctx, size_t first_slot, size_t nslots, uint32_t *d_out);

#define MFH_GATE_XOR 0u
#define MFH_GATE_AND 1u
#define MFH_GATE_OR 2u
#define MFH_GATE_NOT 3u
#define MFH_CIRCUIT_MAX_WIRES 32767u
typedef struct mfh_circuit mfh_circuit;
int mfh_circuit_create(mfh_ctx *ctx, uint32_t nin, uint32_t ngates, const uint32_t *h_gates, uint32_t nasserts, const uint32_t *h_asserts,
                       mfh_circuit **out);
int mfh_circuit_create_global(mfh_ctx *ctx, uint32_t nin, uint32_t ngates, const uint32_t *h_gates, uint32_t nasserts, const uint32_t *h_asserts,
                              mfh_circuit **out);
void mfh_circuit_destroy(mfh_circuit *c);
int mfh_circuit_assign(mfh_ctx *ctx, const mfh_circuit *c, uint32_t nstmt, const uint8_t *h_inputs, size_t in_stride, uint8_t *h_witness_bits,
                       size_t bits_stride, uint8_t *h_holds);

int mfh_poly_mul(mfh_ctx *ctx, const uint32_t *d_a, size_t la, const uint32_t *d_b, size_t lb, uint32_t *d_c);
int mfh_poly_add(mfh_ctx *ctx, const uint32_t *d_a, const uint32_t *d_b, size_t count, uint32_t *d_out);
int mfh_poly_prepare_t(mfh_ctx *ctx, const uint32_t *d_t);
int mfh_ssp_prepare(mfh_ctx *ctx, const uint32_t *d_ssp);
int mfh_poly_h(mfh_ctx *ctx, const uint32_t *d_v, uint32_t *d_h);
int mfh_poly_h_multi(mfh_ctx *ctx, const uint32_t *d_v, uint32_t *d_h, uint32_t nb);
int mfh_set_poly_exact(mfh_ctx *ctx, int mode);
long mfh_poly_exact_fallbacks(mfh_ctx *ctx);

int mfh_setup_messages(mfh_ctx *ctx, const uint32_t *d_ssp, uint32_t alpha, uint32_t beta, uint32_t s, uint32_t *d_msg);
int mfh_setup(mfh_ctx *ctx, const uint32_t *d_ssp, uint32_t alpha, uint32_t beta, uint32_t s, const uint64_t *d_sk,
              const uint64_t *d_err, uint8_t *d_crs_c8);
int mfh_setup_image(mfh_ctx *ctx, const uint32_t *d_ssp, uint32_t alpha, uint32_t beta, uint32_t s, const uint64_t *d_sk,
                    const uint64_t *d_err, uint8_t *d_crs_c8, void *d_rows_image);
int mfh_prove(mfh_ctx *ctx, const uint8_t *d_crs_c8, const uint32_t *d_ssp, const uint8_t *h_witness_bits, uint32_t delta,
              const uint8_t *h_smudge_mag, size_t maglen, const uint8_t *h_smudge_sign, uint64_t *d_proof);

int mfh_verify(mfh_ctx *ctx, const uint32_t *d_ssp, uint32_t alpha, uint32_t beta, uint32_t s, const uint64_t *d_sk,
               const uint64_t *d_proofs, size_t count, uint8_t *d_ok);

int mfh_setup_public(mfh_ctx *ctx, const uint32_t *d_ssp, uint32_t alpha, uint32_t beta, uint32_t s, uint32_t lu, const uint64_t *d_sk,
                     const uint64_t *d_err, uint8_t *d_crs_c8, void *d_rows_image);
int mfh_prove_public(mfh_ctx *ctx, const uint8_t *d_crs_c8, const uint32_t *d_ssp, uint32_t lu, const uint8_t *h_bits, uint32_t delta,
                     const uint8_t *h_smudge_mag, size_t maglen, const uint8_t *h_smudge_sign, uint64_t *d_proof);
int mfh_prove_batch_public(mfh_ctx *ctx, const uint8_t *d_crs_c8, const uint32_t *d_ssp, uint32_t lu, uint32_t nproofs, const uint8_t *h_bits,
                           size_t bits_stride, const uint32_t *h_delta, const uint8_t *h_smudge_mag, size_t maglen, const uint8_t *h_smudge_sign,
                           uint64_t *d_proofs);
int mfh_vk_derive(mfh_ctx *ctx, const uint32_t *d_ssp, uint32_t s, uint32_t lu, uint32_t *d_vk);
int mfh_verify_public(mfh_ctx *ctx, const uint32_t *d_vk, uint32_t lu, uint32_t alpha, uint32_t beta, const uint64_t *d_sk, const uint64_t *d_proofs,
                      const uint8_t *h_statements, size_t stmt_stride, size_t count, uint8_t *d_ok);

size_t mfh_crs_mm_image_bytes(const mfh_ctx *ctx);
int mfh_crs_expand_mm(mfh_ctx *ctx, const uint8_t *d_crs_c8, uint8_t *d_image);
int mfh_crs_set_resident_mm(mfh_ctx *ctx, const uint8_t *d_image);
int mfh_set_expand_path(mfh_ctx *ctx, int path);
int mfh_set_batch_image(mfh_ctx *ctx, int enabled);
int mfh_set_batch_slabs(mfh_ctx *ctx, uint32_t nslabs);
int mfh_set_encrypt_chunks(mfh_ctx *ctx, uint32_t chunks);
int mfh_set_eval_path(mfh_ctx *ctx, int path);
int mfh_set_witness_per(mfh_ctx *ctx, uint32_t statements);
int mfh_set_batch_launch(mfh_ctx *ctx, uint32_t groups_per_launch, int merge_regions);
int mfh_set_batch_bw(mfh_ctx *ctx, int merged);
int mfh_set_mm_stream(mfh_ctx *ctx, int map, int persistent, int sync_mode, uint32_t spin_max);
int mfh_set_mm_width(mfh_ctx *ctx, uint32_t per_xcd, int early_chain);
int mfh_set_mm_chunk_rows(mfh_ctx *ctx, uint32_t rows);
int mfh_set_mm_pack(mfh_ctx *ctx, int on);
int mfh_prove_batch(mfh_ctx *ctx, const uint8_t *d_crs_c8, const uint32_t *d_ssp, uint32_t nproofs, const uint8_t *h_witness_bits,
                    size_t bits_stride, const uint32_t *h_delta, const uint8_t *h_smudge_mag, size_t maglen, const uint8_t *h_smudge_sign,
                    uint64_t *d_proofs);
uint32_t mfh_prove_batch_supergroup(const mfh_ctx *ctx);
int mfh_prove_batch_stream_wait(mfh_ctx *ctx, uint32_t upto, void *hip_stream);
size_t mfh_crs_mm_share_bytes(const mfh_ctx *ctx, uint32_t rank, uint32_t world);
int mfh_crs_expand_mm_share(mfh_ctx *ctx, const uint8_t *d_crs_c8, uint32_t rank, uint32_t world, uint8_t *d_image);
int mfh_crs_set_resident_mm_share(mfh_ctx *ctx, const uint8_t *d_image, uint32_t rank, uint32_t world);
int mfh_batch_chain(mfh_ctx *ctx, const uint32_t *d_ssp, uint32_t nstmt, const uint8_t *h_witness_bits, size_t bits_stride, const uint32_t *h_delta,
                    uint32_t *d_w, uint32_t *d_h, uint32_t *d_v);
int mfh_batch_witness_cols(mfh_ctx *ctx, const uint32_t *d_ssp, uint32_t nstmt, const uint8_t *h_witness_bits, size_t bits_stride, const uint32_t *h_delta,
                           uint32_t col0, uint32_t ncols, uint32_t *d_w, size_t w_stride);
int mfh_batch_chain_from_w(mfh_ctx *ctx, const uint32_t *d_ssp, uint32_t nstmt, const uint32_t *d_w, uint32_t *d_h, uint32_t *d_v);
int mfh_prove_batch_partial(mfh_ctx *ctx, const uint8_t *d_crs_c8, uint32_t rank, uint32_t world, uint32_t nstmt, const uint8_t *h_witness_bits,
                            size_t bits_stride, const uint32_t *d_w, const uint32_t *d_h, const uint32_t *d_v, size_t coef_stride, uint64_t *d_partial);
int mfh_prove_batch_finish(mfh_ctx *ctx, const uint8_t *d_crs_c8, uint32_t nstmt, const uint32_t *h_delta, const uint8_t *h_smudge_mag, size_t maglen,
                           const uint8_t *h_smudge_sign, uint64_t *d_proofs);

int mfh_prove_partial(mfh_ctx *ctx, const uint8_t *d_crs_c8, const uint32_t *d_ssp, const uint8_t *h_witness_bits, uint32_t delta,
                      uint32_t rank, uint32_t world, uint64_t *d_partial);
int mfh_prove_finish(mfh_ctx *ctx, uint64_t *d_proof, const uint8_t *h_smudge_mag, size_t maglen, const uint8_t *h_smudge_sign);
int mfh_witness_poly_multi(mfh_ctx *ctx, const uint32_t *d_ssp, uint32_t nstmt, const uint8_t *h_bits, size_t bits_stride, const uint32_t *h_delta,
                           uint32_t *d_w);
int mfh_witness_poly_mm(mfh_ctx *ctx, const uint32_t *d_ssp, uint32_t nstmt, const uint8_t *h_bits, size_t bits_stride, const uint32_t *h_delta,
                        uint32_t *d_w);
int mfh_witness_poly_mm_cols(mfh_ctx *ctx, const uint32_t *d_ssp, uint32_t nstmt, const uint8_t *h_bits, size_t bits_stride, const uint32_t *h_delta,
                             uint32_t col0, uint32_t ncols, uint32_t *d_w, size_t w_stride);
int mfh_witness_lanes(mfh_ctx *ctx, const uint32_t *d_ssp, const uint8_t *h_witness_bits, uint32_t rank, uint32_t world, uint64_t *d_lanes);
int mfh_witness_from_lanes(mfh_ctx *ctx, const uint32_t *d_ssp, const uint64_t *d_lanes, uint32_t delta, uint32_t *d_w);
int mfh_prove_partial_w(mfh_ctx *ctx, const uint8_t *d_crs_c8, const uint32_t *d_ssp, const uint8_t *h_witness_bits, uint32_t delta,
                        uint32_t rank, uint32_t world, const uint64_t *d_wlanes, uint64_t *d_partial);
uint32_t mfh_lanes_per_value(const mfh_ctx *ctx);
int mfh_ct_to_lanes(mfh_ctx *ctx, const uint64_t *d_cts, size_t count, uint64_t *d_lanes);
int mfh_ct_from_lanes(mfh_ctx *ctx, const uint64_t *d_lanes, size_t count, uint64_t *d_cts);

const char *mfh_version(void);
int mfh_digest128(mfh_ctx *ctx, const void *d_buf, size_t nbytes, uint64_t h_digest[2]);
size_t mfh_workspace_bytes(const mfh_ctx *ctx);
int mfh_eval_rows_multi(mfh_ctx *ctx, uint64_t off, size_t nrows, const uint8_t *d_c8, const uint32_t *d_coeffs, uint32_t nvec,
                        uint32_t coeff_bytes, uint64_t *d_rops, int accumulate);

int mfh_set_timing(mfh_ctx *ctx, int enabled);
int mfh_set_overlap(mfh_ctx *ctx, int mode);
int mfh_timing_drain(mfh_ctx *ctx, const char *which, uint64_t *count, double *total_ms, uint64_t *total_rows, float *last_ms);
float mfh_last_kernel_ms(mfh_ctx *ctx, const char *which);
double mfh_timing_busy_ms(const mfh_ctx *ctx);
uint64_t mfh_timing_work_rows(const mfh_ctx *ctx);

#ifdef __cplusplus
}
#endif
```

Baseline: 14180.

## Run witness/H chain once per call and batch witness groups into one launch

Adds a call-level chain mode, on by default: instead of launching the witness→V→H chain per supergroup on the side stream, interleaved with the row passes, it runs the whole chain once for all proofs before the row loop, using buffers sized for every supergroup. It also adds a grouped witness path that packs all 256-statement groups into one staging upload and one k_witness_mm8q launch, with a block remap that interleaves groups. The aim is to cut launch count, event synchronisation and per-group host overhead. In exchange the W/H/V buffers grow to hold every proof, and the first row pass must wait for the full chain, which removes the finer-grained overlap between chain and rows.

```diff
diff --git a/c-lwe-snarks_amd/__init__.py b/c-lwe-snarks_amd/__init__.py
--- a/c-lwe-snarks_amd/__init__.py
+++ b/c-lwe-snarks_amd/__init__.py
@@ -80,7 +80,7 @@
     "mfh_encrypt_rows", "mfh_decrypt", "mfh_ct_smudge", "mfh_ssp_upload", "mfh_witness_poly", "mfh_version",
     "mfh_workspace_bytes", "mfh_last_kernel_ms", "mfh_set_timing", "mfh_set_overlap", "mfh_eval_rows_multi", "mfh_prove_batch", "mfh_crs_mm_image_bytes", "mfh_crs_expand_mm", "mfh_crs_set_resident_mm", "mfh_witness_poly_multi", "mfh_witness_poly_mm", "mfh_poly_h_multi", "mfh_poly_mul", "mfh_poly_add", "mfh_poly_prepare_t",
     "mfh_ssp_prepare", "mfh_poly_h", "mfh_setup_messages", "mfh_setup", "mfh_setup_image", "mfh_crs_image_set_b", "mfh_prove",
-    "mfh_prove_partial", "mfh_prove_finish", "mfh_ct_to_lanes", "mfh_ct_from_lanes", "mfh_lanes_per_value", "mfh_digest128", "mfh_timing_drain", "mfh_timing_busy_ms", "mfh_timing_work_rows", "mfh_set_batch_image", "mfh_set_batch_slabs", "mfh_set_expand_path", "mfh_set_encrypt_path", "mfh_set_batch_launch", "mfh_set_batch_bw", "mfh_set_mm_chunk_rows", "mfh_set_mm_pack", "mfh_set_poly_exact", "mfh_poly_exact_fallbacks", "mfh_set_mm_stream", "mfh_add_dotp", "mfh_set_encrypt_chunks", "mfh_set_witness_per", "mfh_set_eval_path", "mfh_set_decrypt_path", "mfh_decrypt_rows",
+    "mfh_prove_partial", "mfh_prove_finish", "mfh_ct_to_lanes", "mfh_ct_from_lanes", "mfh_lanes_per_value", "mfh_digest128", "mfh_timing_drain", "mfh_timing_busy_ms", "mfh_timing_work_rows", "mfh_set_batch_image", "mfh_set_batch_slabs", "mfh_set_expand_path", "mfh_set_encrypt_path", "mfh_set_batch_launch", "mfh_set_batch_bw", "mfh_set_batch_chain", "mfh_set_mm_chunk_rows", "mfh_set_mm_pack", "mfh_set_poly_exact", "mfh_poly_exact_fallbacks", "mfh_set_mm_stream", "mfh_add_dotp", "mfh_set_encrypt_chunks", "mfh_set_witness_per", "mfh_set_eval_path", "mfh_set_decrypt_path", "mfh_decrypt_rows",
     "mfh_crs_mm_share_bytes", "mfh_crs_expand_mm_share", "mfh_crs_set_resident_mm_share", "mfh_batch_chain", "mfh_batch_witness_cols", "mfh_batch_chain_from_w", "mfh_witness_poly_mm_cols", "mfh_prove_batch_partial", "mfh_prove_batch_finish",
     "mfh_resident_row_bytes", "mfh_crs_expand", "mfh_eval_rows_resident", "mfh_crs_set_resident",
     "mfh_witness_lanes", "mfh_witness_from_lanes", "mfh_prove_partial_w", "mfh_verify",
@@ -181,6 +181,7 @@
         "mfh_set_mm_stream": (i32, [vp, i32, i32, i32, u32]),
         "mfh_set_batch_launch": (i32, [vp, u32, i32]),
         "mfh_set_batch_bw": (i32, [vp, i32]),
+        "mfh_set_batch_chain": (i32, [vp, i32]),
         "mfh_set_encrypt_path": (i32, [vp, i32]),
         "mfh_set_expand_path": (i32, [vp, i32]),
         "mfh_set_batch_slabs": (i32, [vp, u32]),
@@ -348,6 +349,9 @@
     def set_batch_bw(self, merged=True):
         self._chk(self.lib.mfh_set_batch_bw(self._h, 1 if merged else 0))
 
+    def set_batch_chain(self, call_level=True):
+        self._chk(self.lib.mfh_set_batch_chain(self._h, 1 if call_level else 0))
+
     def set_mm_stream(self, map=0, persistent=False, sync_mode=0, spin_max=64):
         self._chk(self.lib.mfh_set_mm_stream(self._h, int(map), int(persistent), int(sync_mode), int(spin_max)))
 
diff --git a/c-lwe-snarks_amd/csrc/ctx.hpp b/c-lwe-snarks_amd/csrc/ctx.hpp
--- a/c-lwe-snarks_amd/csrc/ctx.hpp
+++ b/c-lwe-snarks_amd/csrc/ctx.hpp
@@ -120,6 +120,7 @@
   uint32_t enc_chunks = 0;
   uint32_t witness_per = 0;
   uint32_t batch_slabs = 0;
+  int batch_call_chain = 1;
   int batch_bw_merged = 1;
   int batch_merge = 1;
   uint32_t batch_ngl = 8;
@@ -228,6 +229,8 @@
 extern "C" int mfh_witness_poly_mm_cols(mfh_ctx *c, const uint32_t *d_ssp, uint32_t nstmt, const uint8_t *h_bits, size_t bits_stride, const uint32_t *h_delta,
                                         uint32_t col0, uint32_t ncols, uint32_t *d_w, size_t w_stride);
 extern "C" int mfh_poly_h_multi(mfh_ctx *c, const uint32_t *d_v, uint32_t *d_h, uint32_t nb);
+extern "C" int poly_h_multi_batches(mfh_ctx *c, const uint32_t *d_v, uint32_t *d_h, uint32_t nb, uint32_t batches);
+extern "C" int witness_poly_mm_groups(mfh_ctx *c, const uint32_t *d_ssp, uint32_t nstmt, const uint8_t *h_bits, size_t bits_stride, const uint32_t *h_delta, uint32_t *d_w);
 int aux_reserve(mfh_ctx *c, size_t bytes);
 int expand_mm_region(mfh_ctx *c, uint64_t off, uint32_t nrows, const uint8_t *c8, uint8_t *image);
 int encrypt_rows_mm(mfh_ctx *c, uint64_t off, size_t nrows, const uint64_t *sk, const uint32_t *msg, const uint64_t *err, uint8_t *c8);
diff --git a/c-lwe-snarks_amd/csrc/evalmm.hip b/c-lwe-snarks_amd/csrc/evalmm.hip
--- a/c-lwe-snarks_amd/csrc/evalmm.hip
+++ b/c-lwe-snarks_amd/csrc/evalmm.hip
@@ -1205,14 +1205,32 @@
 }
 __global__ __launch_bounds__(512) void k_witness_mm8q(const v4i *__restrict__ sspfrag, const v4i *__restrict__ bitfrag, uint32_t nrowsel ,
                                                       uint32_t ksteps_per_chunk, uint32_t d, int *__restrict__ part, const uint32_t *__restrict__ tpoly ,
-                                                      const uint32_t *__restrict__ cnt_delta, uint32_t nstmt, uint32_t *__restrict__ w_out, WCols wc) {
+                                                      const uint32_t *__restrict__ cnt_delta, uint32_t nstmt, uint32_t *__restrict__ w_out, WCols wc,
+                                                      uint32_t ngroups = 1, uint32_t frag_gs = 0, uint32_t cd_gs = 0) {
   constexpr int MT = 8, RING = 4, PF = 4;
   __shared__ v4i bits[RING][MT][64];
   __shared__ uint32_t xch[2][3][16][64];
   const uint32_t tid = threadIdx.x, lane = tid & 63, wave = tid >> 6;
   const uint32_t r32 = lane & 31, h = lane >> 5;
   const uint32_t tile = wave >> 2, pl = wave & 3;
-  const uint32_t ktl = blockIdx.x * 2 + tile, kt = wc.kt0 + ktl;
+  uint32_t bx = blockIdx.x;
+  if (ngroups > 1) {
+    const uint32_t nx = gridDim.x / ngroups;
+    uint32_t g;
+    if (nx % 8 == 0) {
+      const uint32_t r = bx >> 3;
+      g = r % ngroups;
+      bx = (r / ngroups) * 8 + (bx & 7);
+    } else {
+      g = bx / nx;
+      bx %= nx;
+    }
+    bitfrag += (uint64_t)g * frag_gs;
+    cnt_delta += (uint64_t)g * cd_gs;
+    w_out += (uint64_t)g * 256 * wc.wstride;
+    nstmt = min(256u, nstmt - 256 * g);
+  }
+  const uint32_t ktl = bx * 2 + tile, kt = wc.kt0 + ktl;
   const uint32_t K0 = blockIdx.y * ksteps_per_chunk, K1 = min((nrowsel + 31) / 32, K0 + ksteps_per_chunk);
   v16i acc[MT];
 #pragma unroll
@@ -1728,6 +1746,23 @@
 }
 int mfh_crs_set_resident_mm(mfh_ctx *c, const uint8_t *d_image) { return mfh_crs_set_resident_mm_share(c, d_image, 0, 1); }
 
+static int ssp_frag_ensure(mfh_ctx *c, const uint32_t *d_ssp) {
+  const uint32_t d = c->P.d, nrowsel = c->P.m - 1, ksteps = (nrowsel + 31) / 32;
+  const size_t sfrag_b = (size_t)ksteps * 32 * d * 4;
+  if (c->ssp_frag_src != d_ssp || c->ssp_frag_bytes < sfrag_b) {
+    if (c->ssp_frag_bytes < sfrag_b) {
+      if (c->ssp_frag) { hipStreamSynchronize(c->stream); hipFree(c->ssp_frag); c->ssp_frag = nullptr; c->ssp_frag_bytes = 0; }
+      HIP_TRY(c, hipMalloc(&c->ssp_frag, sfrag_b));
+      c->ssp_frag_bytes = sfrag_b;
+    }
+    const uint64_t nthreads = (uint64_t)ksteps * (d / 32) * 256;
+    hipLaunchKernelGGL(k_ssp_frag, dim3((uint32_t)((nthreads + 255) / 256)), dim3(256), 0, c->stream, d_ssp, nrowsel, d, (uint32_t *)c->ssp_frag);
+    HIP_TRY(c, hipGetLastError());
+    c->ssp_frag_src = d_ssp;
+  }
+  return MFH_OK;
+}
+
 int mfh_witness_poly_mm_cols(mfh_ctx *c, const uint32_t *d_ssp, uint32_t nstmt, const uint8_t *h_bits, size_t bits_stride, const uint32_t *h_delta,
                              uint32_t col0, uint32_t ncols, uint32_t *d_w, size_t w_stride) {
   if (!c || !h_bits || !h_delta || !d_w || nstmt == 0 || nstmt > 256) return MFH_EINVAL;
@@ -1751,17 +1786,9 @@
   const uint32_t nrowsel = m - 1, ksteps = (nrowsel + 31) / 32;
   const bool fused = MT == 8 && src.dense && m < 65536 && (nc >= 16384 || ksteps <= 64);
   const uint32_t nchunks = fused ? 1u : std::min(ksteps, 4u), kpc = (ksteps + nchunks - 1) / nchunks;
-  const size_t sfrag_b = (size_t)ksteps * 32 * d * 4;
-  if (src.dense && (c->ssp_frag_src != d_ssp || c->ssp_frag_bytes < sfrag_b)) {
-    if (c->ssp_frag_bytes < sfrag_b) {
-      if (c->ssp_frag) { hipStreamSynchronize(c->stream); hipFree(c->ssp_frag); c->ssp_frag = nullptr; c->ssp_frag_bytes = 0; }
-      HIP_TRY(c, hipMalloc(&c->ssp_frag, sfrag_b));
-      c->ssp_frag_bytes = sfrag_b;
-    }
-    const uint64_t nthreads = (uint64_t)ksteps * (d / 32) * 256;
-    hipLaunchKernelGGL(k_ssp_frag, dim3((uint32_t)((nthreads + 255) / 256)), dim3(256), 0, c->stream, d_ssp, nrowsel, d, (uint32_t *)c->ssp_frag);
-    HIP_TRY(c, hipGetLastError());
-    c->ssp_frag_src = d_ssp;
+  if (src.dense) {
+    int rcf = ssp_frag_ensure(c, d_ssp);
+    if (rcf) return rcf;
   }
   const size_t packed = (size_t)nstmt * bits_stride, head_b = ((packed + 8 + 256 * 8 + 255) & ~(size_t)255);
   const size_t frag_b = (size_t)ksteps * MT * 1024, part_b = (size_t)nchunks * 4 * 32 * MT * nc * 4;
@@ -1829,4 +1856,62 @@
   return mfh_witness_poly_mm_cols(c, d_ssp, nstmt, h_bits, bits_stride, h_delta, 0, c->P.d, d_w, c->P.d);
 }
 
-}
+int witness_poly_mm_groups(mfh_ctx *c, const uint32_t *d_ssp, uint32_t nstmt, const uint8_t *h_bits, size_t bits_stride, const uint32_t *h_delta, uint32_t *d_w) {
+  if (!c || !h_bits || !h_delta || !d_w || nstmt == 0) return MFH_EINVAL;
+  const uint32_t d = c->P.d, m = c->P.m, G = (nstmt + 255) / 256;
+  const uint32_t nrowsel = m - 1, ksteps = (nrowsel + 31) / 32;
+  mf::SspSrc src;
+  bool one = G > 1 && !ssp_is_rows(c, d_ssp) && d % 128 == 0 && m >= 2 && m < 65536 && (d >= 16384 || ksteps <= 64);
+  if (one) {
+    int rc0 = ssp_src(c, d_ssp, src);
+    if (rc0) return rc0;
+    one = src.dense;
+  }
+  if (!one) {
+    for (uint32_t b0 = 0; b0 < nstmt; b0 += 256) {
+      int r = mfh_witness_poly_mm(c, d_ssp, std::min(256u, nstmt - b0), h_bits + (size_t)b0 * bits_stride, bits_stride, h_delta + b0, d_w + (size_t)b0 * d);
+      if (r) return r;
+    }
+    return MFH_OK;
+  }
+  for (uint32_t b = 0; b < nstmt; b++)
+    if (h_delta[b] >= MFH_P) { c->err = "delta must be < p"; return MFH_EINVAL; }
+  HIP_TRY(c, hipSetDevice(c->device));
+  int rc = ssp_frag_ensure(c, d_ssp);
+  if (rc) return rc;
+  const size_t packed = (size_t)256 * bits_stride, cd_off = packed + ((8 - packed % 8) % 8);
+  const size_t head_b = (cd_off + 256 * 8 + 255) & ~(size_t)255, frag_b = (size_t)ksteps * 8 * 1024;
+  rc = wws_reserve(c, G * (head_b + frag_b));
+  if (rc) return rc;
+  PinBuf &wpin = c->pin_wring[c->pin_wnext++ % 8];
+  uint8_t *stage = (uint8_t *)pin_acquire(c, wpin, G * head_b);
+  if (!stage) return MFH_ENOMEM;
+  for (uint32_t g = 0; g < G; g++) {
+    const uint32_t b0 = 256 * g, nb = std::min(256u, nstmt - b0);
+    uint8_t *hg = stage + (size_t)g * head_b;
+    memcpy(hg, h_bits + (size_t)b0 * bits_stride, (size_t)nb * bits_stride);
+    uint32_t *cd = (uint32_t *)(hg + cd_off);
+    for (uint32_t b = 0; b < nb; b++) {
+      uint32_t cnt = 0;
+      const uint8_t *hb = h_bits + (size_t)(b0 + b) * bits_stride;
+      for (uint32_t r = 0; r + 8 <= nrowsel; r += 8) cnt += (uint32_t)__builtin_popcount(hb[r >> 3]);
+      for (uint32_t r = nrowsel & ~7u; r < nrowsel; r++) cnt += (hb[r >> 3] >> (r & 7)) & 1;
+      cd[2 * b] = cnt;
+      cd[2 * b + 1] = h_delta[b0 + b];
+    }
+  }
+  uint8_t *dev = (uint8_t *)c->wws;
+  HIP_TRY(c, hipMemcpyAsync(dev, stage, G * head_b, hipMemcpyHostToDevice, c->stream));
+  pin_release(c, wpin);
+  int8_t *d_frag = (int8_t *)(dev + G * head_b);
+  for (uint32_t g = 0; g < G; g++)
+    hipLaunchKernelGGL(k_witness_bits, dim3((uint32_t)((frag_b / 16 + 255) / 256)), dim3(256), 0, c->stream, dev + (size_t)g * head_b, bits_stride,
+                       std::min(256u, nstmt - 256 * g), nrowsel, ksteps, 8u, d_frag + (size_t)g * frag_b);
+  const WCols wc = {0, ksteps, (uint64_t)d};
+  hipLaunchKernelGGL(k_witness_mm8q, dim3(G * (d / 64), 1), dim3(512), 0, c->stream, (const v4i *)c->ssp_frag, (const v4i *)d_frag, nrowsel, ksteps, d,
+                     (int *)nullptr, (const uint32_t *)src.t, (const uint32_t *)(dev + cd_off), nstmt, d_w, wc, G, (uint32_t)(frag_b / 16), (uint32_t)(head_b / 4));
+  HIP_TRY(c, hipGetLastError());
+  return MFH_OK;
+}
+
+}
diff --git a/c-lwe-snarks_amd/csrc/mfhip.hip b/c-lwe-snarks_amd/csrc/mfhip.hip
--- a/c-lwe-snarks_amd/csrc/mfhip.hip
+++ b/c-lwe-snarks_amd/csrc/mfhip.hip
@@ -1112,6 +1112,12 @@
   return MFH_OK;
 }
 
+int mfh_set_batch_chain(mfh_ctx *c, int call_level) {
+  if (!c) return MFH_EINVAL;
+  c->batch_call_chain = call_level != 0;
+  return MFH_OK;
+}
+
 int mfh_set_batch_image(mfh_ctx *c, int en) {
   if (!c) return MFH_EINVAL;
   c->batch_image = en != 0;
diff --git a/c-lwe-snarks_amd/csrc/poly.hip b/c-lwe-snarks_amd/csrc/poly.hip
--- a/c-lwe-snarks_amd/csrc/poly.hip
+++ b/c-lwe-snarks_amd/csrc/poly.hip
@@ -937,8 +937,8 @@
   return MFH_OK;
 }
 
-int mfh_poly_h_multi(mfh_ctx *c, const uint32_t *d_v, uint32_t *d_h, uint32_t nb) {
-  if (!c || !d_v || !d_h || !nb || nb > kMaxBatch) return MFH_EINVAL;
+int poly_h_multi_batches(mfh_ctx *c, const uint32_t *d_v, uint32_t *d_h, uint32_t nb, uint32_t batches) {
+  if (!c || !d_v || !d_h || !nb || nb > kMaxBatch || !batches) return MFH_EINVAL;
   PolyState *S = c->poly;
   if (!S || !S->have_t) {
     c->err = "mfh_poly_prepare_t has not been called for this SSP";
@@ -957,7 +957,7 @@
       S->rest = 64;
     }
     if (S->rest) {
-      S->rest--;
+      S->rest -= std::min<uint32_t>(S->rest, batches);
       exact = false;
     }
   }
@@ -1015,6 +1015,7 @@
   HIP_TRY(c, hipGetLastError());
   return MFH_OK;
 }
+int mfh_poly_h_multi(mfh_ctx *c, const uint32_t *d_v, uint32_t *d_h, uint32_t nb) { return poly_h_multi_batches(c, d_v, d_h, nb, 1); }
 int mfh_set_poly_exact(mfh_ctx *c, int mode) {
   if (!c || mode < 0 || mode > 2) return MFH_EINVAL;
   c->poly_exact = mode;
diff --git a/c-lwe-snarks_amd/csrc/snark.hip b/c-lwe-snarks_amd/csrc/snark.hip
--- a/c-lwe-snarks_amd/csrc/snark.hip
+++ b/c-lwe-snarks_amd/csrc/snark.hip
@@ -692,12 +692,15 @@
 };
 
 int batch_chain_launch(mfh_ctx *c, const mf::SspSrc &src, const uint32_t *d_ssp, uint32_t sg, const uint8_t *h_bits, size_t bits_stride,
-                       const uint32_t *h_delta, uint32_t *W, uint32_t *H, uint32_t *V, hipEvent_t ev_witness = nullptr, const PubBatch *pub = nullptr) {
+                       const uint32_t *h_delta, uint32_t *W, uint32_t *H, uint32_t *V, hipEvent_t ev_witness = nullptr, const PubBatch *pub = nullptr,
+                       uint32_t batches = 1) {
   const uint32_t d = c->P.d;
   int rc = MFH_OK;
   auto witness_pass = [&](const uint8_t *bits, size_t stride, const uint32_t *delta, uint32_t *out) -> int {
-    if (d % 128 == 0) {
-      const uint32_t per = c->witness_per ? c->witness_per : 256u;
+    if (d % 128 == 0 && !c->witness_per) {
+      return witness_poly_mm_groups(c, d_ssp, sg, bits, stride, delta, out);
+    } else if (d % 128 == 0) {
+      const uint32_t per = c->witness_per;
       for (uint32_t b0 = 0; b0 < sg; b0 += per) {
         int r = mfh_witness_poly_mm(c, d_ssp, std::min(per, sg - b0), bits + (size_t)b0 * stride, stride, delta + b0, out + (size_t)b0 * d);
         if (r) return r;
@@ -724,7 +727,7 @@
   else
     hipLaunchKernelGGL(k_add_slot_multi, dim3((d + 255) / 256, sg), dim3(256), 0, c->stream, W, src, 1u, d, V);
   HIP_TRY(c, hipGetLastError());
-  return mfh_poly_h_multi(c, V, H, sg);
+  return poly_h_multi_batches(c, V, H, sg, batches);
 }
 
 struct BatchCoef {
@@ -983,7 +986,8 @@
       }
     }
   }
-  const uint32_t nbuf = nsl > 1 ? nsg : 2;
+  const bool call_chain = c->batch_call_chain && will_stream && nsl == 1;
+  const uint32_t nbuf = nsl > 1 || call_chain ? nsg : 2;
   while (c->ev_sgdone.size() < nsg) {
     hipEvent_t e;
     HIP_TRY(c, hipEventCreateWithFlags(&e, hipEventDisableTiming));
@@ -1008,6 +1012,12 @@
   }
   hipStream_t const main_stream = c->stream, chain_stream = c->side2;
   auto whv_of = [&](uint32_t sgi, uint32_t *&W, uint32_t *&H, uint32_t *&V) {
+    if (call_chain) {
+      W = B.WHV + (size_t)sgi * SG * d;
+      H = W + (size_t)nproofs * d;
+      V = H + (size_t)nproofs * d;
+      return;
+    }
     W = B.WHV + (size_t)(sgi % nbuf) * 3 * BSG * d;
     H = W + (size_t)BSG * d;
     V = H + (size_t)BSG * d;
@@ -1024,10 +1034,12 @@
     HIP_TRY(c, hipEventRecord(c->ev_cdone[sgi % nbuf], chain_stream));
     return MFH_OK;
   };
-  HIP_TRY(c, hipEventRecord(c->ev_chain, main_stream));
-  HIP_TRY(c, hipStreamWaitEvent(chain_stream, c->ev_chain, 0));
-  rc = launch_chain(0);
-  if (rc) return rc;
+  if (!call_chain) {
+    HIP_TRY(c, hipEventRecord(c->ev_chain, main_stream));
+    HIP_TRY(c, hipStreamWaitEvent(chain_stream, c->ev_chain, 0));
+    rc = launch_chain(0);
+    if (rc) return rc;
+  }
   if (nsl > 1) {
     for (uint32_t k = 1; k < nsg; k++) {
       rc = launch_chain(k);
@@ -1083,6 +1095,17 @@
   if (rc) return rc;
   rc = batch_ct_t(c, d_crs_c8, B);
   if (rc) return rc;
+  if (call_chain) {
+    HIP_TRY(c, hipEventRecord(c->ev_chain, main_stream));
+    HIP_TRY(c, hipStreamWaitEvent(chain_stream, c->ev_chain, 0));
+    uint32_t *WALL, *HALL, *VALL;
+    whv_of(0, WALL, HALL, VALL);
+    OnStream chain(c, chain_stream);
+    rc = batch_chain_launch(c, src, d_ssp, nproofs, h_witness_bits, bits_stride, h_delta, WALL, HALL, VALL, c->ev_wdone[0], pub, nsg);
+    if (rc) return rc;
+    HIP_TRY(c, hipEventRecord(c->ev_cdone[0], chain_stream));
+    HIP_TRY(c, hipStreamWaitEvent(main_stream, c->ev_wdone[0], 0));
+  }
   bool bw_done = false;
   if (c->batch_bw_merged && nsg > 1 && mm_image_covers(c, (uint64_t)ctb0 * n * 2 * d, m)) {
     const uint64_t ctr_ct = (uint64_t)ctb0 * n, pstride = 5 * ctl;
@@ -1113,19 +1136,20 @@
     uint32_t *WALL, *HALL, *VALL;
     whv_of(sgi, WALL, HALL, VALL);
     const BatchCoef co = {WALL, HALL, VALL, d};
-    if (early && sgi + 1 < nsg) {
+    if (early && !call_chain && sgi + 1 < nsg) {
       if (sgi >= 1) HIP_TRY(c, hipStreamWaitEvent(chain_stream, c->ev_rdone[(sgi - 1) % nbuf], 0));
       rc = launch_chain(sgi + 1);
       if (rc) return rc;
     }
     if (early && sgi >= 2) HIP_TRY(c, hipStreamWaitEvent(main_stream, c->ev_sgdone[sgi - 2], 0));
-    HIP_TRY(c, hipStreamWaitEvent(main_stream, c->ev_wdone[sgi % nbuf], 0));
+    if (!call_chain) HIP_TRY(c, hipStreamWaitEvent(main_stream, c->ev_wdone[sgi % nbuf], 0));
     bool on_side = false;
+    hipEvent_t const chain_ev = !call_chain ? c->ev_cdone[sgi % nbuf] : sgi == 0 ? c->ev_cdone[0] : nullptr;
     rc = batch_rows_supergroup(c, d_crs_c8, 0, 1, sg, h_witness_bits + (size_t)s0 * bits_stride, bits_stride, co, sproofs, B, slot, h_delta + s0,
-                               c->ev_cdone[sgi % nbuf], 0, B.CW + (size_t)sgi * B.cw_stride, bw_done, sgi, early ? &on_side : nullptr);
+                               chain_ev, 0, B.CW + (size_t)sgi * B.cw_stride, bw_done, sgi, early ? &on_side : nullptr);
     if (rc) return rc;
-    if (early) HIP_TRY(c, hipEventRecord(c->ev_rdone[sgi % nbuf], main_stream));
-    else if (sgi + 1 < nsg) {
+    if (early && !call_chain) HIP_TRY(c, hipEventRecord(c->ev_rdone[sgi % nbuf], main_stream));
+    else if (!call_chain && sgi + 1 < nsg) {
       HIP_TRY(c, hipEventRecord(c->ev_rdone[sgi % nbuf], main_stream));
       HIP_TRY(c, hipStreamWaitEvent(chain_stream, c->ev_rdone[sgi % nbuf], 0));
       rc = launch_chain(sgi + 1);
diff --git a/include/mfhip.h b/include/mfhip.h
--- a/include/mfhip.h
+++ b/include/mfhip.h
@@ -134,6 +134,7 @@
 int mfh_set_witness_per(mfh_ctx *ctx, uint32_t statements);
 int mfh_set_batch_launch(mfh_ctx *ctx, uint32_t groups_per_launch, int merge_regions);
 int mfh_set_batch_bw(mfh_ctx *ctx, int merged);
+int mfh_set_batch_chain(mfh_ctx *ctx, int call_level);
 int mfh_set_mm_stream(mfh_ctx *ctx, int map, int persistent, int sync_mode, uint32_t spin_max);
 int mfh_set_mm_width(mfh_ctx *ctx, uint32_t per_xcd, int early_chain);
 int mfh_set_mm_chunk_rows(mfh_ctx *ctx, uint32_t rows);
```

Result: no change. 14220, median of 6 (+0.3%).
